# chahuja/mix-stage

Measured on AMD Instinct MI355X. Metric: train-step clips/sec (B=32, T=64, M=8), higher is better.
Workload: dtype f32; 1 GPU; Mix-StAGE GAN train step (reference D/G coin flip, seed 4321: 457 G + 510 D steps), B=32 clips per GPU, T=64, 128-mel, 104-dim pose, M=S=8, audio branch pinned; fp32 arithmetic (the reference trains in fp64, trainer.py:138; held to it at 1e-4 pose L1); global_batch=32, parallelism=dp1, hip_graphs=True, bn_sync=local

## Files before the change

### include/mixstage.h

```cpp
#ifndef MIXSTAGE_H_
#define MIXSTAGE_H_

#include <stddef.h>
#include <stdint.h>

#ifdef __cplusplus
extern "C" {
#endif

#define MS_ABI_VERSION 4

enum ms_block_mode {
  MS_BARE = 0,
  MS_LRELU = 1,
  MS_BN_TRAIN = 2,
  MS_BN_EVAL = 3
};

enum ms_input_mode {
  MS_IN_PLAIN = 0,
  MS_IN_BCAST = 1,
  MS_IN_UP2ADD = 2
};

enum ms_dtype { MS_F32 = 0, MS_BF16 = 1, MS_F16 = 2 };
#define MS_DT_OUT_F32 0x100
#define MS_DT_BN_FOLDED 0x200
#define MS_DT_STAT_PAIR 0x400

typedef struct ms_conv_desc {
  int32_t B;
  int32_t Cin;
  int32_t H, W;
  int32_t Cout;
  int32_t groups;
  int32_t KH, KW, SH, SW, PH, PW;
  int32_t OH, OW;
  int32_t mode;
  int32_t in_mode;
  float slope;
  float eps;
  float momentum;
  int32_t dtype;
} ms_conv_desc;

const char* ms_last_error(void);
int ms_abi_version(void);
int ms_stat_pair_ok(const ms_conv_desc* d);

size_t ms_conv_block_fwd_workspace(const ms_conv_desc* d);
size_t ms_conv_block_bwd_workspace(const ms_conv_desc* d);

int ms_conv_block_fwd(const ms_conv_desc* d, const float* x, const float* x2, const float* w,
                      const float* bias, const float* gamma, const float* beta, float* running_mean,
                      float* running_var, float* y_raw, float* y, float* save, void* workspace,
                      size_t workspace_bytes, void* stream);

typedef struct ms_fwd_options {
  const void* w_planes;
  int32_t* bn_sync;
  int32_t bn_sync_words;
} ms_fwd_options;
int ms_conv_block_fwd_ex(const ms_conv_desc* d, const float* x, const float* x2, const float* w,
                         const float* bias, const float* gamma, const float* beta, float* running_mean,
                         float* running_var, float* y_raw, float* y, float* save, void* workspace,
                         size_t workspace_bytes, void* stream, const ms_fwd_options* opt);
size_t ms_fwd_weights_bytes(const ms_conv_desc* d);
int ms_fwd_weights_prepare(int n, const ms_conv_desc* descs, const float* const* w, void* const* planes, void* stream);

int ms_conv_block_bwd(const ms_conv_desc* d, const float* x, const float* x2, const float* w,
                      const float* gamma, const float* running_mean, const float* running_var,
                      const float* y_raw, const float* y, const float* save, const float* dy, float* dyr,
                      float* dx, float* dx2, float* dw, float* dbias, float* dgamma, float* dbeta,
                      void* workspace, size_t workspace_bytes, void* stream);

typedef struct ms_bwd_options {
  void* side_stream;
  void* side_workspace;
  size_t side_workspace_bytes;
  const float* wt_prepared;
  float* wgrad_partials;
  int defer_wgrad_launch;
  const float* prev_y;
  const float* prev_y_raw;
  const float* prev_save;
  const float* prev_gamma;
  float* prev_dgamma;
  float* prev_dbeta;
  float* prev_dbias;
  float prev_slope;
  int32_t* bn_sync;
  int32_t bn_sync_words;
  int dy_is_dyr;
  const float* dx_accum;
} ms_bwd_options;
int ms_dgrad_takes_accum(const ms_conv_desc* d);
int ms_dgrad_fuses_prev_bn(const ms_conv_desc* d);
int ms_conv_block_bwd_ex(const ms_conv_desc* d, const float* x, const float* x2, const float* w,
                         const float* gamma, const float* running_mean, const float* running_var,
                         const float* y_raw, const float* y, const float* save, const float* dy, float* dyr,
                         float* dx, float* dx2, float* dw, float* dbias, float* dgamma, float* dbeta,
                         void* workspace, size_t workspace_bytes, void* stream, const ms_bwd_options* opt);

typedef struct ms_prep16_item {
  const ms_conv_desc* desc;
  const float* w;
  const float* bias;
  const float* gamma;
  const float* beta;
  const float* running_mean;
  const float* running_var;
  void* fwd;
  void* dgrad;
} ms_prep16_item;
size_t ms_weights16_bytes(const ms_conv_desc* d, int which);
int ms_weights16_prepare(int n, const ms_prep16_item* items, void* stream);

int ms_set_bn_sync_buffer(int32_t* zeroed_words, int n);

int ms_cb8_from_plain(int dtype, const float* x, void* y, int B, int C, int HW, void* stream);
int ms_cb8_to_plain(int dtype, const void* x, float* y, int B, int C, int HW, void* stream);
int ms_cb8_from_btc(int dtype, const float* x, void* y, int B, int T, int C, int velocity, void* stream);
int ms_cb8_to_btc(int dtype, const void* x, float* y, int B, int T, int C, int velocity_bwd, void* stream);

size_t ms_dgrad_weights_elems(const ms_conv_desc* d, const float* w);
int ms_set_precision(int mode);
int ms_get_precision(void);
int ms_tuning_epoch(void);
int ms_dgrad_weights_prepare(int n, const ms_conv_desc* descs, const float* const* w, float* const* wt, void* stream);

size_t ms_wgrad_partials_elems(const ms_conv_desc* d, int* splits);
int ms_set_wgrad_batched(int on, int tiles_per_workgroup);
int ms_wgrad_flush(void* stream);
int ms_wgrad_discard(void);
int ms_wgrad_reduce_multi(int n, const float* const* partials, float* const* dw, const int* elems, const int* splits,
                          void* stream);

int ms_bn_stats(const float* y_raw, float* stats, int B, int C, int HW, void* stream);
int ms_bn_train_apply(const float* stats_all, int world, int n_local, const float* gamma, const float* beta, float* running_mean,
                      float* running_var, const float* y_raw, float* y, float* save, int B, int C, int HW, float eps,
                      float momentum, float slope, void* stream);
size_t ms_bn_bwd_workspace(int B, int C);
int ms_bn_bwd_sums(const float* dy, const float* y_raw, const float* save, float* sums, int B, int C, int HW, float slope,
                   void* workspace, size_t workspace_bytes, void* stream);
int ms_bn_bwd_apply(const float* dy, const float* y_raw, const float* save, const float* gamma, const float* sums_global,
                    double n_global, float* dyr, int B, int C, int HW, float slope, void* stream);

int ms_lerp_time_fwd(const float* x, float* y, int B, int C, int Tin, int F, int Tout, void* stream);
int ms_lerp_time_bwd(const float* dy, float* dx, int B, int C, int Tin, int F, int Tout, void* stream);

int ms_softmax_mix_fwd(const float* z, const float* score, float* soft, float* out, int B, int M, int P,
                       int T, void* stream);
int ms_softmax_mix_bwd(const float* z, const float* soft, const float* dout, float* dz, float* dscore,
                       int B, int M, int P, int T, void* stream);

#define MS_CHAIN_MAX_BLOCKS 4
typedef struct ms_chain_desc {
  int32_t B, M, T, cin0, C, P, n_blocks;
  int32_t mode;
  int32_t dtype;
  int32_t sync_first_word;
  int32_t keep_all_raw;
  float slope, eps, momentum;
} ms_chain_desc;
typedef struct ms_chain_tensors {
  const void* x;
  const float* score;
  const float* w[MS_CHAIN_MAX_BLOCKS];
  const float* bias[MS_CHAIN_MAX_BLOCKS];
  const float* gamma[MS_CHAIN_MAX_BLOCKS];
  const float* beta[MS_CHAIN_MAX_BLOCKS];
  float* running_mean[MS_CHAIN_MAX_BLOCKS];
  float* running_var[MS_CHAIN_MAX_BLOCKS];
  void* y_raw[MS_CHAIN_MAX_BLOCKS];
  void* y[MS_CHAIN_MAX_BLOCKS];
  float* save[MS_CHAIN_MAX_BLOCKS];
  const float* w_logits;
  const float* bias_logits;
  float* z;
  float* soft;
  float* out;
  const void* prepared;
  int32_t* sync;
  int32_t sync_words;
} ms_chain_tensors;
int ms_decoder_chain_supported(const ms_chain_desc* d);
size_t ms_decoder_chain_prepared_bytes(const ms_chain_desc* d);
size_t ms_decoder_chain_workspace(const ms_chain_desc* d);
int ms_decoder_chain_sync_words(const ms_chain_desc* d);
int ms_decoder_chain_prepare(const ms_chain_desc* d, const float* const* w, const float* w_logits, void* prepared, void* stream);
int ms_decoder_chain_fwd(const ms_chain_desc* d, const ms_chain_tensors* t, void* workspace, size_t workspace_bytes, void* stream);

int ms_decoder_chain_eval_supported(const ms_chain_desc* d);
size_t ms_decoder_chain_eval_workspace(const ms_chain_desc* d);
int ms_decoder_chain_eval_sync_words(const ms_chain_desc* d);
int ms_decoder_chain_eval_plan(const ms_chain_desc* d, int32_t* n_tiles, int32_t* groups_per_workgroup, int32_t* tile_first,
                               int32_t* own_lo, int32_t* own_hi, int32_t cap);
int ms_decoder_chain_eval_fwd(const ms_chain_desc* d, const ms_chain_tensors* t, void* workspace, size_t workspace_bytes, void* stream);

int ms_kmeans_labels(const float* pose, const int32_t* keep, const double* centers, int64_t* labels, int B, int T, int P,
                     int PK, int M, int feats, void* stream);
int ms_znorm_select(const float* x, const int32_t* keep, const double* mean, const double* inv_std, float* y, size_t rows,
                    int P, int PK, void* stream);

int ms_step_metrics(const float* ycap, const float* gt, const int32_t* keep, const int32_t* slot_of, const double* mean,
                    const double* stdv, const float* alphas, int n_alpha, double* out, int B, int T, int P, int PK,
                    void* stream);
int ms_eval_accumulate(const float* ycap, const float* gt, const int32_t* keep, const double* mean, const double* stdv,
                       double* fid_sums, double* fid_gram, unsigned long long* w1_hist, int B, int T, int P, int PK,
                       double bin_width, int nbins, void* stream);

int ms_concat_style_fwd(const float* x, const float* emb, const int64_t* ids, int ids_stride_b, int ids_stride_t, float* out,
                        int B, int C, int D, int T, void* stream);
int ms_concat_style_bwd(const float* dout, const int64_t* ids, int ids_stride_b, int ids_stride_t, float* dx, float* demb,
                        int B, int C, int D, int T, int S, void* stream);

int ms_cross_entropy_fwd(const float* score, const int64_t* target, float* loss, float* row_scratch,
                         int n_outer, int n_inner, int C, int stride_outer, int stride_c,
                         int stride_inner, void* stream);
// ... 54 lines not shown
```

### include/mixstage_aux.h

```cpp
#ifndef MIXSTAGE_AUX_H_
#define MIXSTAGE_AUX_H_

#include "mixstage.h"

#ifdef __cplusplus
extern "C" {
#endif

int ms_set_counter_buffer(int32_t* zeroed_counters, int n);

int ms_conv_block_bwd_overlap(const ms_conv_desc* d, const float* x, const float* x2, const float* w,
                              const float* gamma, const float* running_mean, const float* running_var,
                              const float* y_raw, const float* y, const float* save, const float* dy, float* dyr,
                              float* dx, float* dx2, float* dw, float* dbias, float* dgamma, float* dbeta,
                              void* workspace, size_t workspace_bytes, void* stream, void* side_stream,
                              void* side_workspace, size_t side_workspace_bytes);

int ms_timing_enable(int on);
size_t ms_timing_report(char* buf, size_t cap);

int ms_debug_set_patch_min_workgroups(int n);
int ms_debug_set_patch_tuning(int intra_split, int force_splitk);

int ms_debug_set_conv16_tile(int wm, int wn);
int ms_debug_set_conv16_ring(int nstg, int wide8);
int ms_debug_set_wgrad16_target(int workgroups);
int ms_debug_set_wgrad16_ring(int buffers);
int ms_debug_set_wgrad_target(int workgroups);
int ms_debug_set_wgrad_wave(int on);
int ms_debug_set_conv_tile(int on);
int ms_debug_set_bn_fused(int on);
int ms_debug_set_bn_fused_min_workgroups(int n);
int ms_debug_set_skip(const char* patterns);

int ms_debug_set_clip32(int on);

int ms_selftest_mfma(const float* A, const float* B, float* C, int K, void* stream);
int ms_probe_peak(int kind, long iters, void* a, void* b, double* work, void* stream);

#ifdef __cplusplus
}
#endif
#endif
```

### mix_stage_amd/_lib.py

```python
import ctypes
import os

_HERE = os.path.dirname(os.path.abspath(__file__))
LIB_PATH = os.path.join(_HERE, 'libmixstage_hip.so')
_ALT_LIB = os.environ.get('MS_LIB_PATH')
if _ALT_LIB:
  LIB_PATH = _ALT_LIB

c_void_p, c_int, c_float, c_size_t = ctypes.c_void_p, ctypes.c_int, ctypes.c_float, ctypes.c_size_t


class BwdOptions(ctypes.Structure):
  _fields_ = [('side_stream', ctypes.c_void_p), ('side_workspace', ctypes.c_void_p), ('side_workspace_bytes', ctypes.c_size_t),
              ('wt_prepared', ctypes.c_void_p), ('wgrad_partials', ctypes.c_void_p), ('defer_wgrad_launch', ctypes.c_int),
              ('prev_y', ctypes.c_void_p), ('prev_y_raw', ctypes.c_void_p), ('prev_save', ctypes.c_void_p), ('prev_gamma', ctypes.c_void_p),
              ('prev_dgamma', ctypes.c_void_p), ('prev_dbeta', ctypes.c_void_p), ('prev_dbias', ctypes.c_void_p), ('prev_slope', ctypes.c_float),
              ('bn_sync', ctypes.c_void_p), ('bn_sync_words', ctypes.c_int32), ('dy_is_dyr', ctypes.c_int),
              ('dx_accum', ctypes.c_void_p)]


class LossScale(ctypes.Structure):
  _fields_ = [('scale', ctypes.c_float), ('scale_dev', ctypes.c_void_p)]


class FwdOptions(ctypes.Structure):
  _fields_ = [('w_planes', ctypes.c_void_p), ('bn_sync', ctypes.c_void_p), ('bn_sync_words', ctypes.c_int32)]


class ConvDesc(ctypes.Structure):
  _fields_ = [(n, ctypes.c_int32) for n in
              ('B', 'Cin', 'H', 'W', 'Cout', 'groups', 'KH', 'KW', 'SH', 'SW', 'PH', 'PW', 'OH', 'OW',
               'mode', 'in_mode')] + \
             [('slope', c_float), ('eps', c_float), ('momentum', c_float), ('dtype', ctypes.c_int32)]


class ChainDesc(ctypes.Structure):
  _fields_ = [(n, ctypes.c_int32) for n in ('B', 'M', 'T', 'cin0', 'C', 'P', 'n_blocks', 'mode', 'dtype', 'sync_first_word', 'keep_all_raw')] + \
             [('slope', c_float), ('eps', c_float), ('momentum', c_float)]


class ChainTensors(ctypes.Structure):
  _fields_ = [('x', ctypes.c_void_p), ('score', ctypes.c_void_p)] + \
             [(n, ctypes.c_void_p * 4) for n in ('w', 'bias', 'gamma', 'beta', 'running_mean', 'running_var', 'y_raw', 'y', 'save')] + \
             [(n, ctypes.c_void_p) for n in ('w_logits', 'bias_logits', 'z', 'soft', 'out', 'prepared', 'sync')] + \
             [('sync_words', ctypes.c_int32)]


class Prep16Item(ctypes.Structure):
  _fields_ = [('desc', ctypes.POINTER(ConvDesc))] + [(n, ctypes.c_void_p) for n in
             ('w', 'bias', 'gamma', 'beta', 'running_mean', 'running_var', 'fwd', 'dgrad')]


MS_BARE, MS_LRELU, MS_BN_TRAIN, MS_BN_EVAL = 0, 1, 2, 3
MS_IN_PLAIN, MS_IN_BCAST, MS_IN_UP2ADD = 0, 1, 2
MS_F32, MS_BF16, MS_F16, MS_DT_OUT_F32, MS_DT_BN_FOLDED = 0, 1, 2, 0x100, 0x200
MS_DT_STAT_PAIR = 0x400

_P = c_void_p
_DESC = ctypes.POINTER(ConvDesc)

SIGNATURES = {
    'ms_last_error': (ctypes.c_char_p, []),
    'ms_abi_version': (c_int, []),
    'ms_set_counter_buffer': (c_int, [_P, c_int]),
    'ms_set_bn_sync_buffer': (c_int, [_P, c_int]),
    'ms_debug_set_bn_fused': (c_int, [c_int]),
    'ms_debug_set_bn_fused_min_workgroups': (c_int, [c_int]),
    'ms_conv_block_fwd_workspace': (c_size_t, [_DESC]),
    'ms_conv_block_bwd_workspace': (c_size_t, [_DESC]),
    'ms_conv_block_fwd': (c_int, [_DESC] + [_P] * 11 + [_P, c_size_t, _P]),
    'ms_conv_block_bwd': (c_int, [_DESC] + [_P] * 17 + [_P, c_size_t, _P]),
    'ms_conv_block_bwd_overlap': (c_int, [_DESC] + [_P] * 17 + [_P, c_size_t, _P, _P, _P, c_size_t]),
    'ms_conv_block_bwd_ex': (c_int, [_DESC] + [_P] * 17 + [_P, c_size_t, _P, _P]),
    'ms_dgrad_weights_elems': (c_size_t, [_DESC, _P]),
    'ms_dgrad_weights_prepare': (c_int, [c_int, _P, _P, _P, _P]),
    'ms_tuning_epoch': (c_int, []),
    'ms_conv_block_fwd_ex': (c_int, [_DESC] + [_P] * 11 + [_P, c_size_t, _P, _P]),
    'ms_fwd_weights_bytes': (c_size_t, [_DESC]),
    'ms_fwd_weights_prepare': (c_int, [c_int, _P, _P, _P, _P]),
    'ms_set_precision': (c_int, [c_int]),
    'ms_get_precision': (c_int, []),
    'ms_wgrad_partials_elems': (c_size_t, [_DESC, _P]),
    'ms_wgrad_reduce_multi': (c_int, [c_int, _P, _P, _P, _P, _P]),
    'ms_wgrad_flush': (c_int, [_P]),
    'ms_wgrad_discard': (c_int, []),
    'ms_weights16_bytes': (c_size_t, [_DESC, c_int]),
    'ms_weights16_prepare': (c_int, [c_int, _P, _P]),
    'ms_cb8_from_plain': (c_int, [c_int, _P, _P, c_int, c_int, c_int, _P]),
    'ms_cb8_to_plain': (c_int, [c_int, _P, _P, c_int, c_int, c_int, _P]),
    'ms_cb8_from_btc': (c_int, [c_int, _P, _P, c_int, c_int, c_int, c_int, _P]),
    'ms_cb8_to_btc': (c_int, [c_int, _P, _P, c_int, c_int, c_int, c_int, _P]),
    'ms_bn_stats': (c_int, [_P, _P, c_int, c_int, c_int, _P]),
    'ms_bn_train_apply': (c_int, [_P, c_int, c_int, _P, _P, _P, _P, _P, _P, _P, c_int, c_int, c_int, c_float, c_float, c_float, _P]),
    'ms_bn_bwd_workspace': (c_size_t, [c_int, c_int]),
    'ms_bn_bwd_sums': (c_int, [_P, _P, _P, _P, c_int, c_int, c_int, c_float, _P, c_size_t, _P]),
    'ms_bn_bwd_apply': (c_int, [_P, _P, _P, _P, _P, ctypes.c_double, _P, c_int, c_int, c_int, c_float, _P]),
    'ms_lerp_time_fwd': (c_int, [_P, _P, c_int, c_int, c_int, c_int, c_int, _P]),
    'ms_lerp_time_bwd': (c_int, [_P, _P, c_int, c_int, c_int, c_int, c_int, _P]),
    'ms_softmax_mix_fwd': (c_int, [_P, _P, _P, _P, c_int, c_int, c_int, c_int, _P]),
    'ms_softmax_mix_bwd': (c_int, [_P, _P, _P, _P, _P, c_int, c_int, c_int, c_int, _P]),
    'ms_kmeans_labels': (c_int, [_P, _P, _P, _P, c_int, c_int, c_int, c_int, c_int, c_int, _P]),
    'ms_znorm_select': (c_int, [_P, _P, _P, _P, _P, c_size_t, c_int, c_int, _P]),
    'ms_step_metrics': (c_int, [_P] * 7 + [c_int, _P, c_int, c_int, c_int, c_int, _P]),
    'ms_eval_accumulate': (c_int, [_P] * 8 + [c_int, c_int, c_int, c_int, ctypes.c_double, c_int, _P]),
    'ms_concat_style_fwd': (c_int, [_P, _P, _P, c_int, c_int, _P, c_int, c_int, c_int, c_int, _P]),
    'ms_concat_style_bwd': (c_int, [_P, _P, c_int, c_int, _P, _P, c_int, c_int, c_int, c_int, c_int, _P]),
    'ms_cross_entropy_fwd': (c_int, [_P, _P, _P, _P] + [c_int] * 6 + [_P]),
    'ms_cross_entropy_bwd': (c_int, [_P, _P, _P, _P] + [c_int] * 7 + [_P]),
    'ms_cross_entropy_fwd_ex': (c_int, [_P, _P, _P] + [c_int] * 6 + [_P, _P]),
    'ms_cross_entropy_bwd_ex': (c_int, [_P, _P, _P, _P] + [c_int] * 7 + [_P, _P]),
    'ms_lp_mean_fwd_ex': (c_int, [c_int, _P, _P, c_float, _P, _P, c_size_t, _P, _P]),
    'ms_lp_mean_bwd_ex': (c_int, [c_int, _P, _P, c_float, _P, _P, c_size_t, _P, _P]),
    'ms_lp_mean_pair_fwd': (c_int, [c_int, _P, _P, _P, c_size_t, _P, _P]),
    'ms_lp_mean_pair_bwd': (c_int, [c_int, _P, _P, _P, _P, _P, c_size_t, _P, _P]),
    'ms_velocity_fwd': (c_int, [_P, _P, c_int, c_int, c_int, _P]),
    'ms_velocity_bwd': (c_int, [_P, _P, c_int, c_int, c_int, _P]),
    'ms_transpose_btc': (c_int, [_P, _P, c_int, c_int, c_int, _P]),
    'ms_transpose_bct': (c_int, [_P, _P, c_int, c_int, c_int, _P]),
    'ms_l1_mean_fwd': (c_int, [_P, _P, c_float, _P, _P, c_size_t, _P]),
    'ms_l1_mean_bwd': (c_int, [_P, _P, c_float, _P, _P, c_size_t, _P]),
    'ms_l2_mean_fwd': (c_int, [_P, _P, c_float, _P, _P, c_size_t, _P]),
    'ms_l2_mean_bwd': (c_int, [_P, _P, c_float, _P, _P, c_size_t, _P]),
    'ms_copy_multi': (c_int, [c_int, _P, _P, _P, _P]),
    'ms_write_floats': (c_int, [_P, _P, c_int, _P]),
    'ms_decoder_chain_supported': (c_int, [_P]),
    'ms_decoder_chain_prepared_bytes': (c_size_t, [_P]),
    'ms_decoder_chain_workspace': (c_size_t, [_P]),
    'ms_decoder_chain_sync_words': (c_int, [_P]),
    'ms_decoder_chain_prepare': (c_int, [_P, _P, _P, _P, _P]),
    'ms_decoder_chain_fwd': (c_int, [_P, _P, _P, c_size_t, _P]),
    'ms_decoder_chain_eval_supported': (c_int, [_P]),
    'ms_decoder_chain_eval_workspace': (c_size_t, [_P]),
    'ms_decoder_chain_eval_sync_words': (c_int, [_P]),
    'ms_decoder_chain_eval_plan': (c_int, [_P, _P, _P, _P, _P, _P, c_int]),
    'ms_decoder_chain_eval_fwd': (c_int, [_P, _P, _P, c_size_t, _P]),
    'ms_sqnorm': (c_int, [_P, c_size_t, _P, _P, _P]),
    'ms_adam_step': (c_int, [_P, _P, _P, _P, c_size_t, _P, c_float, c_float, c_float, c_float, c_float, _P, _P]),
    'ms_adam_step_segmented': (c_int, [_P, _P, _P, _P, c_size_t, _P, c_float, c_float, c_float, c_float, c_float, _P, _P, _P, _P,
                                       c_int, _P]),
    'ms_reduce_partials_count': (c_size_t, [c_size_t]),
    'ms_timing_enable': (c_int, [c_int]),
    'ms_timing_report': (c_size_t, [ctypes.c_char_p, c_size_t]),
    'ms_debug_set_patch_min_workgroups': (c_int, [c_int]),
    'ms_debug_set_patch_tuning': (c_int, [c_int, c_int]),
    'ms_debug_set_conv16_tile': (c_int, [c_int, c_int]),
    'ms_debug_set_conv16_ring': (c_int, [c_int, c_int]),
    'ms_debug_set_skip': (c_int, [ctypes.c_char_p]),
    'ms_debug_set_clip32': (c_int, [c_int]),
    'ms_debug_set_wgrad16_target': (c_int, [c_int]),
    'ms_debug_set_wgrad16_ring': (c_int, [c_int]),
    'ms_debug_set_wgrad_target': (c_int, [c_int]),
    'ms_debug_set_wgrad_wave': (c_int, [c_int]),
    'ms_debug_set_conv_tile': (c_int, [c_int]),
    'ms_set_wgrad_batched': (c_int, [c_int, c_int]),
    'ms_dgrad_fuses_prev_bn': (c_int, [_P]),
    'ms_dgrad_takes_accum': (c_int, [_P]),
    'ms_stat_pair_ok': (c_int, [_P]),
    'ms_selftest_mfma': (c_int, [_P, _P, _P, c_int, _P]),
    'ms_probe_peak': (c_int, [c_int, ctypes.c_long, _P, _P, ctypes.POINTER(ctypes.c_double), _P]),
}

_lib = None


class MixStageLibError(RuntimeError):
  pass


def lib():
  global _lib
  if _lib is None:
    if not os.path.isfile(LIB_PATH):
      raise MixStageLibError('%s not built: run `make -C mix_stage_amd/csrc` (or __graft_entry__.build()); '
                             'there is no CPU fallback' % LIB_PATH)
    handle = ctypes.CDLL(LIB_PATH)
    for name, (res, args) in SIGNATURES.items():
      if _ALT_LIB and name.startswith('ms_debug_') and not hasattr(handle, name):
        continue
      fn = getattr(handle, name)
      fn.restype, fn.argtypes = res, args
    mode = os.environ.get('MS_PRECISION', '')
    if mode:
      if mode not in ('fp32', 'bf16x6'):
        raise MixStageLibError('MS_PRECISION=%s: expected fp32 or bf16x6' % mode)
      handle.ms_set_precision(1 if mode == 'bf16x6' else 0)
    if os.environ.get('MS_BN_FUSED'):
      handle.ms_debug_set_bn_fused(int(os.environ['MS_BN_FUSED']))
    if os.environ.get('MS_BN_FUSED_MIN_WGS'):
      handle.ms_debug_set_bn_fused_min_workgroups(int(os.environ['MS_BN_FUSED_MIN_WGS']))
    if os.environ.get('MS_CLIP32'):
      handle.ms_debug_set_clip32(int(os.environ['MS_CLIP32']))
    if os.environ.get('MS_CONV_TILE'):
      handle.ms_debug_set_conv_tile(int(os.environ['MS_CONV_TILE']))
    if os.environ.get('MS_WGRAD_WAVE'):
      handle.ms_debug_set_wgrad_wave(int(os.environ['MS_WGRAD_WAVE']))
    if os.environ.get('MS_PATCH_MIN_WGS'):
      handle.ms_debug_set_patch_min_workgroups(int(os.environ['MS_PATCH_MIN_WGS']))
    _lib = handle
  return _lib


def check(rc, what):
  if rc != 0:
    raise MixStageLibError('%s failed: %s' % (what, lib().ms_last_error().decode()))
```

### mix_stage_amd/csrc/api.hip

```cpp
#include "block_geom.h"

namespace ms {
extern int g_clip32;

static int validate(const ms_conv_desc* d, const char* who) {
  if (!d) return set_error("%s: null descriptor", who);
  if (d->B < 1 || d->Cin < 1 || d->Cout < 1 || d->groups < 1 || d->H < 1 || d->W < 1 || d->KH < 1 || d->KW < 1 ||
      d->SH < 1 || d->SW < 1 || d->PH < 0 || d->PW < 0)
    return set_error("%s: bad geometry", who);
  const int oh = (d->H + 2 * d->PH - d->KH) / d->SH + 1, ow = (d->W + 2 * d->PW - d->KW) / d->SW + 1;
  if (d->H + 2 * d->PH < d->KH || d->W + 2 * d->PW < d->KW || oh != d->OH || ow != d->OW)
    return set_error("%s: output size (%d,%d) does not match geometry (expected %d,%d)", who, d->OH, d->OW, oh, ow);
  if (d->mode < MS_BARE || d->mode > MS_BN_EVAL) return set_error("%s: bad mode %d", who, d->mode);
  if (d->in_mode < MS_IN_PLAIN || d->in_mode > MS_IN_UP2ADD) return set_error("%s: bad in_mode %d", who, d->in_mode);
  if (d->in_mode == MS_IN_UP2ADD && (d->H != 1 || d->KH != 1 || (d->W & 1)))
    return set_error("%s: UP2ADD needs a 1-D block with even W", who);
  if (dt_of(d) > DT_F16 || (d->dtype & ~(0xff | MS_DT_OUT_F32 | MS_DT_BN_FOLDED | MS_DT_STAT_PAIR))) return set_error("%s: bad dtype 0x%x", who, d->dtype);
  if (dt_of(d) == DT_F32 && (d->dtype & ~(0xff | MS_DT_STAT_PAIR))) return set_error("%s: MS_DT_OUT_F32 is a flag of the 16-bit modes", who);
  if ((d->dtype & MS_DT_STAT_PAIR) && (d->B & 1)) return set_error("%s: MS_DT_STAT_PAIR needs an even batch", who);
  const double out_elems = (double)d->B * d->groups * d->Cout * d->OH * d->OW;
  const double in_elems = (double)d->B * d->groups * d->Cin * d->H * d->W;
  const double lim = dt_of(d) == DT_F32 ? 536870912.0 : 1073741824.0;
  if (out_elems >= lim || in_elems >= lim) return set_error("%s: tensor of 2 GiB or more (%.0f elements)", who, std::max(out_elems, in_elems));
  return 0;
}

static inline bool conv_c1_of(const ms_conv_desc* d) {
  return conv_c1_ok(d->groups, d->Cin, d->Cout, d->KH, d->KW, d->SH, d->SW, d->PH, d->PW, d->H, d->in_mode == MS_IN_PLAIN);
}
static inline bool wgrad_c1_of(const ms_conv_desc* d) {
  return dt_of(d) == DT_F32 && g_precision == 0 &&
         wgrad_c1_ok(d->groups, d->Cin, d->Cout, d->KH, d->KW, d->SH, d->SW, d->PH, d->PW, d->H, d->W, d->in_mode == MS_IN_PLAIN);
}

struct FwdPlan {
  BlockGeo g;
  bool clip, c1;
  int c1_tiles;
  PatchPlan pp;
  GatherPlan pl;
  bool pair_epilogue;
  size_t w_bytes;
  struct { size_t stats, part, counts, clip_w, planes, total; } ws;
};
static FwdPlan fwd_plan(const ms_conv_desc* d) {
  FwdPlan p;
  const BlockGeo g = p.g = geo_of(d);
  const bool train = d->mode == MS_BN_TRAIN;
  p.clip = g_precision == 0 && clip32_fwd_ok(d);
  p.c1 = conv_c1_of(d);
  p.c1_tiles = p.c1 ? conv_c1_tiles(d->B, d->H, d->W) : 0;
  p.pp = plan_patch(g.nd, d->Cout, d->groups, d->Cin, d->KH, d->KW, d->SH, d->SW, d->B, d->OH, d->OW, 1, d->W);
  p.pl = plan_gather(d->Cout, g.npix, d->groups, d->Cin * g.khw);
  const PatchPlan& pp = p.pp;
  const bool patch_slab = pp.ok && (pp.splitk > 1 || pp.ksi > 1);
  p.pair_epilogue = !train || ((long)d->B / 2 * g.hw <= 4096 && !p.c1 && (pp.ok ? patch_slab : p.pl.splitk > 1));
  const size_t planes_bytes = (pp.ok && pp.p6) ? (size_t)3 * g.C * patch6_row_elems(d->Cin, d->KH, d->KW) * 2 : 0;
  p.w_bytes = p.clip ? clip32_fwd_weight_bytes(d) : planes_bytes;

  const size_t slab = (size_t)g.npix * g.C * sizeof(float);
  auto tile_stats = [&](int n_tiles) { return align_up((size_t)n_tiles * g.C * 2 * sizeof(float), 256); };
  p.ws.stats = p.ws.part = 0;
  p.ws.counts = p.c1 ? tile_stats(p.c1_tiles) : pp.ok ? tile_stats(pp.n_tiles) : 0;
  size_t front = 256;
  if (train) front = std::max(front, (size_t)p.pl.n_tiles * g.C * 2 * sizeof(float));
  if (pp.ok && train) front = std::max(front, tile_stats(pp.n_tiles) + (size_t)pp.n_tiles * sizeof(float));
  if (patch_slab) front = std::max(front, pp.splitk * slab);
  if (p.pl.splitk > 1) front = std::max(front, p.pl.splitk * slab);
  if (p.c1) front = std::max(front, tile_stats(p.c1_tiles) + (size_t)p.c1_tiles * sizeof(float));
  p.ws.total = align_up(front, 256) + 256;
  p.ws.planes = carve(p.ws.total, align_up(planes_bytes, 256));
  p.ws.clip_w = p.clip ? clip32_part_bytes(d->Cout, d->B * d->OW / 32) : 0;
  if (p.clip) p.ws.total = std::max(p.ws.total, p.ws.clip_w + align_up(p.w_bytes, 256) + 256);
  return p;
}

struct BwdPlan {
  BlockGeo g;
  DgradGeo dg;
  int nchunk;
  bool dg_clip, dg_grouped;
  PatchPlan dpp;
  GatherPlan dpl;
  size_t wt_elems;
  size_t dg_planes_bytes;
  bool wg_c1;
  WgradPatchPlan wp;
  int wg_splits;
  int wg_splits_reserved;
  struct { size_t fuse_part, bn_part, colpart, wt, wg_part, dg_part, dg_planes, total; } ws;
};
static BwdPlan bwd_plan(const ms_conv_desc* d) {
  BwdPlan p;
  const BlockGeo g = p.g = geo_of(d);
  const DgradGeo dg = p.dg = dgrad_geo_of(d);
  int bpc;
  p.nchunk = bwd_chunks(d->B, g.C, &bpc);
  p.dg_clip = g_precision == 0 && clip32_dgrad_ok(d);
  p.dg_grouped = g_precision == 0 && g_clip32 && gdgrad32_ok(d);
  p.dpp = plan_patch(g.nd, d->Cin, dg.tg, dg.tcog, dg.jh, dg.jw, 1, 1, d->B, cdiv(d->H, d->SH), cdiv(d->W, d->SW), dg.ncls, d->OW);
  p.dpl = plan_gather(d->Cin, d->B * cdiv(d->H, d->SH) * cdiv(d->W, d->SW), dg.tg * dg.ncls, dg.tcog * dg.jh * dg.jw);
  p.wt_elems = dgrad_weight_elems(d->groups, d->Cout, d->Cin, d->KH, d->KW, d->SH, d->SW);
  p.dg_planes_bytes = (p.dpp.ok && p.dpp.p6) ? (size_t)3 * dg.ncls * dg.tg * d->Cin * patch6_row_elems(dg.tcog, dg.jh, dg.jw) * 2 : 0;
  p.wg_c1 = wgrad_c1_of(d);
  p.wp = WgradPatchPlan{};
  if (p.wg_c1) {
    p.wg_splits = p.wg_splits_reserved = wgrad_c1_splits(d->B, d->H);
  } else {
    p.wp = plan_wgrad_patch(g.nd, d->Cout, d->Cin * g.khw, d->groups, d->KH, d->KW, d->SH, d->SW, d->B, d->OH, d->OW, d->W, g.up2 != 0);
    const int gather_splits = wgrad_splits(d->Cout, d->Cin * g.khw, d->groups, g.npix);
    p.wg_splits = p.wp.ok ? p.wp.splits : gather_splits;
    p.wg_splits_reserved = std::max(p.wp.ok ? p.wp.splits : 1, gather_splits);
  }

  const size_t dx_bytes = (size_t)d->B * g.cin_tot * d->H * d->W * sizeof(float);
  p.ws.total = 0;
  p.ws.fuse_part = carve(p.ws.total, clip32_dgrad_bn_part_bytes(d));
  p.ws.bn_part = carve(p.ws.total, align_up((size_t)g.C * p.nchunk * 2 * sizeof(float), 256));
  p.ws.colpart = carve(p.ws.total, align_up((size_t)g.C * p.nchunk * sizeof(float), 256));
  p.ws.wt = carve(p.ws.total, align_up(std::max(p.wt_elems, std::max(clip32_dgrad_weight_floats(d), gdgrad32_weight_floats(d))) * sizeof(float), 256));
  p.ws.wg_part = carve(p.ws.total, align_up(wsize_of(d) * sizeof(float) * (p.wg_splits_reserved > 1 ? p.wg_splits_reserved : 0), 256));
  p.ws.dg_part = carve(p.ws.total, (p.dpp.ok && p.dpp.splitk > 1) ? align_up(p.dpp.splitk * dx_bytes, 256) : 0);
  p.ws.dg_planes = carve(p.ws.total, align_up(p.dg_planes_bytes, 256));
  if (p.dpl.splitk > 1) p.ws.total += align_up(p.dpl.splitk * dx_bytes, 256);
  p.ws.total += 256;
  return p;
}

enum { DW_NONE = 0, DW_TRANSPOSED = 1, DW_CLIP = 2, DW_GROUPED = 3 };
static int dgrad_weights_of(const ms_conv_desc* d, const BwdPlan& p, const float* w) {
  if (p.dg_clip) return DW_CLIP;
  if (p.dg_grouped) return DW_GROUPED;
  const bool direct = p.dpp.ok && !p.dpp.p6 && patch_dgrad_direct_ok(w, d->Cin, d->KH, d->KW, d->SH, d->SW, p.g.bcast != 0);
  return direct ? DW_NONE : DW_TRANSPOSED;
}
static size_t dgrad_weights_elems(const ms_conv_desc* d, const BwdPlan& p, int kind) {
  return kind == DW_CLIP ? clip32_dgrad_weight_floats(d) : kind == DW_GROUPED ? gdgrad32_weight_floats(d) : p.wt_elems;
}

}

using namespace ms;

extern "C" {

size_t ms_conv_block_fwd_workspace(const ms_conv_desc* d) {
  if (!d) return 256;
  return dt_of(d) != DT_F32 ? block_fwd16_workspace(d) : fwd_plan(d).ws.total;
}

size_t ms_conv_block_bwd_workspace(const ms_conv_desc* d) {
  if (!d) return 256;
  return dt_of(d) != DT_F32 ? block_bwd16_workspace(d) : bwd_plan(d).ws.total;
}

int ms_conv_block_fwd(const ms_conv_desc* d, const float* x, const float* x2, const float* w, const float* bias,
                      const float* gamma, const float* beta, float* running_mean, float* running_var, float* y_raw, float* y,
                      float* save, void* workspace, size_t workspace_bytes, void* stream) {
  return ms_conv_block_fwd_ex(d, x, x2, w, bias, gamma, beta, running_mean, running_var, y_raw, y, save, workspace,
                              workspace_bytes, stream, nullptr);
}

int ms_conv_block_fwd_ex(const ms_conv_desc* d, const float* x, const float* x2, const float* w, const float* bias,
                         const float* gamma, const float* beta, float* running_mean, float* running_var, float* y_raw,
                         float* y, float* save, void* workspace, size_t workspace_bytes, void* stream,
                         const ms_fwd_options* opt) {
  const unsigned short* w_planes = opt ? (const unsigned short*)opt->w_planes : nullptr;
  int rc = validate(d, "ms_conv_block_fwd");
  if (rc) return rc;
  if (!x || !w || !y) return set_error("ms_conv_block_fwd: null tensor");
  const bool bn = d->mode == MS_BN_TRAIN || d->mode == MS_BN_EVAL;
  if (bn && (!gamma || !beta || !running_mean || !running_var)) return set_error("ms_conv_block_fwd: BN tensors missing");
  if (d->mode == MS_BN_TRAIN && (!y_raw || !save || !workspace)) return set_error("ms_conv_block_fwd: y_raw/save/workspace missing");
  if (d->in_mode == MS_IN_UP2ADD && !x2) return set_error("ms_conv_block_fwd: UP2ADD needs x2");
  if (dt_of(d) != DT_F32)
    return block_fwd16(d, x, x2, w, bias, gamma, beta, running_mean, running_var, y_raw, y, save, workspace, workspace_bytes,
                       (hipStream_t)stream, w_planes, opt ? opt->bn_sync : nullptr, opt ? opt->bn_sync_words : 0);
  const FwdPlan p = fwd_plan(d);
  if (workspace_bytes < p.ws.total) return set_error("ms_conv_block_fwd: workspace too small");
  hipStream_t s = (hipStream_t)stream;
  const BlockGeo& g = p.g;
  const int C = g.C, npix = g.npix, hw = g.hw, Kg = d->Cin * g.khw;
  float* stats = ws_at<float>(workspace, p.ws.stats);
  float* counts = ws_at<float>(workspace, p.ws.counts);
  float* part = ws_at<float>(workspace, p.ws.part);

  if (p.clip) {
    const float* wp = (const float*)w_planes;
    if (!wp) {
      float* mine = ws_at<float>(workspace, p.ws.clip_w);
      rc = clip32_prep_queue(w, mine, d->Cout, d->Cin, d->KW, 0, d->Cin, s);
      if (!rc) rc = clip32_prep_flush(s);
      if (rc) return rc;
      wp = mine;
    }
    rc = clip32_block_fwd(d, x, x2, wp, bias, gamma, beta, running_mean, running_var, y_raw, y, save, stats, opt ? opt->bn_sync : nullptr,
                          opt ? opt->bn_sync_words : 0, s);
    if (rc != -2) return rc;
    rc = 0;
  }

  float* out = d->mode == MS_BN_TRAIN ? y_raw : y;
  const int a_vec = (Kg % 4 == 0) && (((uintptr_t)w & 15) == 0);
  const int ep = d->mode == MS_BARE ? EP_BARE : d->mode == MS_LRELU ? EP_LRELU : d->mode == MS_BN_EVAL ? EP_BN_EVAL : EP_RAW_STATS;
  const int sg = d->mode == MS_BN_TRAIN ? sg_of(d) : 1;
  if (sg > 1 && !p.pair_epilogue)
    return set_error("ms_conv_block_fwd: MS_DT_STAT_PAIR is not implemented for this block's kernels (ms_stat_pair_ok)");
  if (p.c1) {
    rc = launch_conv_c1(x, w, bias, out, gamma, beta, running_mean, running_var, stats, counts, d->B, d->H, d->W, ep, d->slope,
                        d->eps, s);
    if (rc) return rc;
    if (d->mode == MS_BN_TRAIN) {
      rc = launch_bn_finalize_apply(stats, counts, p.c1_tiles, 0, npix, C, gamma, beta, running_mean, running_var, save, d->eps,
                                    d->momentum, y_raw, y, d->B, hw, d->slope, s);
    }
    return rc;
  }
  if (p.pp.ok) {
    const PatchPlan& pp = p.pp;
    PatchArgs q = {};
    q.A = w; q.src = x; q.src2 = x2; q.out = out;
    q.bias = bias; q.bn_g = gamma; q.bn_b = beta; q.bn_m = running_mean; q.bn_v = running_var;
    q.stats = stats; q.counts = counts;
    q.Mg = d->Cout; q.Kg = Kg; q.groups = d->groups; q.Kc = d->Cin; q.bcast = g.bcast; q.a_vec = a_vec; q.ep = ep;
    fill_src(q, plane_strides(g.one_d, d->B, g.cin_tot, d->H, d->W));
    fill_out(q, plane_strides(g.one_d, d->B, C, d->OH, d->OW));
    q.PH = g.one_d ? 0 : d->PH;
    q.PW = d->PW; q.tiles_x = pp.tiles_x; q.tiles_y = pp.tiles_y; q.slope = d->slope; q.eps = d->eps;
    q.o_sh = 1; q.o_sw = 1; q.o_ry = 0; q.o_rx = 0;
    q.splitk = pp.splitk; q.chunks_per_split = pp.chunks_per_split;
    q.src_elems = (size_t)d->B * g.cin_tot * d->H * d->W; q.a_elems = (size_t)C * Kg;
    const bool raw_out = pp.splitk > 1 || (pp.ksi > 1 && d->mode == MS_BN_TRAIN);
    if (raw_out) { q.part = part; q.part_stride = (size_t)npix * C; }
    const double flops = 2.0 * d->Cout * Kg * (double)npix * d->groups;
    const double bytes = 4.0 * ((double)C * Kg + (double)d->B * g.cin_tot * d->H * d->W + (double)npix * C);
    if (pp.p6) {
      const int re = patch6_row_elems(d->Cin, d->KH, d->KW);
      const unsigned short* planes = w_planes;
      if (!planes) {
        unsigned short* mine = ws_at<unsigned short>(workspace, p.ws.planes);
        rc = launch_split_weights(w, mine, C, d->Cin, d->KH, d->KW, s);
        if (rc) return rc;
        planes = mine;
      }
      q.Aplanes = planes; q.plane_stride = (unsigned)((size_t)C * re); q.a_row_elems = re;
      rc = launch_patch6(q, pp, d->KH, d->KW, d->SW, g.up2 != 0, flops, bytes, s);
    } else {
      rc = launch_patch(q, pp, d->KH, d->KW, d->SW, g.up2 != 0, flops, bytes, s);
    }
    if (rc) return rc;
    if (raw_out)
      return launch_splitk_fwd_epilogue(q.part, pp.splitk, q.part_stride, bias, gamma, beta, running_mean, running_var, y_raw,
                                        y, save, d->B, C, hw, ep, d->slope, d->eps, d->momentum, s, sg);
    if (d->mode == MS_BN_TRAIN) {
      rc = launch_bn_finalize_apply(stats, counts, pp.n_tiles, 0, npix, C, gamma, beta, running_mean, running_var, save, d->eps,
                                    d->momentum, y_raw, y, d->B, hw, d->slope, s);
    }
    return rc;
  }
  const GatherPlan& pl = p.pl;
  GatherArgs a = {};
  a.A = w; a.src = x; a.src2 = x2; a.out = out;
  a.bias = bias; a.bn_g = gamma; a.bn_b = beta; a.bn_m = running_mean; a.bn_v = running_var;
  a.stats = stats;
  a.Mg = d->Cout; a.Kg = Kg; a.groups = d->groups; a.Kc = d->Cin;
  a.bcast = g.bcast; a.src_ctotal = g.cin_tot;
  a.SRCH = d->H; a.SRCW = d->W; a.OUTH = d->OH; a.OUTW = d->OW; a.Npix = npix;
  a.KH = d->KH; a.KW = d->KW; a.SH = d->SH; a.SW = d->SW; a.PH = d->PH; a.PW = d->PW;
  a.a_vec = a_vec; a.ep = ep;
  a.slope = d->slope; a.eps = d->eps;
  if (pl.splitk > 1) {
    a.part = part;
    a.part_stride = (size_t)npix * C;
  }
  rc = launch_gather(a, false, g.up2 != 0, pl, s);
  if (rc) return rc;
  if (pl.splitk > 1) {
    return launch_splitk_fwd_epilogue(a.part, pl.splitk, a.part_stride, bias, gamma, beta, running_mean, running_var, y_raw, y,
                                      save, d->B, C, hw, ep, d->slope, d->eps, d->momentum, s, sg);
  }
  if (d->mode == MS_BN_TRAIN) {
    rc = launch_bn_finalize_apply(stats, nullptr, pl.n_tiles, 64 * pl.tn, npix, C, gamma, beta, running_mean, running_var, save,
                                  d->eps, d->momentum, y_raw, y, d->B, hw, d->slope, s);
  }
  return rc;
}

size_t ms_wgrad_partials_elems(const ms_conv_desc* d, int* splits) {
  if (validate(d, "ms_wgrad_partials_elems")) return 0;
  const int sp = dt_of(d) != DT_F32 ? wgrad16_splits(d) : bwd_plan(d).wg_splits;
  if (splits) *splits = sp;
  return sp > 1 ? (size_t)sp * wsize_of(d) : 0;
}

int ms_wgrad_reduce_multi(int n, const float* const* partials, float* const* dw, const int* elems, const int* splits,
                          void* stream) {
  if (n < 0 || (n && (!partials || !dw || !elems || !splits))) return set_error("ms_wgrad_reduce_multi: null argument");
  ReduceBatch rb;
  rb.n = 0;
  for (int i = 0; i < n; ++i) {
    if (!partials[i] || !dw[i] || elems[i] <= 0 || splits[i] < 1) return set_error("ms_wgrad_reduce_multi: bad job %d", i);
    ReduceJob jb = {partials[i], dw[i], elems[i], splits[i], 0, 0};
    rb.job[rb.n++] = jb;
    if (rb.n == REDUCE_BATCH_MAX) {
      const int rc = launch_reduce_splits_multi(rb, (hipStream_t)stream);
      if (rc) return rc;
      rb.n = 0;
    }
  }
  return rb.n ? launch_reduce_splits_multi(rb, (hipStream_t)stream) : 0;
}

size_t ms_dgrad_weights_elems(const ms_conv_desc* d, const float* w) {
  if (validate(d, "ms_dgrad_weights_elems")) return 0;
  if (dt_of(d) != DT_F32) return 0;
  const BwdPlan p = bwd_plan(d);
  const int kind = dgrad_weights_of(d, p, w);
  if (kind == DW_NONE) return 0;
  return align_up(dgrad_weights_elems(d, p, kind), 64) + (p.dg_planes_bytes + 3) / 4;
}

size_t ms_fwd_weights_bytes(const ms_conv_desc* d) {
  if (validate(d, "ms_fwd_weights_bytes")) return 0;
  if (dt_of(d) != DT_F32) return 0;
  return fwd_plan(d).w_bytes;
}

int ms_fwd_weights_prepare(int n, const ms_conv_desc* descs, const float* const* w, void* const* planes, void* stream) {
  if (n < 0 || (n && (!descs || !w || !planes))) return set_error("ms_fwd_weights_prepare: null argument");
  PrepQueueGuard queue_guard;
  SplitBatch sb;
  sb.n = 0;
  for (int i = 0; i < n; ++i) {
    const ms_conv_desc* d = descs + i;
    int rc = validate(d, "ms_fwd_weights_prepare");
    if (rc) return rc;
    if (dt_of(d) != DT_F32) continue;
    const FwdPlan p = fwd_plan(d);
    if (!p.w_bytes) continue;
    if (!planes[i]) return set_error("ms_fwd_weights_prepare: block %d needs a buffer of ms_fwd_weights_bytes bytes", i);
    if (p.clip) {
      rc = clip32_prep_queue(w[i], (float*)planes[i], d->Cout, d->Cin, d->KW, 0, d->Cin, (hipStream_t)stream);
      if (rc) return rc;
      continue;
    }
    SplitJob jb = {w[i], (unsigned short*)planes[i], p.g.C, d->Cin, p.g.khw, 0, 0, 0};
    sb.job[sb.n++] = jb;
    if (sb.n == SPLIT_BATCH_MAX) {
      rc = launch_split_weights_multi(sb, (hipStream_t)stream);
      if (rc) return rc;
      sb.n = 0;
    }
// ... 183 lines not shown
    hipEvent_t ev = fork_event();
    if (!ev || hipEventRecord(ev, s) != hipSuccess || hipStreamWaitEvent(ws_stream, ev, 0) != hipSuccess)
      return set_error("ms_conv_block_bwd_overlap: stream fork failed");
  }

  bool dx_done = false;
  if (dx && p.dg_clip) {
    const float* wp = wt_prepared;
    if (!wp) {
      rc = clip32_prep_queue(w, wt, d->Cin, d->Cout, d->KW, d->KW == 4 ? 2 : 1, d->Cin, s);
      if (!rc) rc = clip32_prep_flush(s);
      if (rc) return rc;
      wp = wt;
    }
    if (have_prev) {
      const Clip32PrevBN pv = {opt->prev_y, opt->prev_y_raw, opt->prev_save, opt->prev_gamma, opt->prev_dgamma, opt->prev_dbeta, opt->prev_dbias, opt->prev_slope};
      rc = clip32_block_dgrad(d, gr, wp, dx, dx2, s, &pv, fuse_part, opt->bn_sync, opt->bn_sync_words, opt->dx_accum);
      if (rc == -2) return set_error("ms_conv_block_bwd: the fused data gradient is not resident at once on this device");
    } else {
      rc = clip32_block_dgrad(d, gr, wp, dx, dx2, s, nullptr, nullptr, nullptr, 0, opt->dx_accum);
    }
    if (rc && rc != -2) return rc;
    dx_done = rc == 0;
    rc = 0;
  }
  if (dx && !dx_done && p.dg_grouped) {
    const float* wp = wt_prepared;
    if (!wp) {
      rc = gdgrad32_prepare(d, w, wt, s);
      if (!rc) rc = gdgrad32_prep_flush(s);
      if (rc) return rc;
      wp = wt;
    }
    rc = gdgrad32_launch(d, gr, wp, dx, s);
    if (rc) return rc;
    dx_done = true;
  }
  if (dx && !dx_done) {
    const PatchPlan& pp0 = p.dpp;
    const int Kg2 = dg.tcog * dg.jh * dg.jw;
    const size_t dx_elems = (size_t)d->B * g.cin_tot * d->H * d->W;
    const bool direct = pp0.ok && !pp0.p6 && patch_dgrad_direct_ok(w, d->Cin, d->KH, d->KW, d->SH, d->SW, bcast);
    if (wt_prepared) {
      wt = const_cast<float*>(wt_prepared);
    } else if (!direct) {
      rc = launch_transpose_weight(w, wt, dg.tg, dg.tcog, d->Cin, d->KH, d->KW, d->SH, d->SW, d->PH, d->PW, pp0.ok ? 1 : 0, s);
      if (rc) return rc;
    }
    if (pp0.ok) {
      PatchArgs q = {};
      q.A = wt; q.src = gr; q.out = dx; q.out2 = dx2;
      q.Mg = d->Cin; q.Kg = Kg2; q.groups = dg.tg; q.Kc = dg.tcog; q.bcast = 0; q.a_vec = (Kg2 % 4 == 0);
      if (direct) { q.A = w; q.a_vec = 2; }
      q.ep = up2 ? EP_DGRAD_UP2 : EP_BARE; q.is_dgrad = 1;
      q.cls_a_stride = (unsigned)((size_t)dg.tg * d->Cin * Kg2);
      fill_src(q, plane_strides(g.one_d, d->B, C, d->OH, d->OW));
      fill_out(q, plane_strides(g.one_d, d->B, g.cin_tot, d->H, d->W));
      const double flops = fill_parity_classes(q, d, dg, g.one_d);
      const double bytes = 4.0 * ((double)dg.ncls * dg.tg * d->Cin * Kg2 + (double)d->B * C * hw) + 4.0 * (double)dx_elems;
      q.tiles_x = pp0.tiles_x; q.tiles_y = pp0.tiles_y;
      q.splitk = pp0.splitk; q.chunks_per_split = pp0.chunks_per_split;
      q.src_elems = (size_t)d->B * C * hw; q.a_elems = (size_t)dg.ncls * dg.tg * d->Cin * Kg2;
      if (pp0.splitk > 1) {
        q.part = dg_part; q.part_stride = dx_elems;
        q.ep = EP_BARE;
      }
      if (pp0.p6) {
        const int re = patch6_row_elems(dg.tcog, dg.jh, dg.jw), rows = dg.ncls * dg.tg * d->Cin;
        const unsigned short* planes;
        if (wt_prepared) {
          planes = (const unsigned short*)(wt_prepared + align_up(p.wt_elems, 64));
        } else {
          unsigned short* mine = ws_at<unsigned short>(workspace, p.ws.dg_planes);
          rc = launch_split_weights(wt, mine, rows, dg.tcog, dg.jh, dg.jw, s);
          if (rc) return rc;
          planes = mine;
        }
        q.Aplanes = planes; q.plane_stride = (unsigned)((size_t)rows * re); q.a_row_elems = re;
        q.cls_a_stride = (unsigned)(dg.tg * d->Cin);
        rc = launch_patch6(q, pp0, dg.jh, dg.jw, 1, false, flops, bytes, s);
      } else {
        rc = launch_patch(q, pp0, dg.jh, dg.jw, 1, false, flops, bytes, s);
      }
      if (rc) return rc;
      if (pp0.splitk > 1) {
        rc = launch_splitk_dgrad_epilogue(dg_part, pp0.splitk, dx_elems, dx, dx2, dx_elems, d->W, up2 ? 1 : 0, s);
        if (rc) return rc;
      }
    } else {
      const GatherPlan& pl = p.dpl;
      GatherArgs a = {};
      a.A = wt; a.src = gr; a.out = dx; a.out2 = dx2;
      a.Mg = d->Cin; a.Kg = Kg2; a.groups = dg.tg; a.Kc = dg.tcog; a.src_ctotal = C;
      a.SRCH = d->OH; a.SRCW = d->OW; a.OUTH = d->H; a.OUTW = d->W; a.Npix = d->B * d->H * d->W; a.batch = d->B;
      a.KH = dg.jh; a.KW = dg.jw; a.SH = d->SH; a.SW = d->SW; a.PH = d->PH; a.PW = d->PW;
      a.bcast = 0;
      a.a_vec = (a.Kg % 4 == 0);
      a.ep = up2 ? EP_DGRAD_UP2 : EP_DGRAD;
      if (pl.splitk > 1) {
        a.part = dg_part;
        a.part_stride = dx_elems;
        a.ep = EP_DGRAD;
      }
      rc = launch_gather(a, true, up2, pl, s);
      if (rc) return rc;
      if (pl.splitk > 1) {
        rc = launch_splitk_dgrad_epilogue(dg_part, pl.splitk, dx_elems, dx, dx2, dx_elems, d->W, up2 ? 1 : 0, s);
        if (rc) return rc;
      }
    }
  }

  if (dw && p.wg_c1) {
    rc = launch_wgrad_c1(gr, x, wg_part, d->B, d->H, d->W, ws_stream);
    if (!rc && !defer_wgrad) rc = launch_reduce_splits(wg_part, dw, C * Kg, p.wg_splits, ws_stream);
    return rc;
  }
  if (dw && p.wp.ok) {
    const WgradPatchPlan& wp = p.wp;
    WgradPatchArgs q = {};
    q.dyr = gr; q.src = x; q.src2 = x2;
    q.out = wp.splits > 1 ? wg_part : dw;
    q.Cog = d->Cout; q.Cig = d->Cin; q.Kg = Kg; q.groups = d->groups; q.bcast = bcast;
    fill_src(q, plane_strides(g.one_d, d->B, g.cin_tot, d->H, d->W));
    fill_out(q, plane_strides(g.one_d, d->B, C, d->OH, d->OW));
    q.PH = g.one_d ? 0 : d->PH;
    q.PW = d->PW; q.tiles_x = wp.tiles_x; q.tiles_y = wp.tiles_y; q.n_tiles = wp.n_tiles;
    q.tiles_per_split = wp.tiles_per_split; q.splits = wp.splits;
    const double flops = 2.0 * d->Cout * q.Kg * (double)npix * d->groups;
    const double bytes = 4.0 * ((double)npix * C + (double)d->B * g.cin_tot * d->H * d->W + (double)C * q.Kg);
    if (wp.splits > 1 && !defer_wgrad && !wp.p6) {
      q.counters = counter_region(CNT_WGRAD, cdiv(q.Kg, 64) * cdiv(d->Cout, 64) * d->groups);
      q.final_out = dw;
    }
    if (opt->defer_wgrad_launch && !wp.p6 && ws_stream == s && (wp.splits == 1 || defer_wgrad))
      return queue_wgrad_patch(q, wp, d->KH, d->KW, d->SW, up2, flops, bytes);
    rc = wp.p6 ? launch_wgrad_patch6(q, wp, d->KH, d->KW, d->SW, up2, flops, bytes, ws_stream)
               : launch_wgrad_patch(q, wp, d->KH, d->KW, d->SW, up2, flops, bytes, ws_stream);
    if (rc) return rc;
    if (wp.splits > 1 && !q.counters && !defer_wgrad) rc = launch_reduce_splits(wg_part, dw, C * q.Kg, wp.splits, ws_stream);
  } else if (dw) {
    WgradArgs a = {};
    a.dyr = gr; a.src = x; a.src2 = x2;
    a.Cog = d->Cout; a.Cig = d->Cin; a.Kg = Kg; a.groups = d->groups;
    a.src_ctotal = g.cin_tot;
    a.H = d->H; a.W = d->W; a.OH = d->OH; a.OW = d->OW; a.Npix = npix;
    a.KH = d->KH; a.KW = d->KW; a.SH = d->SH; a.SW = d->SW; a.PH = d->PH; a.PW = d->PW;
    a.bcast = bcast;
    rc = launch_wgrad(a, up2, dw, wg_part, defer_wgrad, ws_stream, opt->defer_wgrad_launch && ws_stream == s);
  }
  return rc;
}

}
```

### mix_stage_amd/csrc/clip32.hip

```cpp
#include <stdio.h>
#include <stdlib.h>

#include <algorithm>
#include <vector>

#include "kernels.h"
#include "conv16.h"

namespace ms {

typedef unsigned int cl_u32x4 __attribute__((ext_vector_type(4)));
typedef unsigned int cl_u32x2 __attribute__((ext_vector_type(2)));
constexpr int CL_SPIN_LIMIT = 1 << 21;
constexpr int CL_MAXK8W = 9;

struct Clip32Args {
  const float* x;
  const float* x2;
  const float* wp;
  const float* bias;
  const float* gamma;
  const float* beta;
  float* rm;
  float* rv;
  float* y_raw;
  float* y;
  float* y2;
  float* save;
  float* part;
  int* sync;
  int cnt_base;
  int B, Cin, Cout, To, Ti, ep, k8w, npw, rows_valid, nct;
  float slope, eps, momentum;
  const float* pv_y; const float* pv_y_raw; const float* pv_save; const float* pv_gamma;
  float* pv_dgamma; float* pv_dbeta; float* pv_dbias;
  int sg;
  int raw_all;
  const float* acc;
  int cx, px;
  unsigned long long* stamps;
};
#define CL_STAMP(k) do { if (p.stamps && threadIdx.x == 0) p.stamps[(size_t)blockIdx.x * 8 + (k)] = __builtin_amdgcn_s_memrealtime(); } while (0)

__host__ __device__ constexpr int cl_pslots(int n) { return (n + 3) & ~3; }
template <bool SPLIT>
__device__ __forceinline__ int cl_pos(int s, int half) { return SPLIT ? (s & 1) * half + (s >> 1) : s; }

__device__ __forceinline__ float cl_f4e(const float4& v, int j) { return j == 0 ? v.x : j == 1 ? v.y : j == 2 ? v.z : v.w; }

template <int CTRL>
__device__ __forceinline__ double cl_dpp_d(double x) {
  const unsigned long long u = __builtin_bit_cast(unsigned long long, x);
  const unsigned lo = (unsigned)__builtin_amdgcn_mov_dpp((int)(unsigned)u, CTRL, 0xf, 0xf, true);
  const unsigned hi = (unsigned)__builtin_amdgcn_mov_dpp((int)(unsigned)(u >> 32), CTRL, 0xf, 0xf, true);
  return __builtin_bit_cast(double, ((unsigned long long)hi << 32) | lo);
}
__device__ __forceinline__ double cl_sum8_d(double v) {
  v += cl_dpp_d<0xB1>(v);
  v += cl_dpp_d<0x4E>(v);
  v += cl_dpp_d<0x141>(v);
  return v;
}

__device__ __forceinline__ float cl_sum8(float v) {
  v += dpp_rot<0xB1>(v);
  v += dpp_rot<0x4E>(v);
  v += dpp_rot<0x141>(v);
  return v;
}

template <int KW, int S, int NB, bool UP2, int K8W, bool DG2 = false>
__global__ __launch_bounds__(256, 1) void clip32_kernel(const Clip32Args p) {
  prefetch_kernargs<sizeof(Clip32Args)>();
  extern __shared__ float cl_smem[];
  CL_STAMP(0);
  constexpr int NPX = 32 * NB;
  constexpr int NWR = (K8W ? K8W : CL_MAXK8W) * KW;
  const int t = threadIdx.x, lane = t & 63, w = t >> 6, n0 = lane & 31, h = lane >> 5;
  const int nct = p.nct;
  int ct = blockIdx.x % nct, pw = blockIdx.x / nct;
  if (p.cx) {
    const int xcd = blockIdx.x & 7, j = blockIdx.x >> 3, tpx = nct / p.cx, ppx = p.npw / p.px;
    const int xc = xcd % p.cx, xp = xcd / p.cx, jp = j / tpx;
    ct = xc * tpx + (j - jp * tpx);
    pw = xp * ppx + jp;
  }
  const int To = p.To, Ti = p.Ti;
  const int ncl = NPX / To;
  const int b0 = pw * ncl;
  const int row = Ti + 2;
  const int pslots = cl_pslots(ncl * row);
  constexpr bool SPLIT = S == 2 && !DG2;
  const int half = row >> 1;
  const int k8w = K8W ? K8W : p.k8w, nk8 = 4 * k8w;

  float4 wr[NWR];
  const float4* ws = reinterpret_cast<const float4*>(p.wp) + ((size_t)(ct * 4 + w) * k8w * KW) * 64 + lane;
  const bool own_planes = K8W > 0 && (Ti & 3) == 0;
  if (!own_planes) {
#pragma unroll
    for (int i = 0; i < NWR; ++i) wr[i] = ws[(size_t)min(i, k8w * KW - 1) * 64];
  }

  if (own_planes) {
    constexpr int NQ = DG2 ? 8 : 16;
    constexpr int NITEMS = 2 * K8W * NQ;
    constexpr int NI = K8W ? (NITEMS + 63) / 64 : 1;
    const int plw0 = 2 * K8W * w;
    for (int e = lane; e < ncl * 2 * 2 * K8W; e += 64) {
      const int pl = plw0 + e / (ncl * 2), r2 = e % (ncl * 2), cl = r2 >> 1, sl = (r2 & 1) ? Ti + 1 : 0;
      *reinterpret_cast<float4*>(cl_smem + ((size_t)pl * pslots + cl * row + sl) * 4) = float4{0.f, 0.f, 0.f, 0.f};
    }
    float4 v[NI][4];
    float2 va[NI][4];
#pragma unroll
    for (int q = 0; q < NI; ++q) {
      const int it = min(lane + 64 * q, NITEMS - 1);
      const int pl = plw0 + it / NQ, pos = 4 * (it % NQ);
      const int cl = pos / Ti, ti = pos - cl * Ti;
#pragma unroll
      for (int j = 0; j < 4; ++j) {
        const int c = min(4 * pl + j, p.Cin - 1);
        if (UP2) {
          v[q][j] = *reinterpret_cast<const float4*>(p.x2 + ((size_t)(b0 + cl) * p.Cin + c) * Ti + ti);
          va[q][j] = *reinterpret_cast<const float2*>(p.x + ((size_t)(b0 + cl) * p.Cin + c) * (Ti / 2) + ti / 2);
        } else {
          v[q][j] = *reinterpret_cast<const float4*>(p.x + ((size_t)(b0 + cl) * p.Cin + c) * Ti + ti);
        }
      }
    }
#pragma unroll
    for (int i = 0; i < NWR; ++i) wr[i] = ws[(size_t)i * 64];
#pragma unroll
    for (int q = 0; q < NI; ++q) {
      const int it = lane + 64 * q;
      if (it < NITEMS) {
        const int pl = plw0 + it / NQ, pos = 4 * (it % NQ);
        const int cl = pos / Ti, ti = pos - cl * Ti;
        float o[4][4];
#pragma unroll
        for (int j = 0; j < 4; ++j) {
          const bool ok = 4 * pl + j < p.Cin;
          float4 u = v[q][j];
          if (UP2) { u.x += va[q][j].x; u.y += va[q][j].x; u.z += va[q][j].y; u.w += va[q][j].y; }
          o[0][j] = ok ? u.x : 0.f; o[1][j] = ok ? u.y : 0.f; o[2][j] = ok ? u.z : 0.f; o[3][j] = ok ? u.w : 0.f;
        }
        float* dst = cl_smem + ((size_t)pl * pslots + cl * row) * 4;
#pragma unroll
        for (int f = 0; f < 4; ++f) *reinterpret_cast<float4*>(dst + 4 * cl_pos<SPLIT>(1 + ti + f, half)) = float4{o[f][0], o[f][1], o[f][2], o[f][3]};
      }
    }
  } else {
    const int npos = ncl * Ti;
    for (int e = t; e < ncl * 2; e += 256) {
      const int cl = e >> 1, sl = (e & 1) ? Ti + 1 : 0;
      for (int pl = 0; pl < nk8 * 2; ++pl) *reinterpret_cast<float4*>(cl_smem + ((size_t)pl * pslots + cl * row + sl) * 4) = float4{0.f, 0.f, 0.f, 0.f};
    }
    const int pos = t % npos, pl0 = t / npos, pstep = 256 / npos;
    const int cl = pos / Ti, ti = pos - cl * Ti;
    const size_t xoff = (size_t)(b0 + cl) * p.Cin * (UP2 ? Ti / 2 : Ti) + (UP2 ? ti / 2 : ti);
    const size_t x2off = (size_t)(b0 + cl) * p.Cin * Ti + ti;
    const int cstride = UP2 ? Ti / 2 : Ti;
    for (int plb = pl0; plb < nk8 * 2; plb += 8 * pstep) {
      float v[8][4];
#pragma unroll
      for (int i = 0; i < 8; ++i) {
        const int pl = plb + i * pstep;
#pragma unroll
        for (int j = 0; j < 4; ++j) {
          const int c = min(4 * pl + j, p.Cin - 1);
          float val = p.x[xoff + (size_t)c * cstride];
          if (UP2) val += p.x2[x2off + (size_t)c * Ti];
          v[i][j] = val;
        }
      }
#pragma unroll
      for (int i = 0; i < 8; ++i) {
        const int pl = plb + i * pstep;
        if (pl < nk8 * 2) {
          float4 o;
          o.x = 4 * pl < p.Cin ? v[i][0] : 0.f;
          o.y = 4 * pl + 1 < p.Cin ? v[i][1] : 0.f;
          o.z = 4 * pl + 2 < p.Cin ? v[i][2] : 0.f;
          o.w = 4 * pl + 3 < p.Cin ? v[i][3] : 0.f;
          *reinterpret_cast<float4*>(cl_smem + ((size_t)pl * pslots + cl * row + cl_pos<SPLIT>(1 + ti, half)) * 4) = o;
        }
      }
    }
  }
  const int chl = t >> 3, pq = t & 7;
  const int cgl = ct * 32 + chl;
  const bool rowok = cgl < p.rows_valid;
  const int cgc = min(cgl, p.rows_valid - 1);
  const float bias_c = p.bias ? p.bias[cgc] : 0.f;
  float gam = 1.f, bet = 0.f, rmo = 0.f, rvo = 1.f;
  if (p.ep == EP_RAW_STATS || p.ep == EP_BN_EVAL) { gam = p.gamma[cgc]; bet = p.beta[cgc]; rmo = p.rm[cgc]; rvo = p.rv[cgc]; }
  constexpr int FPT_ = NPX / 8;
  float av[UP2 ? 1 : FPT_];
  if constexpr (!UP2) {
#pragma unroll
    for (int k = 0; k < FPT_; ++k) av[k] = 0.f;
    if (p.acc && rowok) {
      const int f0a = FPT_ * pq;
      if (To >= FPT_) {
        const int cl = f0a / To, tt = f0a - cl * To;
        const float* sp = p.acc + ((size_t)(b0 + cl) * p.Cout + cgl) * To + tt;
#pragma unroll
        for (int k = 0; k < FPT_; k += 4) {
          const float4 u = *reinterpret_cast<const float4*>(sp + k);
          av[k] = u.x; av[k + 1] = u.y; av[k + 2] = u.z; av[k + 3] = u.w;
        }
      } else {
#pragma unroll
        for (int k = 0; k < FPT_; ++k) {
          const int f = f0a + k, cl = f / To, tt = f - cl * To;
          av[k] = p.acc[((size_t)(b0 + cl) * p.Cout + cgl) * To + tt];
        }
      }
    }
  }
  CL_STAMP(1);
  if (own_planes) {
    __builtin_amdgcn_fence(__ATOMIC_RELEASE, "wavefront");
    __builtin_amdgcn_wave_barrier();
    __builtin_amdgcn_fence(__ATOMIC_ACQUIRE, "wavefront");
  } else {
    __syncthreads();
  }
  CL_STAMP(2);

  f32x16 acc[NB];
#pragma unroll
  for (int nb = 0; nb < NB; ++nb)
#pragma unroll
    for (int q = 0; q < 16; ++q) acc[nb][q] = 0.f;
// ... 188 lines not shown
      group_stats(pw0, mean, m2);
      expired = lflag[0] != 0;
      if (expired) { mean = __builtin_nan(""); }
    }
    const float var = (float)(m2 / n), fmean = (float)mean;
    const float invstd = 1.0f / sqrtf(var + p.eps);
    sc = gam * invstd;
    sh = bet - fmean * sc;
    if (pw == pw0 && pq == 0 && rowok && fmean == fmean && p.save) {
      float* sv = p.save + (size_t)sgi * 4 * p.Cout;
      sv[cgl] = fmean; sv[p.Cout + cgl] = invstd; sv[2 * p.Cout + cgl] = sc; sv[3 * p.Cout + cgl] = sh;
    }
    if (pw == (p.sg - 1) * npg && !expired) {
      float rmc = rmo, rvc = rvo;
      for (int gi = 0; gi + 1 < p.sg; ++gi) {
        double gmean, gm2;
        group_stats(gi * npg, gmean, gm2);
        if (pq == 0 && rowok) {
          const float ub = n > 1.0 ? (float)(gm2 / (n - 1.0)) : (float)(gm2 / n);
          running_stats_update(&p.rm[cgl], &p.rv[cgl], rmc, rvc, p.momentum, (float)gmean, ub);
          rmc = p.rm[cgl]; rvc = p.rv[cgl];
        }
      }
      if (pq == 0 && rowok && fmean == fmean) {
        const float unbiased = n > 1.0 ? (float)(m2 / (n - 1.0)) : var;
        running_stats_update(&p.rm[cgl], &p.rv[cgl], rmc, rvc, p.momentum, fmean, unbiased);
      }
    }
    if (p.y_raw && rowok && (p.raw_all || bn_inv_unsafe(fmean, invstd, sc, sh, p.slope))) store_frames(p.y_raw, v);
  } else if (p.ep == EP_BN_EVAL) {
    sc = gam * (1.0f / sqrtf(rvo + p.eps));
    sh = bet - rmo * sc;
  } else if (p.ep == EP_DGRAD_BN) {
    const int C = p.Cout;
    const float mean = p.pv_save[cgc], invstd = p.pv_save[C + cgc], scp = p.pv_save[2 * C + cgc], shp = p.pv_save[3 * C + cgc];
    const float gm = p.pv_gamma[cgc];
    const bool from_y = !bn_inv_unsafe(mean, invstd, scp, shp, p.slope);
    const float* src = from_y ? p.pv_y : p.pv_y_raw;
    float yv[FPT];
    if (To >= FPT) {
      const int cl = f0 / To, tt = f0 - cl * To;
      const float* sp = src + ((size_t)(b0 + cl) * C + cgc) * To + tt;
#pragma unroll
      for (int k = 0; k < FPT; k += 4) {
        const float4 u = *reinterpret_cast<const float4*>(sp + k);
        yv[k] = u.x; yv[k + 1] = u.y; yv[k + 2] = u.z; yv[k + 3] = u.w;
      }
    } else {
#pragma unroll
      for (int k = 0; k < FPT; ++k) {
        const int f = f0 + k, cl = f / To, tt = f - cl * To;
        yv[k] = src[((size_t)(b0 + cl) * C + cgc) * To + tt];
      }
    }
    const float beta_c = fmaf(mean, scp, shp), inv_sl = 1.0f / p.slope, inv_g = invstd / scp;
    float dz[FPT], xh[FPT];
    float s1 = 0.f, s2 = 0.f, s3 = 0.f;
#pragma unroll
    for (int k = 0; k < FPT; ++k) {
      bool pos;
      float xv;
      if (from_y) {
        pos = yv[k] > 0.f;
        xv = ((pos ? yv[k] : yv[k] * inv_sl) - beta_c) * inv_g;
      } else {
        pos = fmaf(yv[k], scp, shp) > 0.f;
        xv = (yv[k] - mean) * invstd;
      }
      dz[k] = v[k] * (pos ? 1.f : p.slope);
      xh[k] = xv;
      s1 += dz[k];
      s2 = fmaf(dz[k], xv, s2);
      s3 += xv;
    }
    s1 = cl_sum8(s1); s2 = cl_sum8(s2); s3 = cl_sum8(s3);
    double S1 = (double)s1, S2 = (double)s2, S3 = (double)s3;
    if (p.npw > 1) {
      const __amdgpu_buffer_rsrc_t rsPart = buf_rsrc(p.part);
      if (pq == 0)
        __builtin_amdgcn_raw_buffer_store_b128(__builtin_bit_cast(cl_u32x4, float4{s1, s2, s3, 0.f}), rsPart,
                                               (int)(16u * (unsigned)((ct * p.npw + pw) * 32 + chl)), 0, 16);
      asm volatile("s_waitcnt vmcnt(0)" ::: "memory");
      __syncthreads();
      int* lflag = reinterpret_cast<int*>(cl_smem + 4 * 32 * RP);
      if (t == 0) {
        int* counter = p.sync + p.cnt_base + 32 * ct;
        const int prior = __hip_atomic_load(p.sync, __ATOMIC_RELAXED, __HIP_MEMORY_SCOPE_AGENT);
        const unsigned old = (unsigned)__hip_atomic_fetch_add(counter, 1, __ATOMIC_RELAXED, __HIP_MEMORY_SCOPE_AGENT);
        const unsigned target = (old / (unsigned)p.npw + 1u) * (unsigned)p.npw;
        int spins = 0, bad = 0;
        while ((int)((unsigned)__hip_atomic_load(counter, __ATOMIC_RELAXED, __HIP_MEMORY_SCOPE_AGENT) - target) < 0) {
          __builtin_amdgcn_s_sleep(2);
          if (++spins > CL_SPIN_LIMIT) { __hip_atomic_store(p.sync, 21, __ATOMIC_RELAXED, __HIP_MEMORY_SCOPE_AGENT); bad = 1; break; }
        }
        lflag[0] = bad | (prior != 0);
      }
      __syncthreads();
      const unsigned base = 16u * (unsigned)(ct * p.npw * 32 + chl);
      double a1 = 0.0, a2 = 0.0, a3 = 0.0;
      float4 pv4[4];
      for (int i0 = pq; i0 < p.npw; i0 += 32) {
#pragma unroll
        for (int u = 0; u < 4; ++u) {
          const int i = min(i0 + 8 * u, p.npw - 1);
          pv4[u] = __builtin_bit_cast(float4, __builtin_amdgcn_raw_buffer_load_b128(rsPart, (int)(base + 16u * (unsigned)(i * 32)), 0, 16));
        }
#pragma unroll
        for (int u = 0; u < 4; ++u)
          if (i0 + 8 * u < p.npw) { a1 += (double)pv4[u].x; a2 += (double)pv4[u].y; a3 += (double)pv4[u].z; }
      }
      S1 = cl_sum8_d(a1); S2 = cl_sum8_d(a2); S3 = cl_sum8_d(a3);
      if (lflag[0]) S1 = __builtin_nan("");
    }
    const double n = (double)p.npw * NPX;
    const float m1 = (float)(S1 / n), m2 = (float)(S2 / n), gi = gm * invstd;
#pragma unroll
    for (int k = 0; k < FPT; ++k) v[k] = gi * (dz[k] - m1 - xh[k] * m2);
    if (pw == 0 && pq == 0 && rowok) {
      if (p.pv_dgamma) { p.pv_dgamma[cgl] = (float)S2; p.pv_dbeta[cgl] = (float)S1; }
      if (p.pv_dbias) p.pv_dbias[cgl] = -gi * m2 * (float)S3;
    }
    if (rowok) store_frames(p.y, v);
    return;
  }
  if (!rowok) return;
  if (p.ep == EP_DGRAD_UP2) {
    store_frames(p.y2, v);
    float hv[FPT / 2];
#pragma unroll
    for (int k = 0; k < FPT / 2; ++k) hv[k] = v[2 * k] + v[2 * k + 1];
    const int Th = To / 2, fh = f0 / 2;
    if (Th >= FPT / 2) {
      const int cl = fh / Th, tt = fh - cl * Th;
      float* d = p.y + ((size_t)(b0 + cl) * p.Cout + cgl) * Th + tt;
#pragma unroll
      for (int k = 0; k < FPT / 2; ++k) d[k] = hv[k];
    } else {
#pragma unroll
      for (int k = 0; k < FPT / 2; ++k) {
        const int f = fh + k, cl = f / Th, tt = f - cl * Th;
        p.y[((size_t)(b0 + cl) * p.Cout + cgl) * Th + tt] = hv[k];
      }
    }
    return;
  }
  if (p.ep != EP_BARE) {
#pragma unroll
    for (int k = 0; k < FPT; ++k) v[k] = lrelu(p.ep == EP_LRELU ? v[k] : fmaf(v[k], sc, sh), p.slope);
  }
  store_frames(p.y, v);
  CL_STAMP(7);
}

struct ClipPrepJob {
  const float* w;
  float* out;
  int rows, red, KW, k8w, transposed, w_rows, w_cols, block_end;
};
enum { CLIP_PREP_MAX = 40 };
struct ClipPrepBatch { int n; ClipPrepJob job[CLIP_PREP_MAX]; };

constexpr int CLP_LDS = 32 * 289;
__global__ __launch_bounds__(256) void clip32_prep_kernel(const ClipPrepBatch pb) {
  __shared__ float lds[CLP_LDS];
  int j = 0;
  while (j + 1 < pb.n && (int)blockIdx.x >= pb.job[j].block_end) ++j;
  const ClipPrepJob& jb = pb.job[j];
  const int blk = blockIdx.x - (j ? pb.job[j - 1].block_end : 0);
  const int wv = blk & 3, ct = blk >> 2, t = threadIdx.x;
  const int KW = jb.KW, k8w = jb.k8w;
  const int c_lo = wv * k8w * 8, nc = min(k8w * 8, max(0, jb.red - c_lo));
  const int r_lo = 32 * ct, nr = min(32, jb.rows - r_lo);
  int pitch;
  if (!jb.transposed) {
    const int seg = nc * KW;
    pitch = (k8w * 8 * KW) | 1;
    for (int k = t; k < seg; k += 256) {
      const float* src = jb.w + ((size_t)r_lo * jb.w_cols + c_lo) * KW + k;
      const size_t rstride = (size_t)jb.w_cols * KW;
      float v[32];
#pragma unroll
      for (int rr = 0; rr < 32; ++rr) v[rr] = src[(size_t)min(rr, nr - 1) * rstride];
#pragma unroll
      for (int rr = 0; rr < 32; ++rr)
        if (rr < nr) lds[rr * pitch + k] = v[rr];
    }
  } else {
    const int seg = nr * KW;
    pitch = (32 * KW) | 1;
    const int n = nc * seg;
    for (int e0 = t; e0 < n; e0 += 8 * 256) {
      float v[8];
      int dst[8];
#pragma unroll
      for (int u = 0; u < 8; ++u) {
        const int e = min(e0 + 256 * u, n - 1);
        const int cc = e / seg, k = e - cc * seg;
        dst[u] = cc * pitch + k;
        v[u] = jb.w[((size_t)(c_lo + cc) * jb.w_cols + r_lo) * KW + k];
      }
#pragma unroll
      for (int u = 0; u < 8; ++u)
        if (e0 + 256 * u < n) lds[dst[u]] = v[u];
    }
  }
  __syncthreads();
  float4* dst = reinterpret_cast<float4*>(jb.out) + ((size_t)(ct * 4 + wv) * k8w * KW) * 64;
  const int lane = t & 63, rr = lane & 31, h = lane >> 5;
  for (int u = t >> 6; u < k8w * KW; u += 4) {
    const int k8l = u / KW, tap = u - k8l * KW;
    float vv[4];
#pragma unroll
    for (int q = 0; q < 4; ++q) {
      const int cl = 8 * k8l + 4 * h + q;
      float val = 0.f;
      if (rr < nr && cl < nc) val = jb.transposed ? lds[cl * pitch + rr * KW + (jb.transposed == 1 ? KW - 1 - tap : tap)] : lds[rr * pitch + cl * KW + tap];
      vv[q] = val;
    }
    dst[(size_t)u * 64 + lane] = float4{vv[0], vv[1], vv[2], vv[3]};
  }
}

int g_clip32 = 1;

static int clip_k8w(int red) { return (cdiv(red, 8) + 3) / 4; }

static bool clip_geom_ok(int B, int rows, int red, int To, int KW, int S, int groups, int nb) {
  if (!g_clip32 || groups != 1) return false;
  if (!((KW == 3 && S == 1) || (KW == 4 && S == 2))) return false;
  if (To < 1 || To > 32 * nb || (To & (To - 1))) return false;
  if ((B * To) % (32 * nb)) return false;
  if (red > 8 * 4 * CL_MAXK8W || rows < 1) return false;
  return true;
}

bool clip32_fwd_ok(const ms_conv_desc* d) {
  if ((d->dtype & 0xff) != 0) return false;
  if (!(d->H == 1 && d->KH == 1 && d->PW == 1 && d->in_mode != MS_IN_BCAST)) return false;
  const int nb = d->SW == 2 ? 1 : 2;
  if (d->in_mode == MS_IN_UP2ADD && !(d->KW == 3 && d->SW == 1)) return false;
  if (d->OW * d->SW != d->W) return false;
  return clip_geom_ok(d->B, d->Cout, d->Cin, d->OW, d->KW, d->SW, d->groups, nb);
}

bool clip32_dgrad_ok(const ms_conv_desc* d) {
  if ((d->dtype & 0xff) != 0) return false;
  if (!(d->H == 1 && d->KH == 1 && d->PW == 1 && d->in_mode != MS_IN_BCAST)) return false;
  if (d->KW == 4 && d->SW == 2) return d->in_mode == 0 && 2 * d->OW == d->W && clip_geom_ok(d->B, d->Cin, d->Cout, d->W, 4, 2, d->groups, 2);
  if (!(d->KW == 3 && d->SW == 1)) return false;
  return clip_geom_ok(d->B, d->Cin, d->Cout, d->W, 3, 1, d->groups, 2);
}

size_t clip32_weight_floats(int rows, int red, int KW) { return (size_t)cdiv(rows, 32) * 4 * clip_k8w(red) * KW * 256; }

size_t clip32_fwd_weight_bytes(const ms_conv_desc* d) { return clip32_fwd_ok(d) ? clip32_weight_floats(d->Cout, d->Cin, d->KW) * 4 : 0; }
size_t clip32_dgrad_weight_floats(const ms_conv_desc* d) { return clip32_dgrad_ok(d) ? clip32_weight_floats(d->Cin, d->Cout, d->KW) : 0; }

static ClipPrepBatch g_prep;
static int g_prep_blocks = 0;
int clip32_prep_queue(const float* w, float* out, int rows, int red, int KW, int transposed, int w_cols, hipStream_t s) {
  if (g_prep.n == CLIP_PREP_MAX) { const int rc = clip32_prep_flush(s); if (rc) return rc; }
  ClipPrepJob jb = {w, out, rows, red, KW, clip_k8w(red), transposed, 0, w_cols, 0};
  g_prep_blocks += cdiv(rows, 32) * 4;
  jb.block_end = g_prep_blocks;
  g_prep.job[g_prep.n++] = jb;
  return 0;
}
void clip32_prep_discard() { g_prep.n = 0; g_prep_blocks = 0; }
int clip32_prep_flush(hipStream_t s) {
  if (!g_prep.n) return 0;
  TimingScope ts(s, 0, 0, "clip32_prep_kernel|clip_prep jobs%d", g_prep.n);
  const int blocks = g_prep_blocks;
  ClipPrepBatch pb = g_prep;
  g_prep.n = 0; g_prep_blocks = 0;
  if (ts.skip()) return 0;
  hipLaunchKernelGGL(clip32_prep_kernel, dim3(blocks), dim3(256), 0, s, pb);
  return check_launch("clip32_prep_kernel");
}

size_t clip32_part_bytes(int rows, int npw) { return align_up((size_t)cdiv(rows, 32) * npw * 32 * 2 * sizeof(float), 256); }
int clip32_sync_words(int rows) { return 32 * (cdiv(rows, 32) + 1); }

template <int KW, int S, int NB, bool UP2, int K8W, bool DG2 = false>
static int clip32_launch_k(const Clip32Args& a, int nwg, int lds_bytes, hipStream_t s) {
  auto fn = clip32_kernel<KW, S, NB, UP2, K8W, DG2>;
  static unsigned long long attr_done = 0;
  if (first_time_on_device(attr_done)) {
    if (hipFuncSetAttribute(reinterpret_cast<const void*>(fn), hipFuncAttributeMaxDynamicSharedMemorySize, 160 * 1024) != hipSuccess)
      return set_error("clip32: cannot raise the dynamic LDS limit");
    done_on_device(attr_done);
  }
  hipLaunchKernelGGL(fn, dim3(nwg), dim3(256), lds_bytes, s, a);
  return check_launch("clip32_kernel");
}
template <int KW, int S, int NB, bool UP2, bool DG2 = false>
static int clip32_launch_t(const Clip32Args& a, int nwg, int lds_bytes, hipStream_t s) {
  switch (a.k8w) {
    case 2: return clip32_launch_k<KW, S, NB, UP2, 2, DG2>(a, nwg, lds_bytes, s);
    case 4: return clip32_launch_k<KW, S, NB, UP2, 4, DG2>(a, nwg, lds_bytes, s);
    case 8: return clip32_launch_k<KW, S, NB, UP2, 8, DG2>(a, nwg, lds_bytes, s);
    case 9: return clip32_launch_k<KW, S, NB, UP2, 9, DG2>(a, nwg, lds_bytes, s);
    default: return clip32_launch_k<KW, S, NB, UP2, 0, DG2>(a, nwg, lds_bytes, s);
  }
}

int clip32_launch(Clip32Args a, int KW, int S, bool up2, const char* what, hipStream_t s, bool dg2 = false) {
  const int nb = (S == 2 && !dg2) ? 1 : 2, npx = 32 * nb;
  a.k8w = clip_k8w(a.Cin);
  a.npw = a.B * a.To / npx;
  if (a.sg < 1) a.sg = 1;
  if (a.npw % a.sg) return -2;
  const int nct = cdiv(a.Cout, 32);
  a.nct = nct;
  const int ncl = npx / a.To, pslots = cl_pslots(ncl * (a.Ti + 2));
  const int img = 4 * a.k8w * 2 * pslots * 16, red = (4 * 32 * (npx + 4) + 4) * 4;
  const int lds = std::max(img, red);
  if (lds > 160 * 1024) return set_error("clip32: image of %d bytes", lds);
  const int nwg = nct * a.npw;
  static int xcd_on = -1;
  if (xcd_on < 0) { const char* e = getenv("MS_CLIP_XCD"); xcd_on = e ? atoi(e) : 1; }
  a.cx = a.px = 0;
  if (xcd_on && nwg % 8 == 0) {
    const double wct = 32.0 * a.Cin * KW, imgb = (double)a.Cin * ncl * a.Ti * (up2 ? 1.5 : 1.0);
    double best = nct % 8 == 0 ? wct * (nct / 8) + imgb * a.npw : 1e30;
    for (int cx = 4; cx >= 1; cx >>= 1) {
      const int px = 8 / cx;
      if (nct % cx || a.npw % px) continue;
      const double cost = wct * (nct / cx) + imgb * (a.npw / px);
      if (cost < best) { best = cost; a.cx = cx; a.px = px; }
    }
  }
  int cus = 256;
  cus = current_device_cus();
  if (!cus) cus = 256;
  if ((a.ep == EP_RAW_STATS || a.ep == EP_DGRAD_BN) && a.npw > 1 && nwg > cus) return -2;
  const double flops = 2.0 * a.rows_valid * a.Cin * (dg2 ? 2 : KW) * (double)a.B * a.To;
  const double bytes = 4.0 * ((double)a.rows_valid * a.Cin * KW + (double)a.B * a.Cin * a.Ti + (double)a.B * a.rows_valid * a.To);
  TimingScope ts(s, flops, bytes, "clip32_kernel<%d,%d,%d,%d>|conv_%s_clip k1x%d s%d rows%d red%d T%d B%d ep%d", KW, S, nb, up2 ? 1 : 0, what, KW,
                 S, a.rows_valid, a.Cin, a.To, a.B, a.ep);
  if (ts.skip()) return 0;
  static int dbg = -1;
  if (dbg < 0) { const char* e = getenv("MS_CLIP_DBG"); dbg = e ? atoi(e) : 0; }
  static unsigned long long* g_stamps = nullptr;
  if (dbg & 32) {
    if (!g_stamps && hipMalloc(&g_stamps, 4096 * 8 * 8) != hipSuccess) g_stamps = nullptr;
    if (g_stamps) (void)hipMemsetAsync(g_stamps, 0, 4096 * 8 * 8, s);
    a.stamps = nwg <= 4096 ? g_stamps : nullptr;
  }
  int rc;
  if (dg2) rc = clip32_launch_t<4, 1, 2, false, true>(a, nwg, lds, s);
  else if (KW == 3 && S == 1) rc = up2 ? clip32_launch_t<3, 1, 2, true>(a, nwg, lds, s) : clip32_launch_t<3, 1, 2, false>(a, nwg, lds, s);
  else rc = clip32_launch_t<4, 2, 1, false>(a, nwg, lds, s);
  if (a.stamps) {
    std::vector<unsigned long long> h((size_t)nwg * 8);
    if (hipStreamSynchronize(s) == hipSuccess && hipMemcpy(h.data(), g_stamps, h.size() * 8, hipMemcpyDeviceToHost) == hipSuccess) {
      unsigned long long t0 = ~0ull;
      for (int i = 0; i < nwg; ++i) t0 = std::min(t0, h[(size_t)i * 8]);
      fprintf(stderr, "clip32 %s k%d s%d rows%d red%d ep%d: stamps (us after the first workgroup's entry; min / median / max over %d workgroups)\n", what, KW, S,
              a.rows_valid, a.Cin, a.ep, nwg);
      for (int k = 0; k < 8; ++k) {
        std::vector<double> v;
        for (int i = 0; i < nwg; ++i) if (h[(size_t)i * 8 + k]) v.push_back((double)(h[(size_t)i * 8 + k] - t0) * 0.01);
        if (v.empty()) continue;
        std::sort(v.begin(), v.end());
        fprintf(stderr, "  stamp %d: %7.2f %7.2f %7.2f\n", k, v.front(), v[v.size() / 2], v.back());
      }
    }
  }
  return rc;
}

int clip32_block_fwd(const ms_conv_desc* d, const float* x, const float* x2, const float* wp, const float* bias, const float* gamma,
                     const float* beta, float* rm, float* rv, float* y_raw, float* y, float* save, float* part, int* sync,
                     int sync_words, hipStream_t s) {
  Clip32Args a = {};
  a.x = x; a.x2 = x2; a.wp = wp; a.bias = bias; a.gamma = gamma; a.beta = beta; a.rm = rm; a.rv = rv;
  a.y_raw = d->mode == MS_BN_TRAIN ? y_raw : nullptr; a.y = y; a.save = save; a.part = part; a.sync = sync; a.cnt_base = 32;
  a.B = d->B; a.Cin = d->Cin; a.Cout = d->Cout; a.rows_valid = d->Cout; a.To = d->OW; a.Ti = d->W;
  a.ep = d->mode == MS_BARE ? EP_BARE : d->mode == MS_LRELU ? EP_LRELU : d->mode == MS_BN_EVAL ? EP_BN_EVAL : EP_RAW_STATS;
  a.slope = d->slope; a.eps = d->eps; a.momentum = d->momentum;
  if (a.ep == EP_RAW_STATS && (!sync || sync_words < 32 + clip32_sync_words(d->Cout) || !part)) return -2;
  a.sg = a.ep == EP_RAW_STATS ? sg_of(d) : 1;
  a.raw_all = (long)d->B / a.sg * d->OW > BN_BWD32_FUSED_MAX ? 1 : 0;
  return clip32_launch(a, d->KW, d->SW, d->in_mode == MS_IN_UP2ADD, "fwd", s);
}

bool clip32_dgrad_bn_ok(const ms_conv_desc* d) {
  if (!clip32_dgrad_ok(d) || d->in_mode != MS_IN_PLAIN) return false;
  const int cus = current_device_cus();
  return cus > 0 && cdiv(d->Cin, 32) * (d->B * d->W / 64) <= cus;
}
size_t clip32_dgrad_bn_part_bytes(const ms_conv_desc* d) {
  return clip32_dgrad_ok(d) && d->in_mode == MS_IN_PLAIN ? align_up((size_t)cdiv(d->Cin, 32) * (d->B * d->W / 64) * 32 * 4 * sizeof(float), 256) : 0;
}

int clip32_block_dgrad(const ms_conv_desc* d, const float* g, const float* wp, float* dx, float* dx2, hipStream_t s,
                       const Clip32PrevBN* pv, float* part, int* sync, int sync_words, const float* accum) {
  Clip32Args a = {};
  const bool up2 = d->in_mode == MS_IN_UP2ADD;
  if (accum && up2) return set_error("clip32 data gradient: dx_accum with an upsample-add input");
  a.acc = accum;
  a.x = g; a.wp = wp;
  a.y = dx; a.y2 = dx2;
  a.B = d->B; a.Cin = d->Cout; a.Cout = d->Cin; a.rows_valid = d->Cin; a.To = d->W; a.Ti = d->W;
  a.ep = up2 ? EP_DGRAD_UP2 : EP_BARE;
  if (pv) {
    if (up2 || !part || !sync || sync_words < 32 + clip32_sync_words(d->Cin) || !pv->y || !pv->y_raw || !pv->save || !pv->gamma)
      return set_error("clip32 data gradient with the producer's BatchNorm backward: missing buffer");
    a.ep = EP_DGRAD_BN;
    a.pv_y = pv->y; a.pv_y_raw = pv->y_raw; a.pv_save = pv->save; a.pv_gamma = pv->gamma;
    a.pv_dgamma = pv->dgamma; a.pv_dbeta = pv->dbeta; a.pv_dbias = pv->dbias;
    a.slope = pv->slope; a.part = part; a.sync = sync; a.cnt_base = 32;
  }
  if (d->KW == 4) {
    a.Ti = d->OW;
    return clip32_launch(a, 4, 2, false, "dgrad", s, true);
  }
  return clip32_launch(a, 3, 1, false, "dgrad", s);
}

}
```

### mix_stage_amd/csrc/kernels.h

```cpp
#pragma once
#include "common.h"

namespace ms {

enum { EP_BARE = 0, EP_LRELU = 1, EP_BN_EVAL = 2, EP_RAW_STATS = 3, EP_DGRAD = 4, EP_DGRAD_UP2 = 5, EP_BN_FUSED = 6, EP_DGRAD_BN = 7 };

struct GatherArgs {
  const float* A;
  const float* src;
  const float* src2;
  float* out;
  float* out2;
  const float* bias;
  const float* bn_g;
  const float* bn_b;
  const float* bn_m;
  const float* bn_v;
  float* stats;
  int Mg, Kg, groups, Kc, src_ctotal, SRCH, SRCW, OUTH, OUTW, Npix;
  int KH, KW, SH, SW, PH, PW;
  int bcast, a_vec, ep;
  int batch;
  int splitk, k_per_split;
  float* part;
  size_t part_stride;
  float slope, eps;
};

struct WgradArgs {
  const float* dyr;
  const float* src;
  const float* src2;
  float* out;
  int Cog, Cig, Kg, groups, src_ctotal, H, W, OH, OW, Npix;
  int KH, KW, SH, SW, PH, PW;
  int bcast, splits, r_per_split;
  int accumulate;
};
constexpr int WG_MAX_JOBS = 24;
struct WgradBatch {
  int n;
  int block_end[WG_MAX_JOBS];
  WgradArgs job[WG_MAX_JOBS];
};

struct TimingScope {
  TimingScope(hipStream_t s, double flops, double bytes, const char* fmt, ...);
  ~TimingScope();
  bool skip() const { return skip_; }
  int idx_;
  hipStream_t s_;
  bool skip_;
};

struct PatchArgs {
  const float* A;
  const float* src;
  const float* src2;
  float* out;
  const float* bias;
  const float* bn_g;
  const float* bn_b;
  const float* bn_m;
  const float* bn_v;
  float* stats;
  float* counts;
  int Mg, Kg, groups, Kc, bcast, a_vec, ep;
  int SRCH, SRCW, s_img, s_chan, s_row;
  int OUTH, OUTW, o_img, o_chan, o_row;
  int o_sh, o_sw, o_ry, o_rx;
  float* out2;
  int is_dgrad;
  int gx, gy, gz;
  int splitk, chunks_per_split;
  float* part;
  size_t part_stride;
  int PH, PW, tiles_x, tiles_y;
  float slope, eps;
  size_t src_elems, a_elems;
  int ncls, cls_PH[4], cls_PW[4], cls_OUTH[4], cls_OUTW[4], cls_ry[4], cls_rx[4];
  unsigned cls_a_stride;
  int cls_fast;
  const unsigned short* Aplanes;
  unsigned plane_stride;
  int a_row_elems;
};
struct PatchPlan { int ok, tm, tw, tiles_y, tiles_x, n_tiles, splitk, chunks_per_split, tn, wm, ksi, p6, tile; };
PatchPlan plan_patch(int nd, int Mg, int groups, int Kc, int KH, int KW, int SH, int SW, int B, int OH, int OW, int zmul = 1, int in_w = 0);
extern int g_conv_tile;
bool conv_tile_shape_ok(int KH, int KW, int S);
int launch_tile(const PatchArgs& a, const PatchPlan& pl, int KH, int KW, int S, double flops, double bytes, hipStream_t s);
int patch_chunk_channels(int KH, int KW);
bool patch_dgrad_direct_ok(const float* w, int Cin_g, int KH, int KW, int SH, int SW, bool up2_or_bcast);
int launch_patch(const PatchArgs& a, const PatchPlan& pl, int KH, int KW, int S, bool up2, double flops, double bytes,
                 hipStream_t s);

bool conv_c1_ok(int groups, int Cin, int Cout, int KH, int KW, int SH, int SW, int PH, int PW, int H, int in_plain);
int conv_c1_tiles(int B, int H, int W);
bool wgrad_c1_ok(int groups, int Cin, int Cout, int KH, int KW, int SH, int SW, int PH, int PW, int H, int W, int in_plain);
int wgrad_c1_splits(int B, int H);
int launch_wgrad_c1(const float* dyr, const float* x, float* part, int B, int H, int W, hipStream_t s);
int launch_conv_c1(const float* x, const float* w, const float* bias, float* out, const float* bn_g, const float* bn_b,
                   const float* bn_m, const float* bn_v, float* stats, float* counts, int B, int H, int W, int ep, float slope,
                   float eps, hipStream_t s);
extern int g_patch_intra;
extern int g_precision;
bool patch6_supported(int KH, int KW, int S);
int patch6_row_elems(int Kc, int KH, int KW);
int launch_split_weights(const float* w, unsigned short* planes, int rows, int Kc, int KH, int KW, hipStream_t s);
struct SplitJob {
  const float* w;
  unsigned short* planes;
  int rows, Kc, KHW, CK, row_elems, block_end;
};
enum { SPLIT_BATCH_MAX = 64 };
struct SplitBatch { int n; SplitJob job[SPLIT_BATCH_MAX]; };
int launch_split_weights_multi(SplitBatch& sb, hipStream_t s);
int launch_patch6(const PatchArgs& a, const PatchPlan& pl, int KH, int KW, int S, bool up2, double flops, double bytes,
                  hipStream_t s);
extern int g_patch_min_wgs;

struct WgradPatchArgs {
  const float* dyr;
  const float* src;
  const float* src2;
  float* out;
  int Cog, Cig, Kg, groups, bcast;
  int SRCH, SRCW, s_img, s_chan, s_row, PH, PW;
  int OUTH, OUTW, o_img, o_chan, o_row;
  int tiles_x, tiles_y, n_tiles, tiles_per_split, splits;
  int gx, gy, gz;
  int accumulate;
  int n_steps, steps_per_split;
  int wave_kind;
  int KH, KW, w4, nx4, xrp, xcp, xbuf;
  int* counters;
  float* final_out;
};
struct WgradPatchPlan { int ok, tw, tiles_y, tiles_x, n_tiles, splits, tiles_per_split, p6, wave; };
constexpr int WGP_MAX_JOBS = 48;
struct WgradPatchBatch {
  int n;
  int block_end[WGP_MAX_JOBS];
  WgradPatchArgs job[WGP_MAX_JOBS];
};
int queue_wgrad_patch(const WgradPatchArgs& a, const WgradPatchPlan& pl, int KH, int KW, int S, bool up2, double flops, double bytes);
int wgrad_patch_flush(hipStream_t s);
void wgrad_patch_discard();
bool wgrad6_supported(int KH, int KW, int S);
int launch_wgrad_patch6(const WgradPatchArgs& a, const WgradPatchPlan& pl, int KH, int KW, int S, bool up2, double flops,
                        double bytes, hipStream_t s);
WgradPatchPlan plan_wgrad_patch(int nd, int Cog, int Kg, int groups, int KH, int KW, int SH, int SW, int B, int OH, int OW, int W = 0,
                                bool up2 = false);
int launch_wgrad_patch(const WgradPatchArgs& a, const WgradPatchPlan& pl, int KH, int KW, int S, bool up2, double flops,
                       double bytes, hipStream_t s);
int launch_reduce_splits(const float* part, float* out, int n, int splits, hipStream_t s);

struct Clip32Args;
bool clip32_fwd_ok(const ms_conv_desc* d);
bool clip32_dgrad_ok(const ms_conv_desc* d);
size_t clip32_fwd_weight_bytes(const ms_conv_desc* d);
size_t clip32_dgrad_weight_floats(const ms_conv_desc* d);
size_t clip32_weight_floats(int rows, int red, int KW);
int clip32_prep_queue(const float* w, float* out, int rows, int red, int KW, int transposed, int w_cols, hipStream_t s);
int clip32_prep_flush(hipStream_t s);
void clip32_prep_discard();
void gdgrad32_prep_discard();
struct PrepQueueGuard { ~PrepQueueGuard() { clip32_prep_discard(); gdgrad32_prep_discard(); } };
size_t clip32_part_bytes(int rows, int npw);
int clip32_sync_words(int rows);
int clip32_block_fwd(const ms_conv_desc* d, const float* x, const float* x2, const float* wp, const float* bias, const float* gamma,
                     const float* beta, float* rm, float* rv, float* y_raw, float* y, float* save, float* part, int* sync,
                     int sync_words, hipStream_t s);
struct Clip32PrevBN { const float* y; const float* y_raw; const float* save; const float* gamma; float* dgamma; float* dbeta; float* dbias; float slope; };
size_t clip32_dgrad_bn_part_bytes(const ms_conv_desc* d);
bool clip32_dgrad_bn_ok(const ms_conv_desc* d);
int clip32_block_dgrad(const ms_conv_desc* d, const float* g, const float* wp, float* dx, float* dx2, hipStream_t s,
                       const Clip32PrevBN* pv = nullptr, float* part = nullptr, int* sync = nullptr, int sync_words = 0,
                       const float* accum = nullptr);

bool gdgrad32_ok(const ms_conv_desc* d);
size_t gdgrad32_weight_floats(const ms_conv_desc* d);
int gdgrad32_prepare(const ms_conv_desc* d, const float* w, float* out, hipStream_t s);
int gdgrad32_prep_flush(hipStream_t s);
int gdgrad32_launch(const ms_conv_desc* d, const float* g, const float* wp, float* dx, hipStream_t s);

int chain32_supported(const ms_chain_desc* d);
size_t chain32_prepared_bytes(const ms_chain_desc* d);
size_t chain32_workspace(const ms_chain_desc* d);
int chain32_sync_words(const ms_chain_desc* d);
int chain32_prepare(const ms_chain_desc* d, const float* const* w, const float* wl, void* prepared, hipStream_t s);
int chain32_fwd(const ms_chain_desc* d, const ms_chain_tensors* tn, void* workspace, size_t workspace_bytes, hipStream_t s);
int chain16_supported(const ms_chain_desc* d);
size_t chain16_prepared_bytes(const ms_chain_desc* d);
size_t chain16_workspace(const ms_chain_desc* d);
int chain16_sync_words(const ms_chain_desc* d);
int chain16_prepare(const ms_chain_desc* d, const float* const* w, const float* wl, void* prepared, hipStream_t s);
int chain16_fwd(const ms_chain_desc* d, const ms_chain_tensors* tn, void* workspace, size_t workspace_bytes, hipStream_t s);
constexpr int CHAIN_EVAL_TILE = 64, CHAIN_EVAL_HALO = 4, CHAIN_EVAL_STEP = CHAIN_EVAL_TILE - 2 * CHAIN_EVAL_HALO, CHAIN_EVAL_FILL = 256,
              CHAIN_EVAL_MAX_PARTS = 2048;
struct ChainEvalPlan { int n_tiles, gpw, ngw; long units; };
ChainEvalPlan chain_eval_plan(const ms_chain_desc* d);
int chain_eval_shape_ok(const ms_chain_desc* d);
size_t chain_eval_workspace(const ms_chain_desc* d);
int chain_eval_sync_words(const ms_chain_desc* d);
int chain16_eval_fwd(const ms_chain_desc* d, const ms_chain_tensors* tn, void* workspace, size_t workspace_bytes, hipStream_t s);

struct GatherPlan { int tm, tn, splitk, k_per_split, n_tiles; };
GatherPlan plan_gather(int Mg, int npix, int zcount, int Kg);
int launch_gather(GatherArgs a, bool transposed, bool up2, const GatherPlan& plan, hipStream_t s);
int launch_splitk_fwd_epilogue(const float* part, int splitk, size_t part_stride, const float* bias, const float* gamma,
                               const float* beta, float* rm, float* rv, float* y_raw, float* y, float* save, int B, int C,
                               int HW, int ep, float slope, float eps, float momentum, hipStream_t s, int sg = 1);
int launch_splitk_dgrad_epilogue(const float* part, int splitk, size_t part_stride, float* dx, float* dx2, size_t n, int W,
                                 int up2, hipStream_t s);
int wgrad_splits(int Cog, int Kg, int groups, int Npix);
int launch_wgrad(WgradArgs a, bool up2, float* dw, float* partial_ws, bool defer_reduce, hipStream_t s, bool queue = false);
int wgrad_gather_flush(hipStream_t s);
void wgrad_gather_discard();
struct ReduceJob {
  const float* part;
  float* out;
  int n, splits, wave, block_end;
};
enum { REDUCE_BATCH_MAX = 96 };
struct ReduceBatch { int n; ReduceJob job[REDUCE_BATCH_MAX]; };
int launch_reduce_splits_multi(ReduceBatch& rb, hipStream_t s);
struct TransposeJob {
  const float* w;
  float* wt;
  int groups, Cog, Cig, KH, KW, SH, SW, PH, PW, flip;
  int block_end;
};
enum { TRANSPOSE_BATCH_MAX = 48 };
struct TransposeBatch { int n; TransposeJob job[TRANSPOSE_BATCH_MAX]; };
int launch_transpose_weight_multi(TransposeBatch& tb, hipStream_t s);
int launch_transpose_weight(const float* w, float* wt, int groups, int Cog, int Cig, int KH, int KW, int SH, int SW,
                            int PH, int PW, int flip, hipStream_t s);
size_t dgrad_weight_elems(int groups, int Cog, int Cig, int KH, int KW, int SH, int SW);
int launch_bn_finalize(const float* stats, const float* counts, int n_tiles, int tile_n, int N, int C, const float* gamma,
                       const float* beta, float* rm, float* rv, float* save, float eps, float momentum, hipStream_t s);
int launch_bn_apply(const float* y_raw, float* y, const float* save, int C, int HW, size_t total, float slope, hipStream_t s);
int launch_bn_finalize_apply(const float* stats, const float* counts, int n_tiles, int tile_n, int N, int C, const float* gamma,
                             const float* beta, float* rm, float* rv, float* save, float eps, float momentum, const float* y_raw,
                             float* y, int B, int HW, float slope, hipStream_t s);
int bwd_chunks(int B, int C, int* b_per_chunk);
constexpr int BN_BWD32_FUSED_MAX = 256 * 16;
int launch_bn_bwd(const float* dy, const float* y_raw, const float* y, const float* save, const float* gamma, float* partial, float* dyr,
                  float* colpart, float* dbias, float* dgamma, float* dbeta, int B, int C, int HW, float slope, int* fused,
                  hipStream_t s, int sg = 1);
int launch_act_bwd(const float* dy, const float* y, float* dyr, float* colpart, float* dbias, int B, int C, int HW, int mode, float slope, int* fused,
                   hipStream_t s);
int launch_colsum_finalize(const float* colpart, float* out, int B, int C, hipStream_t s);

}
```

### mix_stage_amd/joint_late_cluster_soft_style.py

```python
import contextlib

import torch
import torch.nn as nn

from . import ops, ops16
from .layers import (AudioEncoder, ClusterClassify, ConvNormRelu, Curriculum, EmbLin, Group, PoseEncoder,
                     PoseStyleEncoder, TextEncoder1D, UNet1D, bare_conv)
from .speech2gesture import Speech2Gesture_D

JointLateClusterSoftStyle4_D = Speech2Gesture_D


@contextlib.contextmanager
def some_grad(model):
  flags = [(p, p.requires_grad) for p in model.parameters()]
  for p, _ in flags:
    p.requires_grad_(False)
  try:
    yield
  finally:
    for p, f in flags:
      p.requires_grad_(f)


class JointLateClusterSoftStyle4_G(nn.Module):

  def __init__(self, time_steps=64, in_channels=256, out_feats=104, p=0, num_clusters=8, cluster=None,
               style_dict={}, style_dim=10, lambda_id=1, train_only=0, softmax=1, argmax=0, some_grad_flag=False,
               **kwargs):
    super().__init__()
    self.num_clusters = num_clusters
    self.audio_encoder = AudioEncoder(output_feats=time_steps, p=p)
    self.style_dict = style_dict
    self.style_dim = style_dim
    self.lambda_id = lambda_id
    self.train_only = train_only
    self.softmax = softmax
    self.argmax = argmax
    self.some_grad_flag = some_grad_flag
    self.out_feats = out_feats

    text_key = None
    for key in kwargs['shape']:
      if key in ['text/w2v', 'text/bert']:
        text_key = key
    if text_key:
      self.text_encoder = TextEncoder1D(output_feats=time_steps, input_channels=kwargs['shape'][text_key][-1], p=p)
    else:
      self.text_encoder = TextEncoder1D(output_feats=time_steps, p=p)
    self.pose_encoder = PoseEncoder(output_feats=time_steps, input_channels=out_feats, p=p)
    self.unet = UNet1D(input_channels=in_channels, output_channels=in_channels, p=p, groups=1)

    self.pose_style_encoder = PoseStyleEncoder(input_channels=out_feats, p=p, num_speakers=len(self.style_dict))
    self.style_emb = EmbLin(num_embeddings=len(self.style_dict), embedding_dim=self.style_dim)
    self.style_dec = nn.Sequential(*nn.ModuleList([ConvNormRelu(in_channels, in_channels, type='1d', leaky=True,
                                                                downsample=False, p=p, groups=self.style_dim)
                                                   for i in range(2)]))
    self.style_dec_gr = Group([self.style_dec], groups=self.style_dim)

    decoder_list = nn.ModuleList()
    decoder_list.append(ConvNormRelu(self.style_dim + in_channels, in_channels, type='1d', leaky=True,
                                     downsample=False, p=p, groups=self.num_clusters))
    decoder_list += nn.ModuleList([ConvNormRelu(in_channels, in_channels, type='1d', leaky=True, downsample=False,
                                                p=p, groups=self.num_clusters) for i in range(3)])
    self.decoder = nn.Sequential(*decoder_list)
    self.concat_encoder = nn.Sequential(*nn.ModuleList([ConvNormRelu(512, 256, type='1d', leaky=True,
                                                                     downsample=False, p=p)]))
    self.logits = nn.Conv1d(in_channels * self.num_clusters, out_feats * self.num_clusters, kernel_size=1, stride=1,
                            groups=self.num_clusters)
    self.classify_cluster = ClusterClassify(num_clusters=self.num_clusters, groups=1,
                                            input_channels=self.style_dim + in_channels)
    self.classify_loss = nn.CrossEntropyLoss()
    self.eye = nn.Parameter(torch.eye(self.num_clusters, self.num_clusters), requires_grad=False)
    self.smoothen = ConvNormRelu(out_feats, out_feats, type='1d', leaky=True, downsample=False, p=p)
    self.cluster = cluster

    self.thresh = Curriculum(0, 1, 1000)
    self.labels_cap_soft = None

  def index_select_outputs(self, x, labels, groups):
    from .layers import Group
    return Group.mix_groups(x, labels, groups)

  def forward(self, x, y, time_steps=None, **kwargs):
    internal_losses = []
    labels = x[-1]
    x = list(x[:-1])

    if torch.rand(1).item() > self.thresh.step(self.training) and self.training:
      x = self.pose_encoder(y, time_steps)
    else:
      for i, modality in enumerate(kwargs['input_modalities']):
        if modality.split('/')[0] == 'text':
          x[i] = self.text_encoder(x[i], time_steps)
        if modality.split('/')[0] == 'audio':
          if x[i].dim() == 3:
            x[i] = x[i].unsqueeze(dim=1)
          x[i] = self.audio_encoder(x[i], time_steps)
      if len(x) >= 2:
        x = self.concat_encoder[0](torch.cat(tuple(x), dim=1))
      else:
        x = x[0]

    dt = getattr(self, '_ms_dt', 0)
    if dt:
      x = ops16.to_cb8(x, dt)
    x = self.unet(x)
    x = ops.backward_marker(x)
    B, T = x.shape[0], x.shape[2]

    style = kwargs['style']
    pose_style_encoder_flag = not kwargs['sample_flag'] and (kwargs['description'] == 'train' or not self.train_only)
    if pose_style_encoder_flag:
      mode = 'lin'
      pose_style_score = self.pose_style_encoder(y)
      style_id = style[:, 0].contiguous()
      id_in_loss = ops.cross_entropy(pose_style_score, style_id, scale=self.lambda_id)
      if self.softmax:
        pose_style = torch.softmax(pose_style_score, dim=-1)
        if self.argmax:
          pose_style = torch.argmax(pose_style, dim=-1).unsqueeze(1).expand(B, T)
          mode = 'emb'
        else:
          pose_style = pose_style.unsqueeze(1).expand(B, T, pose_style.shape[-1])
      else:
        pose_style = pose_style_score.unsqueeze(1).expand(B, T, pose_style_score.shape[-1])
    else:
      pose_style = style
      if len(style.shape) == 2:
        mode = 'emb'
      elif len(style.shape) == 3:
        mode = 'lin'
      id_in_loss = torch.zeros(1)[0]
    if mode == 'emb' and pose_style.dim() == 2 and pose_style.shape != (B, T) and pose_style.numel() == B * T:
      pose_style = pose_style.reshape(B, T)
    if dt:
      x = ops16.from_cb8(x, self.unet.conv2[-1].conv.weight.shape[0])
    if mode == 'emb' and pose_style.dim() == 2 and pose_style.shape[1] == T:
      self.pose_style_ids = pose_style
      x = ops.concat_style(x, self.style_emb.emb.weight, pose_style)
    else:
      labels_style = self.style_emb(pose_style, mode=mode)
      if labels_style.shape[1] != T:
        labels_style = labels_style.view(B, -1, labels_style.shape[-1])
      x = torch.cat([x, labels_style.transpose(2, 1)], dim=1)

    if dt:
      x = ops16.to_cb8(x, dt)
    labels_score = self.classify_cluster(x)
    internal_losses.append(ops.cross_entropy(labels_score, labels, layout='bct'))

    chained = (ops16.decoder_chain16 if dt else ops.decoder_chain)(x, list(self.decoder), self.logits, labels_score, self.out_feats)
    if chained is not None:
      x, self.labels_cap_soft = chained
    else:
      z = self.decoder[0].forward_broadcast(x)
      for m in list(self.decoder)[1:]:
        z = m(z)
      z = bare_conv(self.logits, z, out_f32=True)
      x, self.labels_cap_soft = ops.softmax_mix(z, labels_score, self.out_feats)

    if pose_style_encoder_flag:
      if self.some_grad_flag:
        with some_grad(self.pose_style_encoder):
          pose_style_score_out = self.pose_style_encoder(x)
      else:
        pose_style_score_out = self.pose_style_encoder(x)
      id_out_loss = ops.cross_entropy(pose_style_score_out, style_id, scale=self.lambda_id)
    else:
      id_out_loss = torch.zeros(1)[0]

    internal_losses.append(id_in_loss if pose_style_encoder_flag else id_in_loss * self.lambda_id)
    internal_losses.append(id_out_loss if pose_style_encoder_flag else id_out_loss * self.lambda_id)
    return x, internal_losses
```

### mix_stage_amd/layers.py

```python
import torch
import torch.nn as nn

from . import ops, ops16
from ._lib import MS_BARE, MS_BN_EVAL, MS_BN_TRAIN, MS_IN_BCAST, MS_IN_PLAIN, MS_IN_UP2ADD, MS_LRELU


def set_compute_dtype(module, dtype):
  code = 0 if dtype in (None, 'fp32', 'f32', 'float32', torch.float32) else (
      ops16.MS_DT[dtype] if isinstance(dtype, torch.dtype) else ops16.NAME_DT[dtype])
  for m in module.modules():
    m._ms_dt = code
  return module


def set_inference_folding(module, on=True):
  for m in module.modules():
    if isinstance(m, ConvNormRelu):
      m._bn_folded = bool(on)
  return module


def compute_dtype(module):
  return getattr(module, '_ms_dt', 0)


_train_tape = None


def set_train_tape(tape):
  global _train_tape
  _train_tape = tape


def num_powers_of_two(x):
  n = 0
  while x > 1 and x % 2 == 0:
    x //= 2
    n += 1
  return n


def next_multiple_power_of_two(x, power=5):
  have = num_powers_of_two(x)
  return x * (2 ** (power - have)) if have < power else x


def _default_padding(kernel_size, stride):
  kt, st = isinstance(kernel_size, tuple), isinstance(stride, tuple)
  if not kt and st:
    return tuple(int((kernel_size - s) / 2) for s in stride)
  if kt and not st:
    return tuple(int((k - stride) / 2) for k in kernel_size)
  if kt and st:
    assert len(kernel_size) == len(stride), \
        'dims in kernel_size are {} and stride are {}. They must be the same'.format(len(kernel_size), len(stride))
    return tuple(0 for _ in kernel_size)
  return int((kernel_size - stride) / 2)


def bare_conv(conv, x, lrelu_slope=None, out_f32=False):
  geom = getattr(conv, '_ms_geom', None)
  if geom is None:
    nd = 1 if isinstance(conv, nn.Conv1d) else 2
    geom = ops.ConvGeom(nd, conv.groups, conv.kernel_size, conv.stride, conv.padding,
                        slope=0.0 if lrelu_slope is None else lrelu_slope)
    conv._ms_geom = geom
  mode = MS_BARE if lrelu_slope is None else MS_LRELU
  dt = getattr(conv, '_ms_dt', 0)
  if dt:
    was_plain = not ops16.is_cb8(x)
    if was_plain:
      x = ops16.to_cb8(x, dt)
    y = ops16.conv_block16(x, conv.weight, conv.bias, geom, mode, out_f32=out_f32)
    return ops16.from_cb8(y, conv.weight.shape[0]) if (was_plain and not out_f32) else y
  return ops.conv_block(x, conv.weight, conv.bias, geom, mode)


class ConvNormRelu(nn.Module):
  def __init__(self, in_channels, out_channels, type='1d', leaky=False, downsample=False, kernel_size=None,
               stride=None, padding=None, p=0, groups=1):
    super(ConvNormRelu, self).__init__()
    if kernel_size is None and stride is None:
      kernel_size, stride = (4, 2) if downsample else (3, 1)
    if padding is None:
      padding = _default_padding(kernel_size, stride)
    in_channels, out_channels = in_channels * groups, out_channels * groups
    if type == '1d':
      self.conv = nn.Conv1d(in_channels=in_channels, out_channels=out_channels, kernel_size=kernel_size,
                            stride=stride, padding=padding, groups=groups)
      self.norm = nn.BatchNorm1d(out_channels)
      self.dropout = nn.Dropout(p=p)
    elif type == '2d':
      self.conv = nn.Conv2d(in_channels=in_channels, out_channels=out_channels, kernel_size=kernel_size,
                            stride=stride, padding=padding, groups=groups)
      self.norm = nn.BatchNorm2d(out_channels)
      self.dropout = nn.Dropout2d(p=p)
    self.relu = nn.LeakyReLU(negative_slope=0.2) if leaky else nn.ReLU()
    self._nd = 1 if type == '1d' else 2
    self._slope = 0.2 if leaky else 0.0
    self._p = p
    self._geom = None
    self._pending_batches = 0
    self._register_state_dict_hook(ConvNormRelu._flush_hook)
    self._register_load_state_dict_pre_hook(self._reset_pending)

  @staticmethod
  def _flush_hook(module, state_dict, prefix, local_metadata):
    if module._pending_batches and module.norm.num_batches_tracked is not None:
      module.norm.num_batches_tracked += module._pending_batches
      module._pending_batches = 0
      state_dict[prefix + 'norm.num_batches_tracked'] = module.norm.num_batches_tracked.detach()

  def _reset_pending(self, *args, **kwargs):
    self._pending_batches = 0

  def _geometry(self):
    if self._geom is None:
      c, n = self.conv, self.norm
      self._geom = ops.ConvGeom(self._nd, c.groups, c.kernel_size, c.stride, c.padding, slope=self._slope,
                                eps=n.eps, momentum=0.1 if n.momentum is None else n.momentum)
    return self._geom

  def _note_train_pass(self):
    self._pending_batches += 1
    if _train_tape is not None:
      _train_tape.append(self)

  def _run(self, x, x2=None, in_mode=MS_IN_PLAIN, out_f32=False, chain_prev=False, link=None):
    if self._p and self.training:
      raise NotImplementedError('dropout p>0 is not on the Mix-StAGE path (p=0 everywhere, JL:26)')
    n = self.norm
    if self.training and n.track_running_stats:
      mode = MS_BN_TRAIN
      self._note_train_pass()
      if ops.stat_pair_active():
        self._note_train_pass()
    else:
      mode = MS_BN_EVAL
    dt = getattr(self, '_ms_dt', 0)
    if dt:
      was_plain = not ops16.is_cb8(x)
      if was_plain:
        x = ops16.to_cb8(x, dt)
        x2 = ops16.to_cb8(x2, dt) if x2 is not None else None
      if mode == MS_BN_TRAIN and ops.bn_sync_active():
        g = self._geometry()
        y_raw = ops16.conv_block16(x, self.conv.weight, self.conv.bias, g, MS_BARE, x2=x2, in_mode=in_mode, out_f32=True)
        y = ops.sync_bn_act(y_raw, n.weight, n.bias, n.running_mean, n.running_var, g.slope, g.eps, g.momentum)
        return y if (was_plain or out_f32) else ops16.to_cb8(y, dt)
      y = ops16.conv_block16(x, self.conv.weight, self.conv.bias, self._geometry(), mode, n.weight, n.bias, n.running_mean,
                             n.running_var, x2=x2, in_mode=in_mode, out_f32=out_f32,
                             bn_folded=getattr(self, '_bn_folded', False))
      return ops16.from_cb8(y, self.conv.weight.shape[0]) if (was_plain and not out_f32) else y
    if mode == MS_BN_TRAIN and ops.bn_sync_active():
      g = self._geometry()
      y_raw = ops.conv_block(x, self.conv.weight, self.conv.bias, g, MS_BARE, x2=x2, in_mode=in_mode)
      return ops.sync_bn_act(y_raw, n.weight, n.bias, n.running_mean, n.running_var, g.slope, g.eps, g.momentum)
    return ops.conv_block(x, self.conv.weight, self.conv.bias, self._geometry(), mode, n.weight, n.bias,
                          n.running_mean, n.running_var, x2=x2, in_mode=in_mode, chain_prev=chain_prev and mode == MS_BN_TRAIN,
                          link=link)

  def forward(self, x, **kwargs):
    residual = kwargs.get('_residual')
    out_f32 = bool(kwargs.get('_out_f32'))
    if residual is not None:
      return self._run(x, x2=residual, in_mode=MS_IN_UP2ADD, out_f32=out_f32, link=kwargs.get('_ms_link'))
    if kwargs.get('_broadcast'):
      return self._run(x, in_mode=MS_IN_BCAST, out_f32=out_f32)
    return self._run(x, out_f32=out_f32, chain_prev=bool(kwargs.get('_ms_chain')), link=kwargs.get('_ms_link'))

  def forward_upsample_add(self, a, residual, _ms_link=None):
    return self(a, _residual=residual, _ms_link=_ms_link)

  def forward_broadcast(self, x):
    return self(x, _broadcast=True)


def _hooked(*mods):
  import torch.nn.modules.module as M
  if (M._global_forward_hooks or M._global_forward_pre_hooks or M._global_backward_hooks or
      getattr(M, '_global_backward_pre_hooks', None) or getattr(M, '_global_forward_hooks_always_called', None)):
    return True
  for m in mods:
    if m._forward_hooks or m._forward_pre_hooks or m._backward_hooks or getattr(m, '_backward_pre_hooks', None):
      return True
  return False


def _chain_ok(stack, i):
  return i > 0 and not _hooked(stack[i - 1], stack[i])


class UNet1D(nn.Module):
  def __init__(self, input_channels, output_channels, max_depth=5, kernel_size=None, stride=None, p=0, groups=1):
    super(UNet1D, self).__init__()
    self.pre_downsampling_conv = nn.ModuleList([])
    self.conv1 = nn.ModuleList([])
    self.conv2 = nn.ModuleList([])
    self.upconv = nn.Upsample(scale_factor=2, mode='nearest')
    self.max_depth = max_depth
    self.groups = groups
    common = dict(type='1d', leaky=True, kernel_size=kernel_size, stride=stride, p=p, groups=groups)
    self.pre_downsampling_conv.append(ConvNormRelu(input_channels, output_channels, downsample=False, **common))
    self.pre_downsampling_conv.append(ConvNormRelu(output_channels, output_channels, downsample=False, **common))
    for _ in range(self.max_depth):
      self.conv1.append(ConvNormRelu(output_channels, output_channels, downsample=True, **common))
    for _ in range(self.max_depth):
      self.conv2.append(ConvNormRelu(output_channels, output_channels, downsample=False, **common))

  def forward(self, x, return_bottleneck=False):
    input_size = x.shape[2] if ops16.is_cb8(x) else x.shape[-1]
    assert input_size / (2 ** (self.max_depth - 1)) >= 1, \
        'Input size is {}. It must be >= {}'.format(input_size, 2 ** (self.max_depth - 1))
    assert num_powers_of_two(input_size) >= self.max_depth, \
        'Input size is {}. It must be a multiple of 2^(max_depth) = 2^{} = {}'.format(
            input_size, self.max_depth, 2 ** self.max_depth)
    dt = getattr(self, '_ms_dt', 0)
    was_plain = bool(dt) and not ops16.is_cb8(x)
    if was_plain:
      x = ops16.to_cb8(x, dt)
    channels = self.conv2[-1].conv.weight.shape[0]
    for i, m in enumerate(self.pre_downsampling_conv):
      x = m(x, _ms_chain=_chain_ok(self.pre_downsampling_conv, i))
    residuals = [x]
    links = []
    for i, down in enumerate(self.conv1):
      producer = self.conv1[i - 1] if i else self.pre_downsampling_conv[-1]
      up = self.conv2[self.max_depth - 1 - i]
      lk = ops.ResidualLink() if (not dt and torch.is_grad_enabled() and not _hooked(producer, down, up)) else None
      links.append(lk)
      x = down(x, _ms_link=(lk, 'consumer')) if lk is not None else down(x)
      if i < self.max_depth - 1:
        residuals.append(x)
    bn = x
    for i, up in enumerate(self.conv2):
      lk = links[self.max_depth - i - 1]
      x = up.forward_upsample_add(x, residuals[self.max_depth - i - 1], _ms_link=(lk, 'residual') if lk is not None else None)
    if was_plain:
      x, bn = ops16.from_cb8(x, channels), ops16.from_cb8(bn, channels)
    return (x, bn) if return_bottleneck else x


class AudioEncoder(nn.Module):

  def __init__(self, output_feats=64, input_channels=1, kernel_size=None, stride=None, p=0, groups=1):
    super(AudioEncoder, self).__init__()
    self.conv = nn.ModuleList([])
    common = dict(type='2d', leaky=True, kernel_size=kernel_size, stride=stride, p=p, groups=groups)
    for cin, cout, down in ((input_channels, 64, False), (64, 64, True), (64, 128, False), (128, 128, True),
                            (128, 256, False), (256, 256, True), (256, 256, False)):
      self.conv.append(ConvNormRelu(cin, cout, downsample=down, **common))
    self.conv.append(ConvNormRelu(256, 256, type='2d', leaky=True, downsample=False, kernel_size=(3, 8), stride=1,
                                  p=p, groups=groups))

  def forward(self, x, time_steps=None):
    if time_steps is None:
      time_steps = x.shape[-2]
    dt = getattr(self, '_ms_dt', 0)
    if dt:
      x = ops16.to_cb8(x, dt)
    for m in self.conv:
      x = m(x)
    if dt:
      x = ops16.from_cb8(x, self.conv[-1].conv.weight.shape[0])
    return ops.lerp_time(x, time_steps)


class _TimeMajorStack(nn.Module):

  def _build(self, specs, kernel_size, stride, p, groups):
    self.conv = nn.ModuleList([])
    for cin, cout, down in specs:
      self.conv.append(ConvNormRelu(cin, cout, type='1d', leaky=True, downsample=down, kernel_size=kernel_size,
                                    stride=stride, p=p, groups=groups))

  def _chain(self, x, last_f32=False):
    dt = getattr(self, '_ms_dt', 0)
    if dt:
      x = ops16.btc_to_cb8(x, dt)
      mods = list(self.conv)
      for m in mods[:-1]:
        x = m(x)
      if last_f32:
        return mods[-1](x, _out_f32=True)
      return ops16.from_cb8(mods[-1](x), mods[-1].conv.weight.shape[0])
    x = ops.to_channel_major(x)
    for i, m in enumerate(self.conv):
      x = m(x, _ms_chain=_chain_ok(self.conv, i))
    return x


def _same_res_specs(cin):
  return ((cin, 64, False), (64, 64, False), (64, 128, False), (128, 128, False), (128, 256, False),
          (256, 256, False))


class PoseEncoder(_TimeMajorStack):

  def __init__(self, output_feats=64, input_channels=96, kernel_size=None, stride=None, p=0, groups=1):
    super(PoseEncoder, self).__init__()
    self._build(_same_res_specs(input_channels), kernel_size, stride, p, groups)

  def forward(self, x, time_steps=None):
    return self._chain(x).squeeze(dim=-1)


class TextEncoder1D(_TimeMajorStack):

  def __init__(self, output_feats=64, input_channels=300, kernel_size=None, stride=None, p=0, groups=1):
    super().__init__()
    self._build(_same_res_specs(input_channels), kernel_size, stride, p, groups)

  def forward(self, x, time_steps=None, **kwargs):
    return self._chain(x).squeeze(dim=-1)


class PoseStyleEncoder(_TimeMajorStack):

  def __init__(self, output_feats=64, input_channels=96, kernel_size=None, stride=None, p=0, groups=1,
               num_speakers=4):
    super().__init__()
    self._build(((input_channels, 64, False), (64, 64, True), (64, 128, True), (128, 128, True), (128, 256, True),
                 (256, 256, True), (256, num_speakers, True)), kernel_size, stride, p, groups)

  def forward(self, x, time_steps=None):
    x = self._chain(x, last_f32=True)
    x = x.mean(-1) if x.shape[-1] > 1 else x.squeeze(-1)
    return x.squeeze(dim=-1)


class ClusterClassify(nn.Module):

  def __init__(self, num_clusters=8, kernel_size=None, stride=None, p=0, groups=1, input_channels=256):
    super().__init__()
    self.conv = nn.ModuleList()
    common = dict(type='1d', leaky=True, downsample=False, kernel_size=kernel_size, stride=stride, p=p, groups=groups)
    self.conv.append(ConvNormRelu(input_channels, 256, **common))
    self.conv += nn.ModuleList([ConvNormRelu(256, 256, **common) for i in range(5)])
    self.logits = nn.Conv1d(256 * groups, num_clusters * groups, kernel_size=1, stride=1, groups=groups)

  def forward(self, x, time_steps=None):
    dt = getattr(self, '_ms_dt', 0)
    if dt and not ops16.is_cb8(x):
      x = ops16.to_cb8(x, dt)
    for i, m in enumerate(self.conv):
      x = m(x, _ms_chain=_chain_ok(self.conv, i))
    return bare_conv(self.logits, x, out_f32=True)


class Group(nn.Module):

  def __init__(self, models, groups=1, dim=1):
    super().__init__()
    if not isinstance(models, list):
      models = [models]
    self.models = nn.ModuleList(models)
    self.groups = groups
    self.dim = dim

  @staticmethod
  def mix_groups(z, weights, groups):
    B, C, T = z.shape
    w = weights.reshape(B, T, groups)
    return torch.einsum('bgft,btg->btf', z.reshape(B, groups, C // groups, T), w)

  def index_select_outputs(self, x, labels):
    return self.mix_groups(x, labels, self.groups)

  def forward(self, x, labels=None, transpose=True, **kwargs):
    if self.dim == 0:
      self.groups = len(x)
    if isinstance(x, (list, tuple)):
      x = torch.cat(list(x), dim=self.dim)
    if transpose:
      x = x.transpose(-1, -2)
    for model in self.models:
      x = model(x, **kwargs) if kwargs else model(x)
    if labels is not None:
      return self.mix_groups(x, labels, self.groups).transpose(-1, -2)
    return list(torch.chunk(x, self.groups, dim=self.dim % x.dim()))


class EmbLin(nn.Module):
  def __init__(self, num_embeddings, embedding_dim):
    super().__init__()
    self.num_embeddings = num_embeddings
    self.embedding_dim = embedding_dim
    self.emb = nn.Embedding(num_embeddings, embedding_dim)

  def forward(self, x, mode='lin'):
    if mode == 'lin':
      return x.matmul(self.emb.weight)
    elif mode == 'emb':
      return torch.nn.functional.embedding(x, self.emb.weight)


class Curriculum():
  def __init__(self, start, end, num_iters):
    self.start = start
    self.end = end
    self.num_iters = num_iters
    self.iters = 0
    self.diff = (end - start) / num_iters
    self.value = start

  def step(self, flag=True):
    if not flag:
      return self.value
    if self.iters >= self.num_iters:
      return self.end
    previous = self.value
    self.value += self.diff
    self.iters += 1
    return previous
```

### mix_stage_amd/ops.py

```python
import contextlib
import ctypes
import os

import torch

from . import _lib
from ._lib import (BwdOptions, ConvDesc, FwdOptions, MS_BARE, MS_BN_EVAL, MS_BN_TRAIN, MS_DT_STAT_PAIR, MS_IN_BCAST, MS_IN_PLAIN,
                   MS_IN_UP2ADD, MS_LRELU, check, lib)

_vp = ctypes.c_void_p


def _ptr(t):
  return None if t is None else _vp(t.data_ptr())


def _stream():
  return _vp(torch.cuda.current_stream().cuda_stream)


def _need_hip(*tensors):
  for t in tensors:
    if t is None:
      continue
    if not t.is_cuda:
      raise _lib.MixStageLibError('mix_stage_amd ops run on the MI355X only (got a %s tensor); there is no CPU '
                                  'fallback' % t.device)
    if t.is_floating_point() and t.dtype != torch.float32:
      raise TypeError('the HIP path computes in float32 (got %s); call .float() on the model and inputs' % t.dtype)


_workspaces = {}
_counters = {}
USE_IN_LAUNCH_SPLIT_REDUCTION = False


def _ensure_counters(device):
  key = (device.type, device.index)
  if key not in _counters:
    buf = torch.zeros(1 << 16, dtype=torch.int32, device=device)
    check(lib().ms_set_counter_buffer(_ptr(buf), buf.numel()), 'ms_set_counter_buffer')
    _counters[key] = buf
  return _counters[key]



def workspace(nbytes, device):
  key = (device.type, device.index, torch.cuda.current_stream(device).cuda_stream)
  if USE_IN_LAUNCH_SPLIT_REDUCTION:
    _ensure_counters(device)
  ws = _workspaces.get(key)
  if ws is None or ws.numel() < nbytes:
    size = max(int(nbytes * 1.5), 1 << 22)
    if ws is not None:
      _retired_workspaces.append(ws)
    ws = torch.empty(size, dtype=torch.uint8, device=device)
    _workspaces[key] = ws
  return ws


_retired_workspaces = []


_side_workspaces = {}


def side_workspace(nbytes, device):
  key = (device.type, device.index)
  ws = _side_workspaces.get(key)
  if ws is None or ws.numel() < nbytes:
    ws = torch.empty(max(int(nbytes * 1.5), 1 << 22), dtype=torch.uint8, device=device)
    _side_workspaces[key] = ws
  return ws


_overlap = {'stream': None, 'keep': []}


def set_backward_overlap(side_stream):
  _overlap['stream'] = side_stream
  _overlap['keep'].clear()


def join_backward_overlap():
  side = _overlap['stream']
  if side is not None:
    torch.cuda.current_stream().wait_stream(side)
  _overlap['keep'].clear()


_prepared = {'on': False, 'entries': {}, 'by_storage': {}}


def enable_prepared_weights(on):
  _prepared['on'] = bool(on)
  if not on:
    _prepared['entries'].clear()
    _prepared['by_storage'].clear()


def _prepare_entries(entries):
  entries = [e for e in entries if e['n']]
  if not entries:
    return
  L = lib()
  tune = L.ms_tuning_epoch()
  e16 = [e for e in entries if e['kind'].endswith('16')]
  if e16:
    from . import ops16
    ops16._prepare16(e16)
  for e in entries:
    if e['kind'] == 'chain32':
      wl = (ctypes.c_void_p * 4)(*[x.data_ptr() for x in e['ws'][:4]])
      check(L.ms_decoder_chain_prepare(ctypes.byref(e['d']), wl, _ptr(e['ws'][4]), _ptr(e['wt']), _stream()), 'ms_decoder_chain_prepare')
      e['version'], e['tune'] = sum(x._version for x in e['ws']), tune
  for kind, fn in (('dgrad', L.ms_dgrad_weights_prepare), ('fwd', L.ms_fwd_weights_prepare)):
    es = [e for e in entries if e['kind'] == kind]
    if not es:
      continue
    n = len(es)
    descs = (ConvDesc * n)(*[e['d'] for e in es])
    ws = (ctypes.c_void_p * n)(*[e['w'].data_ptr() for e in es])
    outs = (ctypes.c_void_p * n)(*[e['wt'].data_ptr() for e in es])
    check(fn(n, descs, ws, outs, _stream()), 'ms_%s_weights_prepare' % kind)
    for e in es:
      e['version'], e['tune'] = e['w']._version, tune


def _prepared_for(w, d, kind='dgrad'):
  if not _prepared['on']:
    return None
  L = lib()
  key = (w.data_ptr(), id(d), kind)
  tune = L.ms_tuning_epoch()
  e = _prepared['entries'].get(key)
  if e is None or e['tune'] != tune:
    if kind == 'dgrad':
      n = L.ms_dgrad_weights_elems(ctypes.byref(d), _ptr(w))
    else:
      n = (L.ms_fwd_weights_bytes(ctypes.byref(d)) + 3) // 4
    if e is None:
      e = dict(w=w, d=d, n=0, wt=None, version=-1, tune=-1, kind=kind)
      _prepared['entries'][key] = e
      _prepared['by_storage'].setdefault(w.untyped_storage().data_ptr(), []).append(e)
    if n != e['n']:
      e['n'], e['wt'] = n, (torch.empty(n, dtype=torch.float32, device=w.device) if n else None)
    e['version'] = -1
    if not n:
      e['tune'] = tune
  if not e['n']:
    return None
  if e['version'] != w._version or e['tune'] != tune:
    _prepare_entries([e])
  return e['wt']


def drop_trainer_caches(storage_ptrs):
  for sp in storage_ptrs:
    for e in _prepared['by_storage'].pop(sp, ()):
      _prepared['entries'] = {k: v for k, v in _prepared['entries'].items() if v is not e}
  _deferred['bufs'] = {k: v for k, v in _deferred['bufs'].items() if v[2] not in storage_ptrs}


def refresh_prepared_weights(flat_params, start=0):
  if _prepared['on']:
    _prepare_entries(_prepared['by_storage'].get(flat_params.untyped_storage().data_ptr(), ())[start:])


def prepared_count(flat_params):
  return len(_prepared['by_storage'].get(flat_params.untyped_storage().data_ptr(), ()))


_deferred = {'on': False, 'jobs': [], 'queued': False, 'bufs': {}, 'keep': [], 'launches': 0}
DEFER_WGRAD_LAUNCH = os.environ.get('MS_DEFER_WGRAD_LAUNCH', '1') != '0'


def enable_deferred_wgrad(on):
  _deferred['on'] = bool(on)
  lib().ms_set_wgrad_batched(1 if (on and DEFER_WGRAD_LAUNCH) else 0, int(os.environ.get('MS_WGRAD_TPS', '0')))
  reset_deferred_wgrad()
  if not on:
    _deferred['bufs'].clear()


def reset_deferred_wgrad():
  _deferred['jobs'].clear()
  _deferred['keep'].clear()
  _deferred['queued'] = False
  if _deferred['launches']:
    _deferred['launches'] = 0
    lib().ms_wgrad_discard()


def _queue_deferred_flush():
  owner = (torch.cuda.current_device(), _stream().value)
  if not _deferred['queued']:
    _deferred['queued'] = True
    _deferred['owner'] = owner
    torch.autograd.Variable._execution_engine.queue_callback(_flush_deferred_wgrad)
  elif _deferred.get('owner') != owner:
    raise _lib.MixStageLibError('deferred weight-gradient work was queued from two devices or streams in one backward pass '
# ... 32 lines not shown
  rounds, seen = [], {}
  for j in jobs:
    k = seen.get(j[1].data_ptr(), 0)
    seen[j[1].data_ptr()] = k + 1
    if k == len(rounds):
      rounds.append([])
    rounds[k].append(j)
  try:
    for rj in rounds:
      n = len(rj)
      parts = (ctypes.c_void_p * n)(*[j[0].data_ptr() for j in rj])
      outs = (ctypes.c_void_p * n)(*[j[1].data_ptr() for j in rj])
      elems = (ctypes.c_int * n)(*[j[1].numel() for j in rj])
      splits = (ctypes.c_int * n)(*[j[2] for j in rj])
      check(lib().ms_wgrad_reduce_multi(n, parts, outs, elems, splits, _stream()), 'ms_wgrad_reduce_multi')
  finally:
    jobs.clear()


class ConvGeom:
  __slots__ = ('nd', 'groups', 'KH', 'KW', 'SH', 'SW', 'PH', 'PW', 'slope', 'eps', 'momentum', '_cache')

  def __init__(self, nd, groups, kernel, stride, padding, slope=0.2, eps=1e-5, momentum=0.1):
    def two(v):
      if isinstance(v, (tuple, list)):
        return (1, int(v[0])) if len(v) == 1 else (int(v[0]), int(v[1]))
      return (int(v), int(v)) if nd == 2 else (1, int(v))
    self.nd, self.groups = nd, groups
    self.KH, self.KW = two(kernel)
    self.SH, self.SW = two(stride)
    ph, pw = two(padding)
    self.PH, self.PW = (ph, pw) if nd == 2 else (0, pw)
    if nd == 1:
      self.KH, self.SH = 1, 1
    self.slope, self.eps, self.momentum = float(slope), float(eps), float(momentum)
    self._cache = {}

  def desc(self, B, Cin_g, H, W, Cout_g, mode, in_mode, dtype=0):
    key = (B, Cin_g, H, W, Cout_g, mode, in_mode, dtype)
    d = self._cache.get(key)
    if d is None:
      OH = (H + 2 * self.PH - self.KH) // self.SH + 1
      OW = (W + 2 * self.PW - self.KW) // self.SW + 1
      if OH < 1 or OW < 1:
        raise RuntimeError('conv block: input (%d,%d) too small for kernel (%d,%d)' % (H, W, self.KH, self.KW))
      d = ConvDesc(B, Cin_g, H, W, Cout_g, self.groups, self.KH, self.KW, self.SH, self.SW, self.PH, self.PW,
                   OH, OW, mode, in_mode, self.slope, self.eps, self.momentum, dtype)
      d._tune = -1
      self._cache[key] = d
    L = lib()
    tune = L.ms_tuning_epoch()
    if d._tune != tune:
      d._fwd_ws = L.ms_conv_block_fwd_workspace(ctypes.byref(d))
      d._bwd_ws = L.ms_conv_block_bwd_workspace(ctypes.byref(d))
      d._tune = tune
    return d


_stat_pair = {'on': False}


@contextlib.contextmanager
def stat_pair():
  old = _stat_pair['on']
  _stat_pair['on'] = True
  try:
    yield
  finally:
    _stat_pair['on'] = old


def stat_pair_active():
  return _stat_pair['on']


def stat_pair_ok(geom, B2, Cin_g, W, Cout_g, mode, dtype=0):
  d = geom.desc(B2, Cin_g, 1, W, Cout_g, mode, MS_IN_PLAIN, dtype | MS_DT_STAT_PAIR)
  return bool(lib().ms_stat_pair_ok(ctypes.byref(d))), d.OW


LATE = 'late'


def _grad_slot(param, shape_like):
  slot = getattr(param, '_ms_grad_slot', None) if param is not None else None
  if slot is not None and torch.is_grad_enabled() is False:
    if getattr(param, '_ms_grad_fresh', False):
      param._ms_grad_fresh = False
      return slot, True
    if _deferred['on']:
      tmp = torch.empty_like(slot)
      _deferred['jobs'].append((tmp, slot, 1))
      _queue_deferred_flush()
      return tmp, LATE
  return torch.empty_like(shape_like), False


_link_stats = {'in_launch': 0}


class ResidualLink:
  __slots__ = ('armed', 'grad', 'taken')

  def __init__(self):
    self.armed, self.grad, self.taken = False, None, False


class _ConvBlockFn(torch.autograd.Function):
  @staticmethod
  def forward(ctx, x, x2, w, bias, gamma, beta, geom, mode, in_mode, stats, pre=None, prev=None, link=None):
    rm, rv = stats if stats is not None else (None, None)
    _need_hip(x, x2, w, bias, gamma, beta, rm, rv)
    x = x.contiguous()
    x2 = x2.contiguous() if x2 is not None else None
    nd = geom.nd
    if x.dim() != nd + 2:
      raise RuntimeError('conv block expects a %d-D input, got %s' % (nd + 2, tuple(x.shape)))
    B = x.shape[0]
    ref = x2 if in_mode == MS_IN_UP2ADD else x
    H, W = (ref.shape[2], ref.shape[3]) if nd == 2 else (1, ref.shape[2])
    ctot = w.shape[0]
    Cout_g = ctot // geom.groups
    Cin_g = w.shape[1]
    exp_c = Cin_g if in_mode == MS_IN_BCAST else Cin_g * geom.groups
    if x.shape[1] != exp_c:
      raise RuntimeError('conv block: expected %d input channels, got %d' % (exp_c, x.shape[1]))
    if in_mode == MS_IN_UP2ADD and (x.shape[2] * 2 != W or x2.shape[1] != exp_c):
      raise RuntimeError('UP2ADD: a %s and residual %s do not match' % (tuple(x.shape), tuple(x2.shape)))
    pair = MS_DT_STAT_PAIR if (_stat_pair['on'] and pre is None) else 0
    d = geom.desc(B, Cin_g, H, W, Cout_g, mode, in_mode, pair)
    oshape = (B, ctot, d.OH, d.OW) if nd == 2 else (B, ctot, d.OW)
    if pre is not None:
      y_raw, y, save = pre
      if tuple(y.shape) != oshape:
        raise RuntimeError('precomputed block output has shape %s, expected %s' % (tuple(y.shape), oshape))
    else:
      y = torch.empty(oshape, dtype=torch.float32, device=x.device)
      y_raw = save = None
      if mode == MS_BN_TRAIN:
        y_raw = torch.empty_like(y)
        save = torch.empty((8 if pair else 4) * ctot, dtype=torch.float32, device=x.device)
    ws = workspace(d._fwd_ws, x.device) if pre is None else None
    planes = _prepared_for(w, d, 'fwd') if pre is None else None
    if pre is None:
      sync = None
      if mode == MS_BN_TRAIN and nd == 1:
        from . import ops16
        sync = ops16.block_sync(x.device, d)
      opt = FwdOptions(planes.data_ptr() if planes is not None else None, sync.data_ptr() if sync is not None else None,
                       sync.numel() if sync is not None else 0)
      check(lib().ms_conv_block_fwd_ex(ctypes.byref(d), _ptr(x), _ptr(x2), _ptr(w), _ptr(bias), _ptr(gamma), _ptr(beta),
                                       _ptr(rm), _ptr(rv), _ptr(y_raw), _ptr(y), _ptr(save), _ptr(ws), ws.numel(),
                                       _stream(), ctypes.byref(opt)), 'ms_conv_block_fwd_ex')
    ctx.geom_desc = d
    ctx.mode, ctx.in_mode = mode, in_mode
    ctx.prev = None
    ctx.dy_is_dyr = False
    if prev is not None and pre is None and in_mode == MS_IN_PLAIN and nd == 1 and getattr(prev, 'mode', None) == MS_BN_TRAIN \
        and not bn_sync_active() and lib().ms_dgrad_fuses_prev_bn(ctypes.byref(d)):
      from . import ops16
      py = prev.saved_tensors[5]
      watched = bool(getattr(x, '_backward_hooks', None)) or bool(getattr(x, 'retains_grad', False))
      if ops16.in_launch_meetings() and not watched and py is not None and py.data_ptr() == x.data_ptr() and tuple(py.shape) == tuple(x.shape):
        ctx.prev = prev
    ctx.link = None
    if link is not None and pre is None and nd == 1 and not bn_sync_active():
      lk, role = link
      if role == 'consumer' and in_mode == MS_IN_PLAIN and x.requires_grad and lib().ms_dgrad_takes_accum(ctypes.byref(d)) \
          and not (getattr(x, '_backward_hooks', None) or getattr(x, 'retains_grad', False)):
        lk.armed = True
        ctx.link = link
      elif role == 'residual' and in_mode == MS_IN_UP2ADD and lk.armed:
        ctx.link = link
    ctx.has_bias = bias is not None
    ctx.params = (w, bias, gamma, beta)
    ctx.save_for_backward(x, x2, w, gamma, y_raw, y if mode in (MS_LRELU, MS_BN_TRAIN) else None, save)
    return y

  @staticmethod
  def backward(ctx, dy):
    x, x2, w, gamma, y_raw, y, save = ctx.saved_tensors
    d, mode, in_mode = ctx.geom_desc, ctx.mode, ctx.in_mode
    if mode == MS_BN_EVAL:
      raise RuntimeError('backward through an eval-mode (running-stats) ConvNormRelu is not on the path')
    need_x, need_x2, need_w = ctx.needs_input_grad[0], ctx.needs_input_grad[1], ctx.needs_input_grad[2]
    need_bn = mode == MS_BN_TRAIN and ctx.needs_input_grad[4]
    dy = dy.contiguous()
    dev = dy.device
    is_dyr = bool(ctx.dy_is_dyr)
    ctx.dy_is_dyr = False
    dyr = torch.empty_like(dy) if (mode != MS_BARE and not is_dyr) else None
    up2 = in_mode == MS_IN_UP2ADD
    want_dx = need_x or (up2 and need_x2)
    dx = torch.empty_like(x) if want_dx else None
    dx2 = torch.empty_like(x2) if (want_dx and up2) else None
    pw, pbias, pgamma, pbeta = ctx.params
    dw = dbias = dgamma = dbeta = None
    direct_w = direct_b = direct_g = direct_be = False
    if need_w:
      dw, direct_w = _grad_slot(pw, w)
      if ctx.has_bias and not is_dyr:
        dbias, direct_b = _grad_slot(pbias, pbias)
    if need_bn and not is_dyr:
      dgamma, direct_g = _grad_slot(pgamma, gamma)
      dbeta, direct_be = _grad_slot(pbeta, gamma)
    if is_dyr:
      direct_b = direct_g = direct_be = True
    fuse = None
    prev = ctx.prev
    if prev is not None and want_dx and not up2 and _overlap['stream'] is None and not torch.is_grad_enabled():
      ppw, ppbias, ppgamma, ppbeta = prev.params
      p_need_w, p_need_bn = prev.needs_input_grad[2], prev.needs_input_grad[4]
      wanted = ([ppbias] if (p_need_w and prev.has_bias) else []) + ([ppgamma, ppbeta] if p_need_bn else [])
      if all(getattr(q, '_ms_grad_slot', None) is not None and (getattr(q, '_ms_grad_fresh', False) or _deferred['on']) for q in wanted):
        _, _, _, pgam_t, py_raw, py, psave = prev.saved_tensors
        if py_raw is not None and py is not None and psave is not None:
          from . import ops16
          sync = ops16.block_sync(dev, d, tag='dgrad_bn')
          if sync is not None:
            pdb = _grad_slot(ppbias, ppbias)[0] if (p_need_w and prev.has_bias) else None
            pdg = _grad_slot(ppgamma, pgam_t)[0] if p_need_bn else None
            pdbe = _grad_slot(ppbeta, pgam_t)[0] if p_need_bn else None
            fuse = (py, py_raw, psave, pgam_t, pdg, pdbe, pdb, sync, float(prev.geom_desc.slope))
    acc = None
    if ctx.link is not None and ctx.link[1] == 'consumer':
      acc, ctx.link[0].grad = ctx.link[0].grad, None
      ctx.link[0].taken = True
      if acc is not None and (not want_dx or tuple(acc.shape) != tuple(x.shape)):
        raise RuntimeError('residual link: a residual gradient of shape %s arrived for an input of shape %s (needs grad: %s)' %
                           (tuple(acc.shape), tuple(x.shape), want_dx))
    acc_in_launch = False
    ws = workspace(d._bwd_ws, dev)
    side = _overlap['stream']
    if side is not None and need_w and direct_w is not True:
      torch.cuda.current_stream().wait_stream(side)
    if side is not None and direct_w is True and (dbias is None or direct_b is True):
      ws2 = side_workspace(d._bwd_ws, dev)
      _overlap['keep'].append((x, x2, dy, dyr))
      check(lib().ms_conv_block_bwd_overlap(ctypes.byref(d), _ptr(x), _ptr(x2), _ptr(w), _ptr(gamma), None, None,
                                            _ptr(y_raw), _ptr(y), _ptr(save), _ptr(dy), _ptr(dyr), _ptr(dx), _ptr(dx2),
                                            _ptr(dw), _ptr(dbias), _ptr(dgamma), _ptr(dbeta), _ptr(ws), ws.numel(),
                                            _stream(), _vp(side.cuda_stream), _ptr(ws2), ws2.numel()),
            'ms_conv_block_bwd_overlap')
    else:
      wt = _prepared_for(w, d) if want_dx else None
      part, nsplit = (None, 1)
      if _deferred['on'] and direct_w is True:
        part, nsplit = _wgrad_partials_for(w, d)
      defer_launch = bool(_deferred['on'] and direct_w is True and dw is not None and DEFER_WGRAD_LAUNCH)
      if wt is not None or part is not None or defer_launch or fuse is not None or is_dyr or acc is not None:
        opt = BwdOptions(None, None, 0, wt.data_ptr() if wt is not None else None,
                         part.data_ptr() if part is not None else None, 1 if defer_launch else 0)
        if acc is not None:
          acc = acc.contiguous()
          opt.dx_accum = acc.data_ptr()
          acc_in_launch = True
          _link_stats['in_launch'] += 1
        if fuse is not None:
          py, py_raw, psave, pgam_t, pdg, pdbe, pdb, sync, pslope = fuse
          opt.prev_y, opt.prev_y_raw, opt.prev_save, opt.prev_gamma = py.data_ptr(), py_raw.data_ptr(), psave.data_ptr(), pgam_t.data_ptr()
          opt.prev_dgamma = pdg.data_ptr() if pdg is not None else None
          opt.prev_dbeta = pdbe.data_ptr() if pdbe is not None else None
          opt.prev_dbias = pdb.data_ptr() if pdb is not None else None
          opt.prev_slope, opt.bn_sync, opt.bn_sync_words = pslope, sync.data_ptr(), sync.numel()
          prev.dy_is_dyr = True
        opt.dy_is_dyr = 1 if is_dyr else 0
        check(lib().ms_conv_block_bwd_ex(ctypes.byref(d), _ptr(x), _ptr(x2), _ptr(w), _ptr(gamma), None, None, _ptr(y_raw),
                                         _ptr(y), _ptr(save), _ptr(dy), _ptr(dyr), _ptr(dx), _ptr(dx2), _ptr(dw),
                                         _ptr(dbias), _ptr(dgamma), _ptr(dbeta), _ptr(ws), ws.numel(), _stream(),
                                         ctypes.byref(opt)), 'ms_conv_block_bwd_ex')
        if defer_launch:
          _deferred['launches'] += 1
          _deferred['keep'].append((x, x2, dy, dyr, dw, part))
          _queue_deferred_flush()
        if part is not None:
          _deferred['jobs'].append((part, dw, nsplit))
          _queue_deferred_flush()
      else:
        check(lib().ms_conv_block_bwd(ctypes.byref(d), _ptr(x), _ptr(x2), _ptr(w), _ptr(gamma), None, None, _ptr(y_raw),
                                      _ptr(y), _ptr(save), _ptr(dy), _ptr(dyr), _ptr(dx), _ptr(dx2), _ptr(dw),
                                      _ptr(dbias), _ptr(dgamma), _ptr(dbeta), _ptr(ws), ws.numel(), _stream()),
              'ms_conv_block_bwd')
    if acc is not None and not acc_in_launch:
      dx.add_(acc)
    if ctx.link is not None and ctx.link[1] == 'residual' and dx2 is not None and ctx.needs_input_grad[1] and not ctx.link[0].taken:
      ctx.link[0].grad = dx2
      dx2 = None
    return (dx, dx2, None if direct_w else dw, None if direct_b else dbias, None if direct_g else dgamma,
            None if direct_be else dbeta, None, None, None, None, None, None, None)


def _f32(t):
  return t.float() if isinstance(t, torch.Tensor) and t.dtype == torch.float64 else t


def _bridge64(fn):
  def wrapped(*args, **kw):
    vals = list(args) + list(kw.values())
    if not any(isinstance(a, torch.Tensor) and a.dtype == torch.float64 for a in vals):
      return fn(*args, **kw)
    out = fn(*[_f32(a) for a in args], **{k: _f32(v) for k, v in kw.items()})
    back = lambda o: o.double() if isinstance(o, torch.Tensor) and o.dtype == torch.float32 else o
    return tuple(back(o) for o in out) if isinstance(out, tuple) else back(out)
  wrapped.__doc__, wrapped.__name__ = fn.__doc__, fn.__name__
  return wrapped


_chain_fusion = {'on': os.environ.get('MS_CHAIN_BN', '1') != '0'}


def enable_chain_fusion(on):
  old = _chain_fusion['on']
  _chain_fusion['on'] = bool(on)
  return old


def conv_block(x, w, bias, geom, mode, gamma=None, beta=None, running_mean=None, running_var=None, x2=None,
               in_mode=MS_IN_PLAIN, chain_prev=False, link=None):
  if w.dtype == torch.float64 or x.dtype == torch.float64:
    rm32, rv32 = _f32(running_mean), _f32(running_var)
    stats = (rm32, rv32) if rm32 is not None else None
    y = _ConvBlockFn.apply(_f32(x), _f32(x2), _f32(w), _f32(bias), _f32(gamma), _f32(beta), geom, mode, in_mode, stats)
    if mode == MS_BN_TRAIN and running_mean is not None and running_mean.dtype == torch.float64:
      with torch.no_grad():
        running_mean.copy_(rm32)
        running_var.copy_(rv32)
    return y.double()
  stats = (running_mean, running_var) if running_mean is not None else None
  prev = x.grad_fn if (chain_prev and _chain_fusion['on'] and x.grad_fn is not None and type(x.grad_fn).__name__ == '_ConvBlockFnBackward') else None
  return _ConvBlockFn.apply(x, x2, w, bias, gamma, beta, geom, mode, in_mode, stats, None, prev,
                            link if (link is not None and _chain_fusion['on'] and torch.is_grad_enabled()) else None)


_marker = {'cb': None}


def set_backward_marker(callback):
  _marker['cb'] = callback


class _BackwardMarkerFn(torch.autograd.Function):
  @staticmethod
  def forward(ctx, x):
    return x.view_as(x)

  @staticmethod
  def backward(ctx, g):
    cb = _marker['cb']
    if cb is not None:
      cb()
    return g


def backward_marker(x):
  return _BackwardMarkerFn.apply(x) if (_marker['cb'] is not None and x.requires_grad) else x


_bn_sync = {'group': None, 'on': False}


def set_bn_sync(on, process_group=None):
  _bn_sync['on'], _bn_sync['group'] = bool(on), process_group


def bn_sync_active():
  import torch.distributed as dist
  return _bn_sync['on'] and dist.is_available() and dist.is_initialized() and dist.get_world_size(_bn_sync['group']) > 1


class _SyncBNActFn(torch.autograd.Function):
  @staticmethod
  def forward(ctx, y_raw, gamma, beta, rm, rv, slope, eps, momentum):
    import torch.distributed as dist
    _need_hip(y_raw, gamma, beta, rm, rv)
    y_raw = y_raw.contiguous()
    B, C = y_raw.shape[0], y_raw.shape[1]
    HW = y_raw.numel() // (B * C)
    group = _bn_sync['group']
    world = dist.get_world_size(group)
    stats = torch.empty((C, 2), dtype=torch.float32, device=y_raw.device)
    check(lib().ms_bn_stats(_ptr(y_raw), _ptr(stats), B, C, HW, _stream()), 'ms_bn_stats')
    allstats = torch.empty((world, C, 2), dtype=torch.float32, device=y_raw.device)
    dist.all_gather_into_tensor(allstats, stats, group=group) if dist.get_backend(group) == 'nccl' else \
        allstats.copy_(torch.stack(_all_gather_list(stats, world, group)))
    y = torch.empty_like(y_raw)
    save = torch.empty(4 * C, dtype=torch.float32, device=y_raw.device)
    check(lib().ms_bn_train_apply(_ptr(allstats), world, B * HW, _ptr(gamma), _ptr(beta), _ptr(rm), _ptr(rv), _ptr(y_raw),
                                  _ptr(y), _ptr(save), B, C, HW, eps, momentum, slope, _stream()), 'ms_bn_train_apply')
    ctx.save_for_backward(y_raw, gamma, save)
    ctx.meta = (B, C, HW, slope, world, group)
    ctx.params = (gamma, beta)
    return y

  @staticmethod
  def backward(ctx, dy):
    import torch.distributed as dist
    y_raw, gamma, save = ctx.saved_tensors
    B, C, HW, slope, world, group = ctx.meta
    dy = dy.contiguous()
    sums = torch.empty((C, 2), dtype=torch.float32, device=dy.device)
    ws = workspace(lib().ms_bn_bwd_workspace(B, C), dy.device)
    check(lib().ms_bn_bwd_sums(_ptr(dy), _ptr(y_raw), _ptr(save), _ptr(sums), B, C, HW, slope, _ptr(ws), ws.numel(), _stream()),
          'ms_bn_bwd_sums')
    pgamma, pbeta = ctx.params
    dgamma, direct_g = _grad_slot(pgamma, gamma)
    dbeta, direct_b = _grad_slot(pbeta, gamma)
    dgamma.copy_(sums[:, 1]); dbeta.copy_(sums[:, 0])
    gsum = sums.clone()
    dist.all_reduce(gsum, op=dist.ReduceOp.SUM, group=group)
    dyr = torch.empty_like(dy)
    check(lib().ms_bn_bwd_apply(_ptr(dy), _ptr(y_raw), _ptr(save), _ptr(gamma), _ptr(gsum), float(world) * B * HW, _ptr(dyr), B, C,
                                HW, slope, _stream()), 'ms_bn_bwd_apply')
    return dyr, None if direct_g else dgamma, None if direct_b else dbeta, None, None, None, None, None


def _all_gather_list(t, world, group):
  import torch.distributed as dist
  out = [torch.empty_like(t) for _ in range(world)]
  dist.all_gather(out, t, group=group)
  return out


def sync_bn_act(y_raw, gamma, beta, running_mean, running_var, slope, eps, momentum):
  return _SyncBNActFn.apply(y_raw, gamma, beta, running_mean, running_var, float(slope), float(eps), float(momentum))


CHAIN_SYNC_FIRST_WORD = 32
USE_DECODER_CHAIN = os.environ.get('MS_DECODER_CHAIN', '1') != '0'
USE_DECODER_CHAIN_EVAL = os.environ.get('MS_CHAIN_EVAL', '1') != '0'


def _chain_desc(B, M, T, cin0, P, mode, blk, dtype=0):
  g = blk._geometry()
  return _lib.ChainDesc(B, M, T, cin0, 256, P, 4, mode, dtype, CHAIN_SYNC_FIRST_WORD, 0, g.slope, g.eps, g.momentum)


_chain_scratch = {}


def _chain_prepared(d, ws):
  key = (ws[0].data_ptr(), d.M, d.cin0, d.P, d.dtype, 'chain32')
  if not _prepared['on']:
    n = (lib().ms_decoder_chain_prepared_bytes(ctypes.byref(d)) + 3) // 4
    buf = _chain_scratch.get(key)
    if buf is None or buf.numel() != n:
      _chain_scratch.clear()
      buf = _chain_scratch[key] = torch.empty(n, dtype=torch.float32, device=ws[0].device)
    _prepare_entries([dict(w=ws[0], ws=list(ws), d=d, n=n, wt=buf, version=-1, tune=-1, kind='chain32')])
    return buf
  e = _prepared['entries'].get(key)
  if e is None:
    n = (lib().ms_decoder_chain_prepared_bytes(ctypes.byref(d)) + 3) // 4
    e = dict(w=ws[0], ws=list(ws), d=d, n=n, wt=torch.empty(n, dtype=torch.float32, device=ws[0].device), version=-1, tune=-1,
             kind='chain32')
    _prepared['entries'][key] = e
    _prepared['by_storage'].setdefault(ws[0].untyped_storage().data_ptr(), []).append(e)
  e['ws'] = list(ws)
  if e['version'] != sum(x._version for x in ws):
    _prepare_entries([e])
  return e['wt']


_chain_eval_sync = {}


def _chain_eval_launch(d, x, score, blocks, logits, ws, P):
  if not USE_DECODER_CHAIN_EVAL or not lib().ms_decoder_chain_eval_supported(ctypes.byref(d)):
    return None
  dev = x.device
  prepared = _chain_prepared(d, ws)
  words = lib().ms_decoder_chain_eval_sync_words(ctypes.byref(d))
  sync = None
  if words:
    key = (dev.type, dev.index, torch.cuda.current_stream(dev).cuda_stream, d.B, d.M, d.T)
    sync = _chain_eval_sync.get(key)
    if sync is None or sync.numel() < CHAIN_SYNC_FIRST_WORD + words:
      sync = _chain_eval_sync[key] = torch.zeros(CHAIN_SYNC_FIRST_WORD + words, dtype=torch.int32, device=dev)
  soft = torch.empty((d.B, d.T, d.M), dtype=torch.float32, device=dev)
  out = torch.empty((d.B, d.T, P), dtype=torch.float32, device=dev)
  tn = _lib.ChainTensors()
  tn.x, tn.score = x.data_ptr(), score.data_ptr()
  for l, m in enumerate(blocks):
    tn.w[l], tn.bias[l] = m.conv.weight.data_ptr(), (m.conv.bias.data_ptr() if m.conv.bias is not None else None)
    tn.gamma[l], tn.beta[l] = m.norm.weight.data_ptr(), m.norm.bias.data_ptr()
# ... 431 lines not shown
```

Baseline: 11110 clips/s.

## Co-run pose style encoder conv blocks with unet conv blocks in paired kernel launches

Adds a hold/flush mechanism so that a pose-style-encoder conv block's clip32 launch can be deferred and fused into a single paired kernel with a unet conv block. Each kernel's workgroups run side by side on otherwise idle CUs. A Python generator-driven co-run driver interleaves the encoder chain with the unet forward and offers each host block as a pairing partner when the combined grid fits on the device. The aim is to fill underused CUs and cut launch count. The cost is added host-side bookkeeping, held-tensor lifetimes, separate workspaces, and more complex ordering and error paths.

```diff
diff --git a/include/mixstage.h b/include/mixstage.h
--- a/include/mixstage.h
+++ b/include/mixstage.h
@@ -65,6 +65,11 @@
                          const float* bias, const float* gamma, const float* beta, float* running_mean,
                          float* running_var, float* y_raw, float* y, float* save, void* workspace,
                          size_t workspace_bytes, void* stream, const ms_fwd_options* opt);
+int ms_clip_hold(void* stream);
+int ms_clip_hold_flush(void* stream);
+int ms_clip_hold_discard(void* stream);
+int ms_clip_grid(const ms_conv_desc* d);
+int ms_clip_pair_ok(const ms_conv_desc* host, const ms_conv_desc* guest);
 size_t ms_fwd_weights_bytes(const ms_conv_desc* d);
 int ms_fwd_weights_prepare(int n, const ms_conv_desc* descs, const float* const* w, void* const* planes, void* stream);
 
diff --git a/include/mixstage_aux.h b/include/mixstage_aux.h
--- a/include/mixstage_aux.h
+++ b/include/mixstage_aux.h
@@ -35,6 +35,8 @@
 
 int ms_debug_set_clip32(int on);
 
+int ms_debug_set_clip_corun(int on);
+
 int ms_selftest_mfma(const float* A, const float* B, float* C, int K, void* stream);
 int ms_probe_peak(int kind, long iters, void* a, void* b, double* work, void* stream);
 
diff --git a/mix_stage_amd/_lib.py b/mix_stage_amd/_lib.py
--- a/mix_stage_amd/_lib.py
+++ b/mix_stage_amd/_lib.py
@@ -147,6 +147,12 @@
     'ms_debug_set_conv16_ring': (c_int, [c_int, c_int]),
     'ms_debug_set_skip': (c_int, [ctypes.c_char_p]),
     'ms_debug_set_clip32': (c_int, [c_int]),
+    'ms_debug_set_clip_corun': (c_int, [c_int]),
+    'ms_clip_hold': (c_int, [_P]),
+    'ms_clip_hold_flush': (c_int, [_P]),
+    'ms_clip_hold_discard': (c_int, [_P]),
+    'ms_clip_grid': (c_int, [_DESC]),
+    'ms_clip_pair_ok': (c_int, [_DESC, _DESC]),
     'ms_debug_set_wgrad16_target': (c_int, [c_int]),
     'ms_debug_set_wgrad16_ring': (c_int, [c_int]),
     'ms_debug_set_wgrad_target': (c_int, [c_int]),
diff --git a/mix_stage_amd/csrc/api.hip b/mix_stage_amd/csrc/api.hip
--- a/mix_stage_amd/csrc/api.hip
+++ b/mix_stage_amd/csrc/api.hip
@@ -161,10 +161,26 @@
                               workspace_bytes, stream, nullptr);
 }
 
+static int conv_block_fwd_impl(const ms_conv_desc* d, const float* x, const float* x2, const float* w, const float* bias,
+                               const float* gamma, const float* beta, float* running_mean, float* running_var, float* y_raw,
+                               float* y, float* save, void* workspace, size_t workspace_bytes, void* stream,
+                               const ms_fwd_options* opt);
+
 int ms_conv_block_fwd_ex(const ms_conv_desc* d, const float* x, const float* x2, const float* w, const float* bias,
                          const float* gamma, const float* beta, float* running_mean, float* running_var, float* y_raw,
                          float* y, float* save, void* workspace, size_t workspace_bytes, void* stream,
                          const ms_fwd_options* opt) {
+  const bool clip_path = d && dt_of(d) == DT_F32 && g_precision == 0 && !validate(d, "ms_conv_block_fwd") && clip32_fwd_ok(d);
+  int rc = clip32_fwd_call_begin((hipStream_t)stream, clip_path, workspace, workspace_bytes);
+  if (!rc) rc = conv_block_fwd_impl(d, x, x2, w, bias, gamma, beta, running_mean, running_var, y_raw, y, save, workspace, workspace_bytes, stream, opt);
+  clip32_fwd_call_end((hipStream_t)stream);
+  return rc;
+}
+
+static int conv_block_fwd_impl(const ms_conv_desc* d, const float* x, const float* x2, const float* w, const float* bias,
+                               const float* gamma, const float* beta, float* running_mean, float* running_var, float* y_raw,
+                               float* y, float* save, void* workspace, size_t workspace_bytes, void* stream,
+                               const ms_fwd_options* opt) {
   const unsigned short* w_planes = opt ? (const unsigned short*)opt->w_planes : nullptr;
   int rc = validate(d, "ms_conv_block_fwd");
   if (rc) return rc;
@@ -197,7 +213,8 @@
     rc = clip32_block_fwd(d, x, x2, wp, bias, gamma, beta, running_mean, running_var, y_raw, y, save, stats, opt ? opt->bn_sync : nullptr,
                           opt ? opt->bn_sync_words : 0, s);
     if (rc != -2) return rc;
-    rc = 0;
+    rc = clip32_hold_flush(s);
+    if (rc) return rc;
   }
 
   float* out = d->mode == MS_BN_TRAIN ? y_raw : y;
@@ -687,4 +704,21 @@
   return rc;
 }
 
-}
+int ms_clip_hold(void* stream) { return clip32_hold_arm((hipStream_t)stream); }
+int ms_clip_hold_flush(void* stream) { return clip32_hold_flush((hipStream_t)stream); }
+int ms_clip_hold_discard(void* stream) { clip32_hold_discard((hipStream_t)stream); return 0; }
+int ms_clip_grid(const ms_conv_desc* d) {
+  if (validate(d, "ms_clip_grid") || dt_of(d) != DT_F32 || g_precision != 0) return 0;
+  return clip32_fwd_grid(d);
+}
+int ms_clip_pair_ok(const ms_conv_desc* host, const ms_conv_desc* guest) {
+  if (validate(host, "ms_clip_pair_ok") || validate(guest, "ms_clip_pair_ok") || dt_of(host) != DT_F32 || dt_of(guest) != DT_F32 || g_precision != 0) return 0;
+  return clip32_fwd_pair_ok(host, guest) ? 1 : 0;
+}
+int ms_debug_set_clip_corun(int on) {
+  const int prev = g_clip_corun < 0 ? 1 : g_clip_corun;
+  g_clip_corun = on ? 1 : 0;
+  return prev;
+}
+
+}
diff --git a/mix_stage_amd/csrc/clip32.hip b/mix_stage_amd/csrc/clip32.hip
--- a/mix_stage_amd/csrc/clip32.hip
+++ b/mix_stage_amd/csrc/clip32.hip
@@ -2,6 +2,8 @@
 #include <stdlib.h>
 
 #include <algorithm>
+#include <map>
+#include <mutex>
 #include <vector>
 
 #include "kernels.h"
@@ -40,7 +42,7 @@
   int cx, px;
   unsigned long long* stamps;
 };
-#define CL_STAMP(k) do { if (p.stamps && threadIdx.x == 0) p.stamps[(size_t)blockIdx.x * 8 + (k)] = __builtin_amdgcn_s_memrealtime(); } while (0)
+#define CL_STAMP(k) do { if (p.stamps && threadIdx.x == 0) p.stamps[(size_t)bid * 8 + (k)] = __builtin_amdgcn_s_memrealtime(); } while (0)
 
 __host__ __device__ constexpr int cl_pslots(int n) { return (n + 3) & ~3; }
 template <bool SPLIT>
@@ -70,17 +72,16 @@
 }
 
 template <int KW, int S, int NB, bool UP2, int K8W, bool DG2 = false>
-__global__ __launch_bounds__(256, 1) void clip32_kernel(const Clip32Args p) {
-  prefetch_kernargs<sizeof(Clip32Args)>();
+__device__ __forceinline__ void clip32_body(const Clip32Args& p, const unsigned bid) {
   extern __shared__ float cl_smem[];
   CL_STAMP(0);
   constexpr int NPX = 32 * NB;
   constexpr int NWR = (K8W ? K8W : CL_MAXK8W) * KW;
   const int t = threadIdx.x, lane = t & 63, w = t >> 6, n0 = lane & 31, h = lane >> 5;
   const int nct = p.nct;
-  int ct = blockIdx.x % nct, pw = blockIdx.x / nct;
+  int ct = bid % nct, pw = bid / nct;
   if (p.cx) {
-    const int xcd = blockIdx.x & 7, j = blockIdx.x >> 3, tpx = nct / p.cx, ppx = p.npw / p.px;
+    const int xcd = bid & 7, j = bid >> 3, tpx = nct / p.cx, ppx = p.npw / p.px;
     const int xc = xcd % p.cx, xp = xcd / p.cx, jp = j / tpx;
     ct = xc * tpx + (j - jp * tpx);
     pw = xp * ppx + jp;
@@ -575,6 +576,28 @@
   CL_STAMP(7);
 }
 
+template <int KW, int S, int NB, bool UP2, int K8W, bool DG2 = false>
+__global__ __launch_bounds__(256, 1) void clip32_kernel(const Clip32Args p) {
+  prefetch_kernargs<sizeof(Clip32Args)>();
+  clip32_body<KW, S, NB, UP2, K8W, DG2>(p, blockIdx.x);
+}
+
+struct ClipPairArgs {
+  int nA;
+  Clip32Args a, b;
+};
+template <int KWA, int SA, int NBA, bool UP2A, int K8WA, int KWB, int SB, int NBB, bool UP2B, int K8WB>
+__global__ __launch_bounds__(256, 1) void clip32_pair_kernel(const ClipPairArgs pp) {
+  const unsigned bid = blockIdx.x;
+  if (bid < (unsigned)pp.nA) {
+    prefetch_kernargs<sizeof(Clip32Args)>();
+    clip32_body<KWA, SA, NBA, UP2A, K8WA>(pp.a, bid);
+  } else {
+    prefetch_kernargs<384>((int)offsetof(ClipPairArgs, b));
+    clip32_body<KWB, SB, NBB, UP2B, K8WB>(pp.b, bid - (unsigned)pp.nA);
+  }
+}
+
 struct ClipPrepJob {
   const float* w;
   float* out;
@@ -727,7 +750,181 @@
   }
 }
 
-int clip32_launch(Clip32Args a, int KW, int S, bool up2, const char* what, hipStream_t s, bool dg2 = false) {
+struct ClipJob {
+  Clip32Args a;
+  int KW, S, nb, nwg, lds;
+  bool up2, dg2;
+  const char* what;
+  double flops, bytes;
+};
+
+enum { CLIP_HOST_DOWN8 = 0, CLIP_HOST_UP8 = 1, CLIP_HOSTS = 2 };
+enum { CLIP_GUEST_K3_4 = 0, CLIP_GUEST_DOWN2 = 1, CLIP_GUEST_DOWN4 = 2, CLIP_GUEST_DOWN8 = 3, CLIP_GUESTS = 4 };
+static int clip_host_kind(const ClipJob& j) {
+  if (j.dg2 || j.a.k8w != 8) return -1;
+  if (j.KW == 4 && j.S == 2 && !j.up2) return CLIP_HOST_DOWN8;
+  if (j.KW == 3 && j.S == 1 && j.up2) return CLIP_HOST_UP8;
+  return -1;
+}
+static int clip_guest_kind(const ClipJob& j) {
+  if (j.dg2 || j.up2) return -1;
+  if (j.KW == 3 && j.S == 1) return j.a.k8w == 4 ? CLIP_GUEST_K3_4 : -1;
+  if (j.KW == 4 && j.S == 2) return j.a.k8w == 2 ? CLIP_GUEST_DOWN2 : j.a.k8w == 4 ? CLIP_GUEST_DOWN4 : j.a.k8w == 8 ? CLIP_GUEST_DOWN8 : -1;
+  return -1;
+}
+template <int KWA, int SA, int NBA, bool UP2A, int K8WA, int KWB, int SB, int NBB, bool UP2B, int K8WB>
+static int clip32_pair_launch_k(const ClipPairArgs& pp, int nwg, int lds_bytes, hipStream_t s) {
+  auto fn = clip32_pair_kernel<KWA, SA, NBA, UP2A, K8WA, KWB, SB, NBB, UP2B, K8WB>;
+  static unsigned long long attr_done = 0;
+  if (first_time_on_device(attr_done)) {
+    if (hipFuncSetAttribute(reinterpret_cast<const void*>(fn), hipFuncAttributeMaxDynamicSharedMemorySize, 160 * 1024) != hipSuccess)
+      return set_error("clip32: cannot raise the dynamic LDS limit");
+    done_on_device(attr_done);
+  }
+  hipLaunchKernelGGL(fn, dim3(nwg), dim3(256), lds_bytes, s, pp);
+  return check_launch("clip32_pair_kernel");
+}
+template <int KWA, int SA, int NBA, bool UP2A>
+static int clip32_pair_launch_g(int guest, const ClipPairArgs& pp, int nwg, int lds_bytes, hipStream_t s) {
+  switch (guest) {
+    case CLIP_GUEST_K3_4: return clip32_pair_launch_k<KWA, SA, NBA, UP2A, 8, 3, 1, 2, false, 4>(pp, nwg, lds_bytes, s);
+    case CLIP_GUEST_DOWN2: return clip32_pair_launch_k<KWA, SA, NBA, UP2A, 8, 4, 2, 1, false, 2>(pp, nwg, lds_bytes, s);
+    case CLIP_GUEST_DOWN4: return clip32_pair_launch_k<KWA, SA, NBA, UP2A, 8, 4, 2, 1, false, 4>(pp, nwg, lds_bytes, s);
+    default: return clip32_pair_launch_k<KWA, SA, NBA, UP2A, 8, 4, 2, 1, false, 8>(pp, nwg, lds_bytes, s);
+  }
+}
+
+static int clip32_issue(ClipJob& j, hipStream_t s) {
+  Clip32Args& a = j.a;
+  const int nwg = j.nwg;
+  TimingScope ts(s, j.flops, j.bytes, "clip32_kernel<%d,%d,%d,%d>|conv_%s_clip k1x%d s%d rows%d red%d T%d B%d ep%d", j.KW, j.S, j.nb, j.up2 ? 1 : 0, j.what,
+                 j.KW, j.S, a.rows_valid, a.Cin, a.To, a.B, a.ep);
+  if (ts.skip()) return 0;
+  static int dbg = -1;
+  if (dbg < 0) { const char* e = getenv("MS_CLIP_DBG"); dbg = e ? atoi(e) : 0; }
+  static unsigned long long* g_stamps = nullptr;
+  if (dbg & 32) {
+    if (!g_stamps && hipMalloc(&g_stamps, 4096 * 8 * 8) != hipSuccess) g_stamps = nullptr;
+    if (g_stamps) (void)hipMemsetAsync(g_stamps, 0, 4096 * 8 * 8, s);
+    a.stamps = nwg <= 4096 ? g_stamps : nullptr;
+  }
+  int rc;
+  if (j.dg2) rc = clip32_launch_t<4, 1, 2, false, true>(a, nwg, j.lds, s);
+  else if (j.KW == 3 && j.S == 1) rc = j.up2 ? clip32_launch_t<3, 1, 2, true>(a, nwg, j.lds, s) : clip32_launch_t<3, 1, 2, false>(a, nwg, j.lds, s);
+  else rc = clip32_launch_t<4, 2, 1, false>(a, nwg, j.lds, s);
+  if (a.stamps) {
+    std::vector<unsigned long long> h((size_t)nwg * 8);
+    if (hipStreamSynchronize(s) == hipSuccess && hipMemcpy(h.data(), g_stamps, h.size() * 8, hipMemcpyDeviceToHost) == hipSuccess) {
+      unsigned long long t0 = ~0ull;
+      for (int i = 0; i < nwg; ++i) t0 = std::min(t0, h[(size_t)i * 8]);
+      fprintf(stderr, "clip32 %s k%d s%d rows%d red%d ep%d: stamps (us after the first workgroup's entry; min / median / max over %d workgroups)\n", j.what, j.KW, j.S,
+              a.rows_valid, a.Cin, a.ep, nwg);
+      for (int k = 0; k < 8; ++k) {
+        std::vector<double> v;
+        for (int i = 0; i < nwg; ++i) if (h[(size_t)i * 8 + k]) v.push_back((double)(h[(size_t)i * 8 + k] - t0) * 0.01);
+        if (v.empty()) continue;
+        std::sort(v.begin(), v.end());
+        fprintf(stderr, "  stamp %d: %7.2f %7.2f %7.2f\n", k, v.front(), v[v.size() / 2], v.back());
+      }
+    }
+    a.stamps = nullptr;
+  }
+  return rc;
+}
+
+int g_clip_corun = -1;
+enum { HOLD_IDLE = 0, HOLD_ARMED = 1, HOLD_PENDING = 2 };
+struct ClipHold {
+  int state = HOLD_IDLE;
+  ClipJob job;
+  const char* ws_lo = nullptr;
+  const char* ws_hi = nullptr;
+};
+static std::mutex g_hold_mu;
+static std::map<hipStream_t, ClipHold> g_hold;
+static thread_local bool t_in_fwd = false;
+static thread_local const char* t_ws_lo = nullptr;
+static thread_local const char* t_ws_hi = nullptr;
+
+static bool clip_corun_on() {
+  if (g_clip_corun < 0) { const char* e = getenv("MS_CLIP_CORUN"); g_clip_corun = e ? (atoi(e) != 0) : 1; }
+  return g_clip_corun != 0;
+}
+
+int clip32_hold_arm(hipStream_t s) {
+  std::lock_guard<std::mutex> lk(g_hold_mu);
+  ClipHold& h = g_hold[s];
+  if (h.state == HOLD_PENDING) return set_error("ms_clip_hold: a held block is pending on this stream (flush or discard it first)");
+  h.state = HOLD_ARMED;
+  return 0;
+}
+void clip32_hold_discard(hipStream_t s) {
+  std::lock_guard<std::mutex> lk(g_hold_mu);
+  auto it = g_hold.find(s);
+  if (it != g_hold.end()) it->second.state = HOLD_IDLE;
+}
+int clip32_hold_flush(hipStream_t s) {
+  ClipJob job;
+  {
+    std::lock_guard<std::mutex> lk(g_hold_mu);
+    auto it = g_hold.find(s);
+    if (it == g_hold.end()) return 0;
+    const int st = it->second.state;
+    it->second.state = HOLD_IDLE;
+    if (st != HOLD_PENDING) return 0;
+    job = it->second.job;
+  }
+  return clip32_issue(job, s);
+}
+int clip32_fwd_call_begin(hipStream_t s, bool clip_path, const void* ws, size_t ws_bytes) {
+  t_in_fwd = true;
+  t_ws_lo = (const char*)ws; t_ws_hi = t_ws_lo + (ws ? ws_bytes : 0);
+  bool flush = false;
+  {
+    std::lock_guard<std::mutex> lk(g_hold_mu);
+    auto it = g_hold.find(s);
+    if (it != g_hold.end() && it->second.state == HOLD_PENDING)
+      flush = !clip_path || (t_ws_lo < it->second.ws_hi && it->second.ws_lo < t_ws_hi);
+  }
+  return flush ? clip32_hold_flush(s) : 0;
+}
+void clip32_fwd_call_end(hipStream_t s) {
+  t_in_fwd = false;
+  std::lock_guard<std::mutex> lk(g_hold_mu);
+  auto it = g_hold.find(s);
+  if (it != g_hold.end() && it->second.state == HOLD_ARMED) it->second.state = HOLD_IDLE;
+}
+
+static bool clip_pair_fits(const ClipJob& A, const ClipJob& B) {
+  if (!clip_corun_on()) return false;
+  if (clip_host_kind(A) < 0 || clip_guest_kind(B) < 0) return false;
+  if (A.nwg % 8) return false;
+  int cus = current_device_cus();
+  if (cus <= 0) cus = 256;
+  return A.nwg + B.nwg <= cus;
+}
+static bool clip_pair_ok(const ClipJob& A, const ClipJob& B) {
+  if (!clip_pair_fits(A, B)) return false;
+  const bool meetA = A.a.ep == EP_RAW_STATS && A.a.npw > 1, meetB = B.a.ep == EP_RAW_STATS && B.a.npw > 1;
+  if (meetA && meetB && (A.a.part == B.a.part || A.a.sync == B.a.sync)) return false;
+  return true;
+}
+static int clip32_issue_pair(ClipJob& A, ClipJob& B, hipStream_t s) {
+  char da[96], db[96];
+  snprintf(da, sizeof(da), "conv_%s_clip k1x%d s%d rows%d red%d T%d B%d ep%d", A.what, A.KW, A.S, A.a.rows_valid, A.a.Cin, A.a.To, A.a.B, A.a.ep);
+  snprintf(db, sizeof(db), "conv_%s_clip k1x%d s%d rows%d red%d T%d B%d ep%d", B.what, B.KW, B.S, B.a.rows_valid, B.a.Cin, B.a.To, B.a.B, B.a.ep);
+  TimingScope ts(s, A.flops + B.flops, A.bytes + B.bytes, "clip32_kernel<%d,%d,%d,%d>+<%d,%d,%d,%d>|%s + %s", A.KW, A.S, A.nb, A.up2 ? 1 : 0, B.KW, B.S,
+                 B.nb, B.up2 ? 1 : 0, da, db);
+  if (ts.skip()) return 0;
+  ClipPairArgs pp;
+  pp.nA = A.nwg; pp.a = A.a; pp.b = B.a;
+  pp.a.stamps = pp.b.stamps = nullptr;
+  const int nwg = A.nwg + B.nwg, lds = std::max(A.lds, B.lds), guest = clip_guest_kind(B);
+  return clip_host_kind(A) == CLIP_HOST_DOWN8 ? clip32_pair_launch_g<4, 2, 1, false>(guest, pp, nwg, lds, s)
+                                              : clip32_pair_launch_g<3, 1, 2, true>(guest, pp, nwg, lds, s);
+}
+
+int clip32_launch(Clip32Args a, int KW, int S, bool up2, const char* what, hipStream_t s, bool dg2 = false, ClipJob* plan = nullptr) {
   const int nb = (S == 2 && !dg2) ? 1 : 2, npx = 32 * nb;
   a.k8w = clip_k8w(a.Cin);
   a.npw = a.B * a.To / npx;
@@ -757,40 +954,54 @@
   cus = current_device_cus();
   if (!cus) cus = 256;
   if ((a.ep == EP_RAW_STATS || a.ep == EP_DGRAD_BN) && a.npw > 1 && nwg > cus) return -2;
-  const double flops = 2.0 * a.rows_valid * a.Cin * (dg2 ? 2 : KW) * (double)a.B * a.To;
-  const double bytes = 4.0 * ((double)a.rows_valid * a.Cin * KW + (double)a.B * a.Cin * a.Ti + (double)a.B * a.rows_valid * a.To);
-  TimingScope ts(s, flops, bytes, "clip32_kernel<%d,%d,%d,%d>|conv_%s_clip k1x%d s%d rows%d red%d T%d B%d ep%d", KW, S, nb, up2 ? 1 : 0, what, KW,
-                 S, a.rows_valid, a.Cin, a.To, a.B, a.ep);
-  if (ts.skip()) return 0;
-  static int dbg = -1;
-  if (dbg < 0) { const char* e = getenv("MS_CLIP_DBG"); dbg = e ? atoi(e) : 0; }
-  static unsigned long long* g_stamps = nullptr;
-  if (dbg & 32) {
-    if (!g_stamps && hipMalloc(&g_stamps, 4096 * 8 * 8) != hipSuccess) g_stamps = nullptr;
-    if (g_stamps) (void)hipMemsetAsync(g_stamps, 0, 4096 * 8 * 8, s);
-    a.stamps = nwg <= 4096 ? g_stamps : nullptr;
-  }
-  int rc;
-  if (dg2) rc = clip32_launch_t<4, 1, 2, false, true>(a, nwg, lds, s);
-  else if (KW == 3 && S == 1) rc = up2 ? clip32_launch_t<3, 1, 2, true>(a, nwg, lds, s) : clip32_launch_t<3, 1, 2, false>(a, nwg, lds, s);
-  else rc = clip32_launch_t<4, 2, 1, false>(a, nwg, lds, s);
-  if (a.stamps) {
-    std::vector<unsigned long long> h((size_t)nwg * 8);
-    if (hipStreamSynchronize(s) == hipSuccess && hipMemcpy(h.data(), g_stamps, h.size() * 8, hipMemcpyDeviceToHost) == hipSuccess) {
-      unsigned long long t0 = ~0ull;
-      for (int i = 0; i < nwg; ++i) t0 = std::min(t0, h[(size_t)i * 8]);
-      fprintf(stderr, "clip32 %s k%d s%d rows%d red%d ep%d: stamps (us after the first workgroup's entry; min / median / max over %d workgroups)\n", what, KW, S,
-              a.rows_valid, a.Cin, a.ep, nwg);
-      for (int k = 0; k < 8; ++k) {
-        std::vector<double> v;
-        for (int i = 0; i < nwg; ++i) if (h[(size_t)i * 8 + k]) v.push_back((double)(h[(size_t)i * 8 + k] - t0) * 0.01);
-        if (v.empty()) continue;
-        std::sort(v.begin(), v.end());
-        fprintf(stderr, "  stamp %d: %7.2f %7.2f %7.2f\n", k, v.front(), v[v.size() / 2], v.back());
-      }
-    }
-  }
-  return rc;
+  ClipJob job;
+  job.a = a; job.KW = KW; job.S = S; job.nb = nb; job.nwg = nwg; job.lds = lds; job.up2 = up2; job.dg2 = dg2; job.what = what;
+  job.flops = 2.0 * a.rows_valid * a.Cin * (dg2 ? 2 : KW) * (double)a.B * a.To;
+  job.bytes = 4.0 * ((double)a.rows_valid * a.Cin * KW + (double)a.B * a.Cin * a.Ti + (double)a.B * a.rows_valid * a.To);
+  if (plan) { *plan = job; return 0; }
+  if (t_in_fwd) {
+    ClipJob held;
+    int st;
+    {
+      std::lock_guard<std::mutex> lk(g_hold_mu);
+      auto it = g_hold.find(s);
+      st = it == g_hold.end() ? HOLD_IDLE : it->second.state;
+      if (st == HOLD_ARMED) {
+        it->second.state = HOLD_PENDING;
+        it->second.job = job;
+        it->second.ws_lo = t_ws_lo; it->second.ws_hi = t_ws_hi;
+      } else if (st == HOLD_PENDING) {
+        it->second.state = HOLD_IDLE;
+        held = it->second.job;
+      }
+    }
+    if (st == HOLD_ARMED) return 0;
+    if (st == HOLD_PENDING) {
+      if (clip_pair_ok(job, held)) return clip32_issue_pair(job, held, s);
+      const int rc = clip32_issue(held, s);
+      if (rc) return rc;
+    }
+  }
+  return clip32_issue(job, s);
+}
+
+static int clip32_fwd_plan(const ms_conv_desc* d, ClipJob* plan) {
+  if (!clip32_fwd_ok(d)) return 0;
+  Clip32Args a = {};
+  a.B = d->B; a.Cin = d->Cin; a.Cout = d->Cout; a.rows_valid = d->Cout; a.To = d->OW; a.Ti = d->W;
+  a.ep = d->mode == MS_BARE ? EP_BARE : d->mode == MS_LRELU ? EP_LRELU : d->mode == MS_BN_EVAL ? EP_BN_EVAL : EP_RAW_STATS;
+  a.sg = a.ep == EP_RAW_STATS ? sg_of(d) : 1;
+  plan->nwg = 0;
+  if (clip32_launch(a, d->KW, d->SW, d->in_mode == MS_IN_UP2ADD, "fwd", nullptr, false, plan) != 0) return 0;
+  return plan->nwg;
+}
+int clip32_fwd_grid(const ms_conv_desc* d) {
+  ClipJob plan;
+  return clip32_fwd_plan(d, &plan);
+}
+bool clip32_fwd_pair_ok(const ms_conv_desc* host, const ms_conv_desc* guest) {
+  ClipJob A, B;
+  return clip32_fwd_plan(host, &A) > 0 && clip32_fwd_plan(guest, &B) > 0 && clip_pair_fits(A, B);
 }
 
 int clip32_block_fwd(const ms_conv_desc* d, const float* x, const float* x2, const float* wp, const float* bias, const float* gamma,
diff --git a/mix_stage_amd/csrc/kernels.h b/mix_stage_amd/csrc/kernels.h
--- a/mix_stage_amd/csrc/kernels.h
+++ b/mix_stage_amd/csrc/kernels.h
@@ -172,6 +172,14 @@
 int clip32_block_fwd(const ms_conv_desc* d, const float* x, const float* x2, const float* wp, const float* bias, const float* gamma,
                      const float* beta, float* rm, float* rv, float* y_raw, float* y, float* save, float* part, int* sync,
                      int sync_words, hipStream_t s);
+extern int g_clip_corun;
+int clip32_hold_arm(hipStream_t s);
+int clip32_hold_flush(hipStream_t s);
+void clip32_hold_discard(hipStream_t s);
+int clip32_fwd_call_begin(hipStream_t s, bool clip_path, const void* ws, size_t ws_bytes);
+void clip32_fwd_call_end(hipStream_t s);
+int clip32_fwd_grid(const ms_conv_desc* d);
+bool clip32_fwd_pair_ok(const ms_conv_desc* host, const ms_conv_desc* guest);
 struct Clip32PrevBN { const float* y; const float* y_raw; const float* save; const float* gamma; float* dgamma; float* dbeta; float* dbias; float slope; };
 size_t clip32_dgrad_bn_part_bytes(const ms_conv_desc* d);
 bool clip32_dgrad_bn_ok(const ms_conv_desc* d);
diff --git a/mix_stage_amd/joint_late_cluster_soft_style.py b/mix_stage_amd/joint_late_cluster_soft_style.py
--- a/mix_stage_amd/joint_late_cluster_soft_style.py
+++ b/mix_stage_amd/joint_late_cluster_soft_style.py
@@ -105,15 +105,20 @@
     dt = getattr(self, '_ms_dt', 0)
     if dt:
       x = ops16.to_cb8(x, dt)
-    x = self.unet(x)
+    style = kwargs['style']
+    pose_style_encoder_flag = not kwargs['sample_flag'] and (kwargs['description'] == 'train' or not self.train_only)
+    pose_style_score = None
+    if pose_style_encoder_flag and not dt and isinstance(y, torch.Tensor):
+      x, pose_style_score = self.pose_style_encoder.forward_beside(y, self.unet, x)
+    else:
+      x = self.unet(x)
     x = ops.backward_marker(x)
     B, T = x.shape[0], x.shape[2]
 
-    style = kwargs['style']
-    pose_style_encoder_flag = not kwargs['sample_flag'] and (kwargs['description'] == 'train' or not self.train_only)
     if pose_style_encoder_flag:
       mode = 'lin'
-      pose_style_score = self.pose_style_encoder(y)
+      if pose_style_score is None:
+        pose_style_score = self.pose_style_encoder(y)
       style_id = style[:, 0].contiguous()
       id_in_loss = ops.cross_entropy(pose_style_score, style_id, scale=self.lambda_id)
       if self.softmax:
diff --git a/mix_stage_amd/layers.py b/mix_stage_amd/layers.py
--- a/mix_stage_amd/layers.py
+++ b/mix_stage_amd/layers.py
@@ -160,6 +160,17 @@
                           n.running_mean, n.running_var, x2=x2, in_mode=in_mode, chain_prev=chain_prev and mode == MS_BN_TRAIN,
                           link=link)
 
+  def _next_desc(self, x):
+    n = self.norm
+    if self._nd != 1 or getattr(self, '_ms_dt', 0) or x.dim() != 3 or (self._p and self.training):
+      return None
+    train = self.training and n.track_running_stats
+    if train and ops.bn_sync_active():
+      return None
+    w = self.conv.weight
+    return self._geometry().desc(x.shape[0], w.shape[1], 1, x.shape[2], w.shape[0] // self.conv.groups, MS_BN_TRAIN if train else MS_BN_EVAL,
+                                 MS_IN_PLAIN, 0)
+
   def forward(self, x, **kwargs):
     residual = kwargs.get('_residual')
     out_f32 = bool(kwargs.get('_out_f32'))
@@ -290,6 +301,14 @@
     return x
 
 
+def _chain_steps(stack, x):
+  x = ops.to_channel_major(x)
+  for i, m in enumerate(stack.conv):
+    yield m._next_desc(x)
+    x = m(x, _ms_chain=_chain_ok(stack.conv, i))
+  return x
+
+
 def _same_res_specs(cin):
   return ((cin, 64, False), (64, 64, False), (64, 128, False), (128, 128, False), (128, 256, False),
           (256, 256, False))
@@ -324,9 +343,21 @@
                  (256, 256, True), (256, num_speakers, True)), kernel_size, stride, p, groups)
 
   def forward(self, x, time_steps=None):
-    x = self._chain(x, last_f32=True)
+    return self._score(self._chain(x, last_f32=True))
+
+  @staticmethod
+  def _score(x):
     x = x.mean(-1) if x.shape[-1] > 1 else x.squeeze(-1)
     return x.squeeze(dim=-1)
+
+  def forward_beside(self, x, host, host_x):
+    blocks = [m for m in list(host.modules()) + list(self.modules()) if isinstance(m, ConvNormRelu)]
+    if (getattr(self, '_ms_dt', 0) or getattr(host, '_ms_dt', 0) or ops16.is_cb8(host_x) or not ops.corun_ok(x, host_x)
+        or any(p.dtype != torch.float32 for p in self.parameters()) or _hooked(host, self, *blocks)):
+      out = host(host_x)
+      return out, self(x)
+    out, z = ops.corun(lambda: host(host_x), _chain_steps(self, x), x.device)
+    return out, self._score(z)
 
 
 class ClusterClassify(nn.Module):
diff --git a/mix_stage_amd/ops.py b/mix_stage_amd/ops.py
--- a/mix_stage_amd/ops.py
+++ b/mix_stage_amd/ops.py
@@ -45,8 +45,13 @@
 
 
 
+_corun = {'driver': None, 'held': False, 'keep': [], 'on': os.environ.get('MS_CLIP_CORUN', '1') != '0', 'merges_offered': 0}
+
+
 def workspace(nbytes, device):
   key = (device.type, device.index, torch.cuda.current_stream(device).cuda_stream)
+  if _corun['held']:
+    key = key + ('held',)
   if USE_IN_LAUNCH_SPLIT_REDUCTION:
     _ensure_counters(device)
   ws = _workspaces.get(key)
@@ -385,6 +390,8 @@
       check(lib().ms_conv_block_fwd_ex(ctypes.byref(d), _ptr(x), _ptr(x2), _ptr(w), _ptr(bias), _ptr(gamma), _ptr(beta),
                                        _ptr(rm), _ptr(rv), _ptr(y_raw), _ptr(y), _ptr(save), _ptr(ws), ws.numel(),
                                        _stream(), ctypes.byref(opt)), 'ms_conv_block_fwd_ex')
+      if _corun['held']:
+        _corun['keep'].append((x, x2, w, bias, gamma, beta, rm, rv, y_raw, y, save, ws, planes, sync))
     ctx.geom_desc = d
     ctx.mode, ctx.in_mode = mode, in_mode
     ctx.prev = None
@@ -561,8 +568,97 @@
     return y.double()
   stats = (running_mean, running_var) if running_mean is not None else None
   prev = x.grad_fn if (chain_prev and _chain_fusion['on'] and x.grad_fn is not None and type(x.grad_fn).__name__ == '_ConvBlockFnBackward') else None
-  return _ConvBlockFn.apply(x, x2, w, bias, gamma, beta, geom, mode, in_mode, stats, None, prev,
-                            link if (link is not None and _chain_fusion['on'] and torch.is_grad_enabled()) else None)
+  link = link if (link is not None and _chain_fusion['on'] and torch.is_grad_enabled()) else None
+  drv = _corun['driver']
+  held = drv is not None and not drv.in_guest and geom.nd == 1 and drv.offer(x, x2, w, geom, mode, in_mode)
+  if not held:
+    return _ConvBlockFn.apply(x, x2, w, bias, gamma, beta, geom, mode, in_mode, stats, None, prev, link)
+  try:
+    y = _ConvBlockFn.apply(x, x2, w, bias, gamma, beta, geom, mode, in_mode, stats, None, prev, link)
+    check(lib().ms_clip_hold_flush(_stream()), 'ms_clip_hold_flush')
+  except BaseException:
+    lib().ms_clip_hold_discard(_stream())
+    raise
+  finally:
+    _corun['keep'].clear()
+  return y
+
+
+class _CoRun:
+
+  def __init__(self, guest_steps, device):
+    self.gen, self.in_guest, self.done, self.result = guest_steps, False, False, None
+    self.cus = torch.cuda.get_device_properties(device).multi_processor_count
+    self.next_desc = None
+    self._resume()
+
+  def _resume(self):
+    self.in_guest = True
+    try:
+      self.next_desc = next(self.gen)
+    except StopIteration as e:
+      self.done, self.result, self.next_desc = True, e.value, None
+    finally:
+      self.in_guest = False
+
+  def offer(self, x, x2, w, geom, mode, in_mode):
+    if self.done or self.next_desc is None or not x.is_cuda or x.dtype != torch.float32 or w.dtype != torch.float32:
+      return False
+    ref = x2 if in_mode == MS_IN_UP2ADD else x
+    if ref is None or ref.dim() != 3:
+      return False
+    L = lib()
+    d = geom.desc(x.shape[0], w.shape[1], 1, ref.shape[2], w.shape[0] // geom.groups, mode, in_mode, 0)
+    n_host, n_guest = L.ms_clip_grid(ctypes.byref(d)), L.ms_clip_grid(ctypes.byref(self.next_desc))
+    if not n_host or not n_guest or n_host + n_guest > self.cus or not L.ms_clip_pair_ok(ctypes.byref(d), ctypes.byref(self.next_desc)):
+      return False
+    stream = _stream()
+    check(L.ms_clip_hold(stream), 'ms_clip_hold')
+    _corun['held'] = True
+    try:
+      self._resume()
+    except BaseException:
+      L.ms_clip_hold_discard(stream)
+      raise
+    finally:
+      _corun['held'] = False
+    _corun['merges_offered'] += 1
+    return True
+
+  def finish(self):
+    while not self.done:
+      self._resume()
+    return self.result
+
+
+def corun(host_fn, guest_steps, device):
+  if _corun['driver'] is not None:
+    raise RuntimeError('corun: a guest chain is already riding along')
+  try:
+    drv = _CoRun(guest_steps, device)
+    _corun['driver'] = drv
+    try:
+      out = host_fn()
+    finally:
+      _corun['driver'] = None
+    return out, drv.finish()
+  except BaseException:
+    _corun['driver'] = None
+    lib().ms_clip_hold_discard(_stream())
+    _corun['keep'].clear()
+    raise
+
+
+def corun_ok(*tensors):
+  from . import ops16
+  return bool(_corun['on'] and _corun['driver'] is None and not bn_sync_active() and not _stat_pair['on'] and ops16.in_launch_meetings()
+              and lib().ms_get_precision() == 0 and all(t.is_cuda and t.dtype == torch.float32 for t in tensors))
+
+
+def enable_corun(on):
+  old = _corun['on']
+  _corun['on'] = bool(on)
+  return old
 
 
 _marker = {'cb': None}
```

New measurement: 11320 clips/s (median of 6 runs). 1.02x the previous value.
